# OzAmram/CaloDiffusion

Measured on AMD Instinct MI355X. Metric: sampled showers/sec (Dataset-2, 400-step DDIM), higher is better.
Workload: dtype f32 (convs: fp32 operands as 2-term fp16 splits on the fp16 MFMA pipe, fp32 accumulate; attention/norms fp32)

## Files before the change

calodiffusion_amd/csrc/cd_common.h:

```cpp
#pragma once
#include <hip/hip_runtime.h>
#include <stdint.h>
#include <stddef.h>
#include <string>

typedef float f32x4 __attribute__((ext_vector_type(4)));
typedef float f32x16 __attribute__((ext_vector_type(16)));

struct CdSamplerOp;

namespace cd {

void set_error(const std::string& msg);
struct Fail {
  int code;
  std::string msg;
};
#define CD_HIP(expr)                                                                                  \
  do {                                                                                                \
    hipError_t _e = (expr);                                                                           \
    if (_e != hipSuccess)                                                                             \
      throw cd::Fail{-2, std::string(#expr) + ": " + hipGetErrorString(_e)};                          \
  } while (0)
#define CD_REQUIRE(cond, msg)                                                                         \
  do {                                                                                                \
    if (!(cond)) throw cd::Fail{-1, std::string(msg)};                                                \
  } while (0)

namespace prof {
bool enabled();
void begin();
int end(char* buf, int cap);
struct Scope {
  Scope(const char* category, hipStream_t s, double flops, double bytes);
  ~Scope();
  int idx;
  hipStream_t stream;
};
}

enum ConvPrecision { PREC_F16X2 = 0, PREC_BF16X3 = 1, PREC_F32 = 2 };
int conv_precision();
void set_conv_precision(int p);
void set_conv_precision_override(int p);

struct Dims3 {
  int d, h, w;
  __host__ __device__ int64_t vox() const { return (int64_t)d * h * w; }
};

inline size_t packed_weight_floats(int cin, int cout, int taps) {
  return (size_t)(cin / 32) * taps * ((cout + 31) / 32) * 2048;
}

struct ConvGeom {
  Dims3 in, out;
  int kd, kh, kw;
  int sz, sh, sw;
};

__device__ __forceinline__ float cd_fast_silu(float t) {
  return t * __builtin_amdgcn_rcpf(1.f + __builtin_amdgcn_exp2f(t * -1.4426950408889634f));
}

struct GnDefer {
  const float* part = nullptr;
  int units = 0;
  const float* gamma = nullptr;
  const float* beta = nullptr;
  const float* add = nullptr;
  int add_ld = 0;
  int C = 0, groups = 0;
  int64_t vox = 0;
  float* coef_out = nullptr;
  float* stat_out = nullptr;
};

struct ConvFusion {
  const float* coef = nullptr;
  int act = 0;
  float* ch_part = nullptr;
  int* units = nullptr;
  const void* wpk_bf16x3 = nullptr;
  int* status = nullptr;
  GnDefer defer;
  float* coef_buf = nullptr;
  const unsigned* in_absmax = nullptr;
  const float* add_src = nullptr;
  int* add_done = nullptr;
  int zs_chunks = 0;
  struct GnOut {
    const float* gamma = nullptr;
    const float* beta = nullptr;
    int groups = 0;
    const float* res0 = nullptr;
    const float* res1 = nullptr;
    int res_c0 = 0;
    float* part_out = nullptr;
    int* done = nullptr;
  } gn_out;
};
struct AbsmaxWords {
  unsigned* next = nullptr;
  unsigned* end = nullptr;
  unsigned* take() {
    CD_REQUIRE(next && next < end, "internal: out of max-|x| words");
    return next++;
  }
};
const unsigned* launch_absmax_bits(const float* x, size_t n, AbsmaxWords* words, hipStream_t s);
__host__ __device__ inline void pow2_scale_for(unsigned mb, float* scale, float* inv) {
  const int e = (int)((mb >> 23) & 0xff) - 127;
  int sexp = mb == 0u ? 0 : 10 - e;
  sexp = sexp < -100 ? -100 : (sexp > 100 ? 100 : sexp);
  union { unsigned u; float f; } a, b;
  a.u = (unsigned)(127 + sexp) << 23;
  b.u = (unsigned)(127 - sexp) << 23;
  *scale = a.f;
  *inv = b.f;
}
inline size_t packed_bf16x3_bytes(int cin, int cout, int taps) {
  return (size_t)(cin / 16) * taps * ((cout + 31) / 32) * 3 * 64 * 16;
}
inline size_t packed_f16x2_bytes(int cin, int cout, int taps) {
  return (size_t)(cin / 16) * taps * ((cout + 31) / 32) * 2 * 64 * 16;
}
inline size_t packed_split16_bytes(int cin, int cout, int taps) {
  return packed_bf16x3_bytes(cin, cout, taps) + packed_f16x2_bytes(cin, cout, taps);
}
void launch_pack_weights_bf16x3(const float* w_torch, void* wpk, int cout, int cin, int taps, hipStream_t s,
                                bool transposed = false, bool flip = false);
void launch_pack_weights_f16x2(const float* w_torch, void* wpk, int cout, int cin, int taps, hipStream_t s,
                               bool transposed = false, bool flip = false);
inline void launch_pack_weights_split16(const float* w_torch, void* wpk, int cout, int cin, int taps, hipStream_t s,
                                        bool transposed = false, bool flip = false) {
  launch_pack_weights_bf16x3(w_torch, wpk, cout, cin, taps, s, transposed, flip);
  launch_pack_weights_f16x2(w_torch, (char*)wpk + packed_bf16x3_bytes(cin, cout, taps), cout, cin, taps, s, transposed, flip);
}

void launch_pack_weights(const float* w_torch, float* wpk, int cout, int cin, int taps, bool transposed, hipStream_t s,
                         bool flip = false);
void launch_pack_init_weights(const float* w_torch, float* wpk, int cout, int cin, hipStream_t s);
struct PackJob {
  const float* src;
  float* raw;
  float* pk;
  void* bf3;
  void* f16;
  int cout, cin, taps;
  int kind;
  int tr, flip;
  unsigned long long numel, n_pk, n_bf3, n_f16;
};
void launch_pack_jobs(const PackJob* d_jobs, int njobs, hipStream_t s);
void launch_pack_jobs_f16x2(const PackJob* d_jobs, int njobs, hipStream_t s);

void launch_conv_mfma(const float* in0, int c0, const float* in1, int c1, const float* wpk, const float* bias, float* out,
                      int batch, int cout, const ConvGeom& g, hipStream_t s, const ConvFusion& fu = ConvFusion());
bool try_launch_conv_zslide(const float* in0, int c0, const float* in1, int c1, const void* wpk_f16x2, const float* bias, float* out,
                            int batch, int cout, const ConvGeom& g, hipStream_t s, const ConvFusion& fu);
bool try_launch_conv_small(const float* in0, int c0, const float* in1, int c1, const void* wpk_f16x2, const float* bias, float* out,
                           int batch, int cout, const ConvGeom& g, hipStream_t s, const ConvFusion& fu);
void launch_conv_transpose_mfma(const float* in, int cin, const float* wpk, const float* bias, float* out, int batch,
                                int cout, Dims3 din, Dims3 dout, int kz, int sz, hipStream_t s,
                                const void* wpk_f16x2 = nullptr, int* status = nullptr, const unsigned* in_absmax = nullptr);

enum A_Prologue { A_NONE = 0, A_AFFINE = 1, A_SOFTMAX32 = 2, A_EXPNORM = 3 };
struct PointwiseArgs {
  const float* in0 = nullptr;
  int ld0 = 0, off0 = 0, c0 = 0;
  const float* in1 = nullptr;
  int ld1 = 0, c1 = 0;
  const float* wpk = nullptr;
  int64_t w_batch_stride = 0;
  const float* bias = nullptr;
  const float* residual = nullptr;
  float* out = nullptr;
  int batch = 0, cout = 0;
  int64_t vox = 0;
  int prologue = A_NONE;
  const float* coef = nullptr;
  int out_ld = 0, out_off = 0;
  float* ch_part = nullptr;
  const float* gn_res = nullptr;
  GnDefer gn_defer;
  const void* wpk16 = nullptr;
  int* status = nullptr;
};
inline int pointwise_units(int64_t vox) { return (int)((vox + 127) / 128); }
void launch_pointwise(const PointwiseArgs& a, hipStream_t s);

struct InitConvArgs {
  const float* x = nullptr;
  int cx = 0;
  int cin = 0;
  const float* scale_b = nullptr;
  int scale_stride = 1;
  const float* sigma_b = nullptr;
  float sigma_data = 1.f;
  const float* r_w = nullptr;
  const float* z_d = nullptr;
  const float* phi_h = nullptr;
  int use_rz = 0, use_phi = 0;
  const float* wpk = nullptr;
  const float* bias = nullptr;
  float* out = nullptr;
  int batch = 0, cout = 0;
  Dims3 dims{};
  float* coord_table = nullptr;
  bool table_ready = false;
  int* status = nullptr;
};
void launch_init_conv(const InitConvArgs& a, hipStream_t s);
void launch_init_coord_table(const InitConvArgs& a, hipStream_t s);

int gn_nsplit_for(int64_t vox, int batch);
void launch_ch_stats(const float* x, float* part, int batch, int channels, int64_t vox, int nsplit, hipStream_t s);
void launch_gn_finalize(const float* part, int units, const float* gamma, const float* beta, const float* add_bc, int add_ld,
                        float* coef, int batch, int channels, int groups, int64_t vox, hipStream_t s,
                        float* stat_out = nullptr );

size_t wgrad_partial_floats(int64_t out_vox, int batch, bool per_sample, int A, int Bc, int T);
struct WgradReduceJob {
  const float* partial;
  float* dw;
  int A, Bc, T, nslots, flags , b_total, b_off;
  unsigned first_block;
};
struct WgradReduceQueue {
  static constexpr int kMax = 80;
  WgradReduceJob job[kMax];
  int n = 0;
  unsigned blocks = 0;
};
void wgrad_queue_flush(WgradReduceQueue* q, hipStream_t s);
struct WgradAux {
  WgradReduceQueue* queue = nullptr;
  AbsmaxWords* words = nullptr;
  const unsigned* gmax = nullptr;
  const unsigned* xmax = nullptr;
};
void launch_wgrad(const float* g, int A, Dims3 dg, const float* x, int Bc, int xld, int xoff, Dims3 dx, int kd, int kh, int kw,
                  int sz, int sxy, int batch, bool per_sample, float* partial, float* dw, bool accumulate, bool transposed_out,
                  hipStream_t s, int b_total = 0, int b_off = 0,
                  const float* xcoef = nullptr, const WgradAux& aux = WgradAux());
// ... 26 lines not shown
  float* db;
  int nout, nin, delta_ld, in_ld;
};
void launch_linear_wgrad(const LinearWgradJob* jobs_dev, int njobs, int max_elems, int batch, hipStream_t s);
void launch_fold_phi(const float* src, float* dst, int batch, Dims3 d, int C, hipStream_t s);
void launch_add_slices(const float* a, int lda, int aoff, const float* b, int ldb, int boff, float* out, int channels,
                       int64_t rows, hipStream_t s);
void launch_bias_grad(const float* part, int units, int batch, int channels, float* db, bool accumulate, hipStream_t s);
size_t gn_backward_scratch_floats(int batch, int channels, int64_t vox);
struct GnParamJob {
  const float* sums_bc;
  float *dgamma, *dbeta, *dbias, *dsumdy;
  int batch, channels;
};
struct GnParamJobs {
  static constexpr int kMax = 64;
  GnParamJob job[kMax];
  int n = 0;
};
struct GnParamQueue {
  GnParamJobs jobs;
  float* sums = nullptr;
  float* sums_end = nullptr;
  float* next_sums = nullptr;
  bool discard = false;
};
void launch_gn_param_jobs(const GnParamJobs& jobs, hipStream_t s);
void launch_gn_backward(const float* dy, const float* h, const float* coef, const float* stat, const float* gamma, float* dh,
                        float* dgamma, float* dbeta, float* dadd, int dadd_ld, int batch, int channels, int64_t vox, int groups,
                        int silu, float* scratch, bool accumulate_params, hipStream_t s,
                        float* dbias = nullptr, float* dsumdy = nullptr,
                        GnParamQueue* queue = nullptr,
                        unsigned* dh_absmax = nullptr);
int gn_apply_blocks_per_sample(int batch, int channels, int64_t vox);
void launch_gn_apply(const float* x, float* y, const float* coef, int batch, int channels, int64_t vox, int silu,
                     const float* residual, const float* residual1, int res_c0, float* part_out, hipStream_t s,
                     const GnDefer* defer = nullptr);

int attn_nsplit_for(int64_t vox, int batch);
size_t attn_partial_floats(int batch, int nsplit);
void launch_attn_context(const float* qkv, float* partials, int batch, int64_t vox, int nsplit, hipStream_t s);
void launch_attn_combine(const float* partials, int nsplit, const float* w_out , int cout, float* wpk_b,
                         int batch, float scale, hipStream_t s, float* ctx_out = nullptr ,
                         float* kstat_out = nullptr ,
                         bool layout_T = false );

int attn_fused_nsplit_for(int64_t vox, int batch);
bool try_launch_res_block_small(const float* x0, int c0, const float* x1, int c1, const void* w1_f16x2, const float* b1,
                                const float* gn1_gamma, const float* gn1_beta, const float* emb, int emb_ld, const void* w2_f16x2,
                                const float* b2, const float* gn2_gamma, const float* gn2_beta, int groups, const float* res0,
                                const float* res1, int res_c0, float* h1, float* out, float* part_out, int batch, int cout,
                                Dims3 dims, int* status, hipStream_t s);
struct DeepLevelDesc {
  Dims3 dims{};
  int Ca = 0, Cb = 0, groups = 0;
  struct Res {
    int c0 = 0, c1 = 0, cout = 0;
    const void *w1 = nullptr, *w2 = nullptr;
    const float *b1 = nullptr, *b2 = nullptr, *g1 = nullptr, *be1 = nullptr, *g2 = nullptr, *be2 = nullptr;
    const float* emb = nullptr;
    int emb_ld = 0;
    const void* wres = nullptr;
    const float* bres = nullptr;
  } res[6];
  struct Attn {
    int C = 0;
    const float *ng = nullptr, *nb = nullptr, *wout = nullptr, *bout = nullptr, *gg = nullptr, *gb = nullptr;
    const void* wqkv = nullptr;
  } attn[3];
  int has_attn[3] = {0, 0, 0};
};
bool deep_level_eligible(const DeepLevelDesc& d);
void launch_deep_level(const DeepLevelDesc& d, const float* x_in, float* x_out, int batch, int* status, hipStream_t s);
struct DeepSideConv {
  const float* in = nullptr;
  int ldc = 0, cin = 0;
  const void* wpk = nullptr;
  const float* bias = nullptr;
  float* out = nullptr;
  int cout = 0;
  Dims3 dims{};
};
int deep_side_conv_chunks(int batch, int cin_side, int cout, Dims3 dims);
void launch_deep_level_side(const DeepLevelDesc& d, const float* x_in, float* x_out, int batch, int* status, const DeepSideConv& side,
                            hipStream_t s);
bool attn_small_eligible(int64_t vox);
void launch_attn_small(const float* x, int C, const float* coef, const void* wqkv_f16x2, float* partials, const float* w_out,
                       float scale, const float* bias, const float* out_gamma, const float* out_beta, float* y, float* ch_part,
                       int batch, int64_t vox, hipStream_t s, const GnDefer* defer, int* status = nullptr,
                       int max_parts = 1, unsigned* coop_sync = nullptr);
constexpr int kAttnCoopSamples = 8192;
bool attn_moments_eligible(int C);
size_t attn_moment_floats(int batch, int nsplit);
void launch_attn_kv_context(const float* x, int C, const float* coef, const void* wqkv_f16x2, float* partials, int batch,
                            int64_t vox, int nsplit, hipStream_t s, const GnDefer* defer = nullptr, int* status = nullptr,
                            float* moments = nullptr);
void launch_attn_out(const float* x, int C, const float* coef, const void* wqkv_f16x2, const float* wT_b, const float* bias,
                     float* y, float* ch_part , int batch, int64_t vox, int nsplit, hipStream_t s,
                     const GnDefer* defer = nullptr,
                     const float* partials = nullptr, const float* w_out = nullptr, float scale = 0.f, int* status = nullptr,
                     const float* moments = nullptr, const float* out_gamma = nullptr, const float* out_beta = nullptr);

struct EmbedLayer {
  const float* w;
  const float* b;
  int cout;
  int offset;
};
struct EmbedArgs {
  const float* cond = nullptr;
  const float* time_or_sigma = nullptr;
  int time_kind = 0;
  float sigma_data = 1.f;
  int cond_size = 0, cond_hidden = 0, half = 0;
  const float *tw1, *tb1, *tw2, *tb2, *tw3, *tb3;
  const float *cw1, *cb1, *cw2, *cb2, *cw3, *cb3;
  const EmbedLayer* layers = nullptr;
  int n_layers = 0;
  float* emb = nullptr;
  int emb_ld = 0;
  float* scal = nullptr;
  int batch = 0;
  int time_sin = 0, cond_sin = 0;
  int cond_rows = 0, time_stride = 0;
  int part = 0;
};
void launch_embed(const EmbedArgs& a, hipStream_t s);
void launch_silu_linear(const float* cond, const float* w, const float* bias, float* out, int batch, int nin, int nout,
                        hipStream_t s);

struct HeadArgs {
  const float* h = nullptr;
  const float* w = nullptr;
  const float* bias = nullptr;
  const float* x = nullptr;
  const float* scal = nullptr;
  int objective = 0;
  float* out = nullptr;
  int batch = 0;
  int64_t vox = 0;
  GnDefer defer;
  const float* res = nullptr;
  const float* upd_stepvals = nullptr;
  const float* upd_noise = nullptr;
  float* upd_x_next = nullptr;
  float* upd_xs = nullptr;
  float* upd_x0s = nullptr;
};
void launch_head(const HeadArgs& a, hipStream_t s);

void launch_ddim_update(const float* x, const float* x0, const float* noise, const float* stepvals, float* x_next,
                        float* xs_slot, float* x0s_slot, int64_t n, hipStream_t s);
struct StepChunk {
  const float* emb_src = nullptr;
  float* emb_dst = nullptr;
  int emb_floats = 0;
  const float* scal_src = nullptr;
  float* scal_dst = nullptr;
  int scal_floats = 0;
  int chunk_steps = 0;
  const float* emb_cond = nullptr;
};
void launch_load_step(const float* table, int* counter, float* stepvals, float* sigma_b, int batch, hipStream_t s,
                      const StepChunk* chunk = nullptr);
void launch_scale(const float* x, float* y, const float* stepvals_sigma, int64_t n, hipStream_t s);
void launch_scale_imm(const float* x, float* y, float scale, int64_t n, hipStream_t s);
void launch_randn(float* out, int64_t n, uint64_t seed, uint64_t offset, hipStream_t s);
void launch_randn_step(float* out, int64_t n, const uint64_t* seed_offset_stride_dev, const int* step_counter, hipStream_t s,
// ... 177 lines not shown
```

calodiffusion_amd/csrc/conv_internal.h:

```cpp
#pragma once
#include "cd_common.h"
#include "split16.h"
#include <cstdio>
#include <cstdlib>
#include <map>
#include <string>

namespace cd {

#define MFMA32(a, b, c) __builtin_amdgcn_mfma_f32_32x32x2f32((a), (b), (c), 0, 0, 0)
#define MFMA_BF16(a, b, c) __builtin_amdgcn_mfma_f32_32x32x16_bf16(__builtin_bit_cast(bf16x8, (a)), __builtin_bit_cast(bf16x8, (b)), (c), 0, 0, 0)

typedef __bf16 bf16x8 __attribute__((ext_vector_type(8)));
typedef __bf16 bf16x2 __attribute__((ext_vector_type(2)));

__device__ __forceinline__ unsigned pack_bf16(float lo, float hi) {
  const bf16x2 v = {(__bf16)lo, (__bf16)hi};
  return __builtin_bit_cast(unsigned, v);
}
__device__ __forceinline__ void split3(const f32x4 x, u32x2& t1, u32x2& t2, u32x2& t3) {
  f32x4 r = x;
  t1 = u32x2{pack_bf16(r[0], r[1]), pack_bf16(r[2], r[3])};
  r[0] -= __uint_as_float(t1[0] << 16); r[1] -= __uint_as_float(t1[0] & 0xffff0000u);
  r[2] -= __uint_as_float(t1[1] << 16); r[3] -= __uint_as_float(t1[1] & 0xffff0000u);
  t2 = u32x2{pack_bf16(r[0], r[1]), pack_bf16(r[2], r[3])};
  r[0] -= __uint_as_float(t2[0] << 16); r[1] -= __uint_as_float(t2[0] & 0xffff0000u);
  r[2] -= __uint_as_float(t2[1] << 16); r[3] -= __uint_as_float(t2[1] & 0xffff0000u);
  t3 = u32x2{pack_bf16(r[0], r[1]), pack_bf16(r[2], r[3])};
}

struct ConvKArgs {
  const float* in0;
  const float* in1;
  int c0, c1;
  const float* wpk;
  const float* bias;
  float* out;
  int Din, Hin, Win, Do, Ho, Wo;
  int KD, KH, KW, SZ, SH, SW;
  int TZ, TH, nTZ, nTH;
  int IZ, IH;
  int cout, CTtot;
  const float* coef;
  int act;
};
struct ConvTiled3Args {
  ConvKArgs k;
  float* ch_part;
  int* status;
};
void launch_conv_tiled_f32(int VT, int CT, const ConvKArgs& a, dim3 grid, int threads, size_t lds, hipStream_t s);
void launch_conv_tiled_split16(int VT, int CT, int NTERM, const ConvTiled3Args& a, dim3 grid, int threads, size_t lds, hipStream_t s);

struct ConvFlatArgs {
  const float* in0;
  const float* in1;
  int c0, c1;
  const float* wpk;
  const float* bias;
  float* out;
  int D, H, W;
  int Do, Ho, Wo;
  int R;
  int P;
  int cout, CTtot;
  int dbg;
  const float* coef;
  int act;
  float* ch_part;
  int* status = nullptr;
  GnDefer defer;
  int coef_lds_off = 0;
  const unsigned* in_absmax = nullptr;
  const float* add_src = nullptr;
};
bool try_launch_conv3_flat(const float* in0, int c0, const float* in1, int c1, const void* wpk, const float* bias, float* out,
                           int batch, int cout, const ConvGeom& g, hipStream_t s, const ConvFusion& fu,
                           int prec );
bool launch_conv_flat_split16(int VT, int CT, int NTERM, int geo, const ConvFlatArgs& a, dim3 grid, int threads, size_t lds, hipStream_t s);

std::map<std::string, int>& tune_cache();
template <typename F>
int autotune(const std::string& key, int ncand, F&& run, hipStream_t s) {
  auto it = tune_cache().find(key);
  if (it != tune_cache().end()) return it->second;
  hipStreamCaptureStatus st = hipStreamCaptureStatusNone;
  if (getenv("CD_NO_AUTOTUNE") || hipStreamIsCapturing(s, &st) != hipSuccess || st != hipStreamCaptureStatusNone || prof::enabled())
    return -1;
  hipEvent_t e0, e1;
  CD_HIP(hipEventCreate(&e0));
  CD_HIP(hipEventCreate(&e1));
  int best = 0;
  float best_ms = 1e30f;
  for (int i = 0; i < ncand; ++i) {
    run(i);
    CD_HIP(hipEventRecord(e0, s));
    run(i);
    run(i);
    CD_HIP(hipEventRecord(e1, s));
    CD_HIP(hipEventSynchronize(e1));
    float ms = 0.f;
    CD_HIP(hipEventElapsedTime(&ms, e0, e1));
    if (getenv("CD_TUNE_VERBOSE") && atoi(getenv("CD_TUNE_VERBOSE")) > 1) std::fprintf(stderr, "[calodiff autotune]   %s cand %d: %.1f us\n", key.c_str(), i, ms * 500.f);
    if (ms < best_ms) { best_ms = ms; best = i; }
  }
  hipEventDestroy(e0);
  hipEventDestroy(e1);
  tune_cache()[key] = best;
  if (getenv("CD_TUNE_VERBOSE")) std::fprintf(stderr, "[calodiff autotune] %s -> candidate %d (%.1f us)\n", key.c_str(), best, best_ms * 500.f);
  return best;
}

}
```

calodiffusion_amd/csrc/forward.hip:

```cpp
#include "plan_internal.h"

#include <cstdio>
#include <cstdlib>

namespace cd {

ResP resolve(const CdPlan* p, const ResW& w, const float* emb) {
  ResP r;
  r.cin = w.cin; r.cout = w.cout; r.has_res = w.has_res;
  r.c1w3 = p->packed3(w.c1w); r.c2w3 = p->packed3(w.c2w);
  r.c1w = p->packed(w.c1w); r.c1b = p->raw(w.c1b); r.n1g = p->raw(w.n1g); r.n1b = p->raw(w.n1b);
  r.c2w = p->packed(w.c2w); r.c2b = p->raw(w.c2b); r.n2g = p->raw(w.n2g); r.n2b = p->raw(w.n2b);
  if (w.has_res) {
    r.rw = p->packed(w.rw); r.rb = p->raw(w.rb);
    if (p->packed3(w.rw)) r.rw16 = (const char*)p->packed3(w.rw) + packed_bf16x3_bytes(w.cin, w.cout, 1);
  }
  if (w.has_mlp && emb) { r.emb = emb + w.emb_off; r.emb_ld = p->emb_ld; }
  return r;
}
AttnP resolve(const CdPlan* p, const AttnW& w) {
  AttnP a;
  a.c = w.c;
  a.ng = p->raw(w.ng); a.nb = p->raw(w.nb); a.qkv = p->packed(w.qkv); a.ow = p->raw(w.ow); a.ob = p->raw(w.ob);
  a.qkv16 = (const char*)p->packed3(w.qkv) + packed_bf16x3_bytes(w.c, 96, 1);
  a.gg = p->raw(w.gg); a.gb = p->raw(w.gb);
  a.coop_sync = p->d_attn_sync;
  return a;
}

float* stats_pass(Run& r, const float* x, int C, int64_t vox, int* units) {
  const int ns = gn_nsplit_for(vox, r.B);
  float* part = r.ws->get<float>((size_t)r.B * ns * C * 2);
  if (!r.dry()) launch_ch_stats(x, part, r.B, C, vox, ns, r.s);
  *units = ns;
  return part;
}

float* conv3_with_stats(Run& r, const float* x0, int c0, const float* x1, int c1, const float* wpk, const void* wpk3,
                        const float* bias, float* out, int cout, Dims3 dims, const float* coef_in, int* units,
                        const GnDefer* defer_in, float* coef_buf, const ConvFusion::GnOut* gn_out) {
  const int64_t vox = dims.vox();
  const int cap = (int)((vox + 31) / 32);
  float* part = r.ws->get<float>((size_t)r.B * cap * cout * 2);
  int u = 0;
  if (!r.dry()) {
    ConvGeom g{dims, dims, 3, 3, 3, 1, 1, 1};
    ConvFusion fu;
    fu.coef = coef_in; fu.act = 1; fu.ch_part = part; fu.units = &u; fu.wpk_bf16x3 = wpk3; fu.status = r.status;
    if (defer_in) { fu.defer = *defer_in; fu.coef_buf = coef_buf; fu.coef = nullptr; }
    if (gn_out) fu.gn_out = *gn_out;
    launch_conv_mfma(x0, c0, x1, c1, wpk, bias, out, r.B, cout, g, r.s, fu);
    if (gn_out && *gn_out->done) {
    } else if (u == 0) {
      u = gn_nsplit_for(vox, r.B);
      if (u > cap) u = cap;
      launch_ch_stats(out, part, r.B, cout, vox, u, r.s);
    }
  }
  *units = u;
  return part;
}

static float* conv3_x_half_with_stats(Run& r, const float* x0, int c0, int c1, const void* wpk3, float* out, int cout, Dims3 dims,
                                      int* units) {
  const int64_t vox = dims.vox();
  const int cap = (int)((vox + 31) / 32);
  float* part = r.ws->get<float>((size_t)r.B * cap * cout * 2);
  int u = 0;
  if (!r.dry()) {
    ConvGeom g{dims, dims, 3, 3, 3, 1, 1, 1};
    ConvFusion fu;
    int added = 0;
    fu.act = 1; fu.ch_part = part; fu.units = &u; fu.status = r.status; fu.add_src = out; fu.add_done = &added;
    char cat[128];
    std::snprintf(cat, sizeof cat, "conv3x3x3_s1 C%d(of %d)->%d @%dx%dx%d", c0, c0 + c1, cout, dims.d, dims.h, dims.w);
    prof::Scope scope(cat, r.s, 2.0 * 27 * c0 * cout * (double)vox * r.B, 4.0 * r.B * (double)vox * (c0 + 2 * cout));
    const bool ran = try_launch_conv_zslide(x0, c0, nullptr, 0, (const char*)wpk3 + packed_bf16x3_bytes(c0 + c1, cout, 27), nullptr, out,
                                            r.B, cout, g, r.s, fu);
    CD_REQUIRE(ran && added && u > 0, "internal: the x half of a side conv must run as a z-slide continuation");
  }
  *units = u;
  return part;
}

struct LazyClose {
  GnDefer gn;
  float* part = nullptr;
  bool on = false;
};
float* res_block(Run& r, const ResP& w, const float* x0, int c0, const float* x1, int c1, Dims3 dims,
                 float** part_out, int* units_out, LazyClose* lazy, float* h1_side) {
  Arena* ws = r.ws;
  CD_REQUIRE(c0 + c1 == w.cin, "internal: resnet block input width mismatch");
  const int64_t vox = dims.vox();
  const int G = r.groups;
  int u1 = 0, u2 = 0;
  static const bool defer_gn = getenv("CD_NO_GNDEFER") == nullptr;
  float* h1 = h1_side ? h1_side : ws->get<float>((size_t)r.B * vox * w.cout);
  const bool whole = vox <= 128 && w.cout == 32 && defer_gn && conv_precision() == PREC_F16X2 && w.c1w3 && w.c2w3;
  float* p1 = nullptr;
  CD_REQUIRE(!h1_side || (!whole && c1 > 0), "internal: a side conv belongs to a concat conv on a full-resolution grid");
  if (h1_side) p1 = conv3_x_half_with_stats(r, x0, c0, c1, w.c1w3, h1, w.cout, dims, &u1);
  else if (!whole) p1 = conv3_with_stats(r, x0, c0, x1, c1, w.c1w, w.c1w3, w.c1b, h1, w.cout, dims, nullptr, &u1);
  else p1 = ws->get<float>((size_t)r.B * ((vox + 31) / 32) * w.cout * 2);
  float* coef1 = ws->get<float>((size_t)r.B * w.cout * 4);
  GnDefer d1;
  d1.part = p1; d1.units = u1; d1.gamma = w.n1g; d1.beta = w.n1b; d1.add = w.emb; d1.add_ld = w.emb_ld; d1.C = w.cout; d1.groups = G;
  d1.vox = vox;
  if (!r.dry() && !defer_gn) launch_gn_finalize(p1, u1, w.n1g, w.n1b, w.emb, w.emb_ld, coef1, r.B, w.cout, G, vox, r.s);
  float* h2 = ws->get<float>((size_t)r.B * vox * w.cout);
  const bool small = vox <= 128;
  float* po = nullptr;
  const bool no_pw_close = getenv("CD_NO_PW_CLOSE") != nullptr;
  const bool pw_close = w.has_res && !small && defer_gn && !no_pw_close && w.cout <= 128;
  const int bps = pw_close ? pointwise_units(vox) : gn_apply_blocks_per_sample(r.B, w.cout, vox);
  if (part_out) {
    po = ws->get<float>((size_t)r.B * bps * w.cout * 2);
    *part_out = po;
  }
  float* res = nullptr;
  auto shortcut_conv = [&](const GnDefer* close = nullptr) {
    if (!close) res = ws->get<float>((size_t)r.B * vox * w.cout);
    if (!r.dry()) {
      PointwiseArgs a;
      a.in0 = x0; a.ld0 = c0; a.off0 = 0; a.c0 = c0; a.in1 = x1; a.ld1 = c1; a.c1 = c1;
      a.wpk = w.rw; a.bias = w.rb; a.out = close ? h2 : res; a.batch = r.B; a.cout = w.cout; a.vox = vox;
      if (conv_precision() == PREC_F16X2 && !getenv("CD_PW_F32")) { a.wpk16 = w.rw16; a.status = r.status; }
      if (close) { a.gn_res = h2; a.gn_defer = *close; a.ch_part = po; }
      launch_pointwise(a, r.s);
    }
  };
  if (small && w.has_res) shortcut_conv();
  int fused = 0;
  if (whole && !r.dry()) {
    const float* sc0 = w.has_res ? res : x0;
    const float* sc1 = w.has_res ? nullptr : (c1 ? x1 : nullptr);
    if (try_launch_res_block_small(x0, c0, x1, c1, (const char*)w.c1w3 + packed_bf16x3_bytes(c0 + c1, 32, 27), w.c1b, w.n1g, w.n1b,
                                   w.emb, w.emb_ld, (const char*)w.c2w3 + packed_bf16x3_bytes(32, 32, 27), w.c2b, w.n2g, w.n2b, G, sc0,
                                   sc1, w.has_res ? 0 : c0, h1, h2, po, r.B, w.cout, dims, r.status, r.s))
      fused = 2;
    else
      p1 = (ws->release(p1), conv3_with_stats(r, x0, c0, x1, c1, w.c1w, w.c1w3, w.c1b, h1, w.cout, dims, nullptr, &u1));
  }
  ConvFusion::GnOut go;
  if (small && defer_gn && fused != 2) {
    go.gamma = w.n2g; go.beta = w.n2b; go.groups = G; go.part_out = po; go.done = &fused;
    if (w.has_res) { go.res0 = res; }
    else { go.res0 = x0; go.res1 = c1 ? x1 : nullptr; go.res_c0 = c0; }
  }
  float* p2 = nullptr;
  if (fused == 2) p2 = ws->get<float>((size_t)r.B * ((vox + 31) / 32) * w.cout * 2);
  else p2 = conv3_with_stats(r, h1, w.cout, nullptr, 0, w.c2w, w.c2w3, w.c2b, h2, w.cout, dims, coef1, &u2, defer_gn ? &d1 : nullptr,
                             coef1, go.gamma ? &go : nullptr);
  ws->release(p1);
  ws->release(h1);
  ws->release(coef1);
  float* coef2 = ws->get<float>((size_t)r.B * w.cout * 4);
  GnDefer d2;
  d2.part = p2; d2.units = u2; d2.gamma = w.n2g; d2.beta = w.n2b; d2.C = w.cout; d2.groups = G; d2.vox = vox;
  if (!r.dry() && !defer_gn) launch_gn_finalize(p2, u2, w.n2g, w.n2b, nullptr, 0, coef2, r.B, w.cout, G, vox, r.s);
  const GnDefer* dp2 = defer_gn ? &d2 : nullptr;
  if (part_out) *units_out = fused ? 1 : bps;
  if (pw_close) {
    shortcut_conv(&d2);
  } else if (w.has_res) {
    if (!res) shortcut_conv();
    if (!r.dry() && !fused) launch_gn_apply(h2, h2, coef2, r.B, w.cout, vox, 1, res, nullptr, 0, po, r.s, dp2);
    ws->release(res);
  } else if (lazy && !small && defer_gn && c1 == 0 && w.cout == 32 && !part_out) {
    lazy->gn = d2;
    lazy->part = p2;
    lazy->on = true;
    ws->release(coef2);
    return h2;
  } else {
    if (!r.dry() && !fused) launch_gn_apply(h2, h2, coef2, r.B, w.cout, vox, 1, x0, c1 ? x1 : nullptr, c0, po, r.s, dp2);
  }
  ws->release(p2);
  ws->release(coef2);
  return h2;
}

float* attn_block(Run& r, const AttnP& w, const float* x, Dims3 dims, float* xpart, int xunits) {
  Arena* ws = r.ws;
  const int64_t vox = dims.vox();
// ... 184 lines not shown
  if (dx) {
    float* wp = pre ? nullptr : ws->get<float>(packed_weight_floats(c, c, T));
    float* wp3 = pre ? nullptr : ws->get<float>(packed_split16_bytes(c, c, T) / 4);
    if (!r.dry()) {
      if (!pre) {
        launch_pack_weights(w_raw, wp, c, c, T, false, r.s);
        launch_pack_weights_split16(w_raw, wp3, c, c, T, r.s, false, false);
      }
      ConvGeom gd{dout, din, kz, 4, 4, sz, 2, 2};
      ConvFusion fu;
      fu.wpk_bf16x3 = pre ? img->pk3 : wp3;
      dy_max = launch_absmax_bits(dy, (size_t)r.B * dout.vox() * c, &r.amax, r.s);
      fu.in_absmax = dy_max;
      launch_conv_mfma(dy, c, nullptr, 0, pre ? img->pk : wp, nullptr, dx, r.B, c, gd, r.s, fu);
    }
    if (wp3) ws->release(wp3);
    if (wp) ws->release(wp);
  }
  if (r.param_grads) {
    float* part = r.wgrad_part(wgrad_partial_floats(din.vox(), r.B, false, c, c, T));
    if (!r.dry())
      launch_wgrad(x, c, din, dy, c, c, 0, dout, kz, 4, 4, sz, 2, r.B, false, part, dw, false, false, r.s, 0, 0, nullptr,
                   r.wgrad_aux(nullptr, dy_max));
    r.release_wgrad_part(part);
    if (db) bias_grad(r, dy_full, c, dout_full.vox(), db);
  }
  if (folded) ws->release(folded);
}

bool deep_level_desc(const CdPlan* p, const float* emb, DeepLevelDesc* out) {
  const CdUnetDesc& d = p->desc;
  const int nres = p->nres;
  if (conv_precision() != PREC_F16X2) return false;
  DeepLevelDesc L;
  L.dims = p->shapes[nres - 1];
  L.Ca = d.layer_sizes[nres - 1]; L.Cb = d.layer_sizes[nres]; L.groups = d.groups;
  const ResW* rw[6] = {&p->downs[nres - 1].r1, &p->downs[nres - 1].r2, &p->mid1, &p->mid2, &p->ups[0].r1, &p->ups[0].r2};
  for (int i = 0; i < 6; ++i) {
    const ResW& w = *rw[i];
    DeepLevelDesc::Res& r = L.res[i];
    const bool cat = i == 4;
    r.c0 = cat ? L.Cb : w.cin; r.c1 = cat ? w.cin - L.Cb : 0; r.cout = w.cout;
    if (!p->packed3(w.c1w) || !p->packed3(w.c2w)) return false;
    r.w1 = (const char*)p->packed3(w.c1w) + packed_bf16x3_bytes(w.cin, w.cout, 27);
    r.w2 = (const char*)p->packed3(w.c2w) + packed_bf16x3_bytes(w.cout, w.cout, 27);
    r.b1 = p->raw(w.c1b); r.b2 = p->raw(w.c2b); r.g1 = p->raw(w.n1g); r.be1 = p->raw(w.n1b); r.g2 = p->raw(w.n2g); r.be2 = p->raw(w.n2b);
    if (w.has_mlp && emb) { r.emb = emb + w.emb_off; r.emb_ld = p->emb_ld; }
    if (w.has_res) {
      if (!p->packed3(w.rw)) return false;
      r.wres = (const char*)p->packed3(w.rw) + packed_bf16x3_bytes(w.cin, w.cout, 1);
      r.bres = p->raw(w.rb);
    }
  }
  const AttnW* aw[3] = {&p->downs[nres - 1].attn, &p->mid_attn, &p->ups[0].attn};
  const bool on[3] = {d.block_attn != 0, d.mid_attn != 0, d.block_attn != 0};
  for (int i = 0; i < 3; ++i) {
    L.has_attn[i] = on[i] ? 1 : 0;
    if (!on[i]) continue;
    const AttnW& w = *aw[i];
    DeepLevelDesc::Attn& a = L.attn[i];
    a.C = w.c; a.ng = p->raw(w.ng); a.nb = p->raw(w.nb); a.wout = p->raw(w.ow); a.bout = p->raw(w.ob); a.gg = p->raw(w.gg); a.gb = p->raw(w.gb);
    if (!p->packed3(w.qkv)) return false;
    a.wqkv = (const char*)p->packed3(w.qkv) + packed_bf16x3_bytes(w.c, 96, 1);
  }
  if (L.res[0].c0 != L.Ca || L.res[0].cout != L.Cb || L.res[4].cout != L.Ca || L.res[4].c1 != L.Cb || L.res[5].cout != L.Ca) return false;
  if (!deep_level_eligible(L)) return false;
  *out = L;
  return true;
}

float* unet_body(CdPlan* p, Run& r, const float* emb, float* h, LazyClose* lazy = nullptr, float** xin = nullptr) {
  const CdUnetDesc& d = p->desc;
  const int nres = p->nres;
  const int zs = d.compress_z ? 2 : 1;
  std::vector<float*> skips(nres, nullptr);
  float* x = h;
  int cx = d.layer_sizes[0];
  DeepLevelDesc deep;
  const bool deep_on = deep_level_desc(p, emb, &deep);
  const ResW& side_w = p->ups[nres - 1].r1;
  const int side_c = nres >= 2 ? d.layer_sizes[1] : 0;
  const bool side_on = deep_on && nres >= 2 && side_w.cin == 2 * side_c && p->packed3(side_w.c1w) &&
                       deep_side_conv_chunks(r.B, side_c, side_w.cout, p->shapes[0]) > 0;
  float* side_h1 = nullptr;
  for (int i = 0; i < nres; ++i) {
    const Dims3 dims = p->shapes[i];
    if (deep_on && i == nres - 1) {
      float* y = r.ws->get<float>((size_t)r.B * dims.vox() * cx);
      if (side_on) {
        side_h1 = r.ws->get<float>((size_t)r.B * p->shapes[0].vox() * side_w.cout);
        if (!r.dry()) {
          DeepSideConv sc;
          sc.in = skips[0]; sc.ldc = side_c; sc.cin = side_c;
          sc.wpk = (const char*)p->packed3(side_w.c1w) + packed_bf16x3_bytes(side_w.cin, side_w.cout, 27) +
                   (size_t)(side_c / 16) * 27 * (side_w.cout / 32) * 128 * 16;
          sc.bias = p->raw(side_w.c1b); sc.out = side_h1; sc.cout = side_w.cout; sc.dims = p->shapes[0];
          launch_deep_level_side(deep, x, y, r.B, r.status, sc, r.s);
        }
      } else if (!r.dry()) {
        launch_deep_level(deep, x, y, r.B, r.status, r.s);
      }
      r.ws->release(x);
      x = y;
      break;
    }
    float* t = res_block(r, resolve(p, p->downs[i].r1, emb), x, cx, nullptr, 0, dims);
    r.ws->release(x);
    x = t; cx = p->downs[i].r1.cout;
    float* xp = nullptr;
    int xu = 0;
    t = res_block(r, resolve(p, p->downs[i].r2, emb), x, cx, nullptr, 0, dims, d.block_attn ? &xp : nullptr, &xu);
    r.ws->release(x);
    x = t;
    if (d.block_attn) {
      t = attn_block(r, resolve(p, p->downs[i].attn), x, dims, xp, xu);
      r.ws->release(xp);
      r.ws->release(x);
      x = t;
    }
    skips[i] = x;
    if (i + 1 < nres) {
      const Dims3 nd = p->shapes[i + 1];
      float* y = r.ws->get<float>((size_t)r.B * nd.vox() * cx);
      if (!r.dry()) {
        ConvGeom g{dims, nd, 3, 4, 4, zs, 2, 2};
        ConvFusion fu;
        fu.wpk_bf16x3 = p->packed3(p->downs[i].sw);
        launch_conv_mfma(x, cx, nullptr, 0, p->packed(p->downs[i].sw), p->raw(p->downs[i].sb), y, r.B, cx, g, r.s, fu);
      }
      x = y;
    } else {
      x = skips[i];
    }
  }
  const Dims3 md = p->shapes[nres - 1];
  float* t = nullptr;
  if (!deep_on) {
    float* mp = nullptr;
    int mu = 0;
    t = res_block(r, resolve(p, p->mid1, emb), x, cx, nullptr, 0, md, d.mid_attn ? &mp : nullptr, &mu);
    x = t;
    if (d.mid_attn) {
      t = attn_block(r, resolve(p, p->mid_attn), x, md, mp, mu);
      r.ws->release(mp);
      r.ws->release(x);
      x = t;
    }
    t = res_block(r, resolve(p, p->mid2, emb), x, cx, nullptr, 0, md);
    r.ws->release(x);
    x = t;
  }

  for (int i = 0; i < nres; ++i) {
    const int lv = nres - 1 - i;
    const Dims3 dims = p->shapes[lv];
    const int cs = d.layer_sizes[lv + 1];
    if (!(deep_on && i == 0)) {
      CD_REQUIRE(cx == cs, "internal: up path width mismatch");
      t = res_block(r, resolve(p, p->ups[i].r1, emb), x, cx, skips[lv], cs, dims, nullptr, nullptr, nullptr,
                    lv == 0 ? side_h1 : nullptr);
      r.ws->release(x);
      r.ws->release(skips[lv]);
      x = t; cx = p->ups[i].r1.cout;
      float* up = nullptr;
      int uu = 0;
      t = res_block(r, resolve(p, p->ups[i].r2, emb), x, cx, nullptr, 0, dims, d.block_attn ? &up : nullptr, &uu);
      r.ws->release(x);
      x = t;
      if (d.block_attn) {
        t = attn_block(r, resolve(p, p->ups[i].attn), x, dims, up, uu);
        r.ws->release(up);
        r.ws->release(x);
        x = t;
      }
    }
    if (i + 1 < nres) {
      const Dims3 od = p->up_out[i];
      float* y = r.ws->get<float>((size_t)r.B * od.vox() * cx);
      if (!r.dry())
        launch_conv_transpose_mfma(x, cx, p->packed(p->ups[i].sw), p->raw(p->ups[i].sb), y, r.B, cx, dims, od, p->up_kz[i], zs, r.s,
                                   p->packed3(p->ups[i].sw), r.status);
      r.ws->release(x);
      x = y;
    }
  }
  t = res_block(r, resolve(p, p->fin, nullptr), x, cx, nullptr, 0, p->shapes[0], nullptr, nullptr, lazy);
  if (lazy && lazy->on) *xin = x;
  else r.ws->release(x);
  return t;
}

EmbedArgs embed_args(CdPlan* p, int B, const float* cond, const float* t, int kind, float* emb, float* scal) {
  const CdUnetDesc& d = p->desc;
  EmbedArgs e;
  e.cond = cond; e.time_or_sigma = t; e.time_kind = kind; e.sigma_data = d.sigma_data;
  e.cond_size = d.cond_size; e.half = d.cond_dim / 2;
  e.cond_hidden = d.cond_size > e.half / 2 ? d.cond_size : e.half / 2;
  e.time_sin = d.time_sin; e.cond_sin = d.cond_sin;
  e.tw1 = d.time_sin ? nullptr : p->raw(p->tw[0]); e.tb1 = d.time_sin ? nullptr : p->raw(p->tb[0]);
  e.tw2 = p->raw(p->tw[1]); e.tb2 = p->raw(p->tb[1]);
  e.tw3 = p->raw(p->tw[2]); e.tb3 = p->raw(p->tb[2]);
  e.cw1 = d.cond_sin ? nullptr : p->raw(p->cw[0]); e.cb1 = d.cond_sin ? nullptr : p->raw(p->cb[0]);
  e.cw2 = p->raw(p->cw[1]); e.cb2 = p->raw(p->cb[1]);
  e.cw3 = p->raw(p->cw[2]); e.cb3 = p->raw(p->cb[2]);
  e.layers = p->d_embed_layers; e.n_layers = p->n_embed_layers; e.emb = emb; e.emb_ld = p->emb_ld; e.scal = scal; e.batch = B;
  return e;
}

void forward_impl(CdPlan* p, int B, const float* x, const float* cond, const float* t, float* out, bool raw, hipStream_t s,
                  const FwdOpts* opt) {
  const CdUnetDesc& d = p->desc;
  const Dims3 dims = p->shapes[0];
  Run r{&p->ws, s, B, d.groups};
  r.status = p->status_word;
  const bool pre = opt && opt->emb_pre;
  float* emb = pre ? opt->emb_pre : p->ws.get<float>((size_t)B * p->emb_ld);
  float* scal = pre ? opt->scal_pre : p->ws.get<float>((size_t)B * 4);
  float* h = p->ws.get<float>((size_t)B * dims.vox() * d.layer_sizes[0]);
  if (!r.dry()) {
    if (!pre) launch_embed(embed_args(p, B, cond, t, raw ? CD_TIME_RAW : d.time_embed_kind, emb, raw ? nullptr : scal), s);
    InitConvArgs a;
    a.x = x; a.cin = d.in_channels; a.wpk = p->packed(p->init_w); a.bias = p->raw(p->init_b); a.out = h; a.batch = B;
    a.cout = d.layer_sizes[0]; a.dims = dims;
    if (raw) {
      a.cx = d.in_channels;
    } else {
      a.cx = 1; a.sigma_b = t; a.sigma_data = d.sigma_data; a.use_rz = d.rz_input; a.use_phi = d.phi_input;
      a.r_w = p->d_coords; a.z_d = p->d_coords + d.grid[2]; a.phi_h = p->d_coords + d.grid[2] + d.grid[0];
      a.coord_table = p->d_init_table; a.table_ready = true; a.status = r.status;
    }
    launch_init_conv(a, s);
  }
  LazyClose lazy;
  float* xin = nullptr;
  static const bool head_fused = getenv("CD_NO_HEAD_GN") == nullptr;
  float* hf = unet_body(p, r, emb, h, head_fused ? &lazy : nullptr, &xin);
  if (!r.dry()) {
    HeadArgs ha;
    ha.h = hf; ha.w = p->raw(p->head_w); ha.bias = p->raw(p->head_b); ha.out = out; ha.batch = B; ha.vox = dims.vox();
    if (!raw) { ha.x = x; ha.scal = scal; ha.objective = d.objective; }
    if (lazy.on) { ha.defer = lazy.gn; ha.res = xin; }
    if (opt && opt->upd) {
      ha.upd_stepvals = opt->upd->upd_stepvals; ha.upd_noise = opt->upd->upd_noise; ha.upd_x_next = opt->upd->upd_x_next;
// ... 98 lines not shown
```

calodiffusion_amd/csrc/kernels_conv_flat.hip:

```cpp
#include "conv_internal.h"
#include "gn_defer.h"
#include <vector>

namespace cd {

template <int VT, int CT>
__global__ void __launch_bounds__(512, (VT * CT <= 2 ? 3 : 2)) conv3_flat_kernel(ConvFlatArgs a) {
  extern __shared__ __attribute__((aligned(16))) float lds[];
  const int tid = threadIdx.x, lane = tid & 63, wave = tid >> 6, nthreads = blockDim.x;
  const int b = blockIdx.y;
  const int ct0 = blockIdx.z * CT;
  const int HW = a.H * a.W;
  const int vox = a.D * HW;
  const int v0 = blockIdx.x * a.R;
  const int vend = min(v0 + a.R, vox);
  const int zA = v0 / HW - 1;
  const int zB = (vend - 1) / HW + 1;
  const int nstage = (zB - zA + 1) * HW;
  const int NZ = a.P * HW;
  const int half = lane >> 5, col = lane & 31;
  if (tid < 16) lds[NZ * 16 + tid] = 0.f;

  int nb[VT], rowm[VT], rowp[VT], ooff[VT];
  unsigned wmask[VT];
// ... 381 lines not shown
          const int off = __shfl(ooff, row, 64);
          if (off >= 0) {
#pragma unroll
            for (int ct = 0; ct < CT; ++ct) {
              const float v = acc[ct][r] + bv[ct];
              outb[off + (ct0 + ct) * 32 + col] = v;
              s1[ct] += v;
              s2[ct] += v * v;
            }
          }
        }
        if (a.ch_part) {
#pragma unroll
          for (int ct = 0; ct < CT; ++ct) {
            const float t1 = s1[ct] + __shfl_xor(s1[ct], 32, 64), t2 = s2[ct] + __shfl_xor(s2[ct], 32, 64);
            if (half == 0) {
              scratch[((mw * CT + ct) * 32 + col) * 2] = t1;
              scratch[((mw * CT + ct) * 32 + col) * 2 + 1] = t2;
            }
          }
        }
      }
    }
    __syncthreads();
  }
  if (loader && a.ch_part && nph > 0) {
    const int u = blockIdx.x + (my_units - 1) * gridDim.x;
    for (int i = tid; i < CT * 32; i += nlw * 64) {
      float t1 = 0.f, t2 = 0.f;
      for (int w = 0; w < nmw; ++w) {
        t1 += scratch[((w * CT * 32) + i) * 2];
        t2 += scratch[((w * CT * 32) + i) * 2 + 1];
      }
      float* dst = a.ch_part + ((size_t)u * a.cout + ct0 * 32 + i) * 2;
      dst[0] = t1;
      dst[1] = t2;
    }
  }
}

namespace {
template <int CT, int KD, int KH, int KW, int SZ, int SXY>
void launch_ws_geo(const ConvFlatArgs& a, dim3 grid, int threads, size_t lds, int nlw, int ups, int total, hipStream_t s) {
  static bool attr_set = false;
  if (!attr_set) {
    CD_HIP(hipFuncSetAttribute((const void*)conv_flat_ws_kernel<CT, KD, KH, KW, SZ, SXY>,
                               hipFuncAttributeMaxDynamicSharedMemorySize, 160 * 1024));
    attr_set = true;
  }
  hipLaunchKernelGGL((conv_flat_ws_kernel<CT, KD, KH, KW, SZ, SXY>), grid, dim3(threads), lds, s, a, nlw, ups, total);
  CD_HIP(hipGetLastError());
}
template <int CT>
void launch_ws_inst(const ConvFlatArgs& a, dim3 grid, int threads, size_t lds, int nlw, int ups, int total, hipStream_t s, int geo) {
  if (geo == 0) launch_ws_geo<CT, 3, 3, 3, 1, 1>(a, grid, threads, lds, nlw, ups, total, s);
  else if (geo == 1) launch_ws_geo<CT, 3, 4, 4, 2, 2>(a, grid, threads, lds, nlw, ups, total, s);
  else if (geo == 2) launch_ws_geo<CT, 3, 4, 4, 1, 2>(a, grid, threads, lds, nlw, ups, total, s);
  else launch_ws_geo<CT, 4, 4, 4, 2, 2>(a, grid, threads, lds, nlw, ups, total, s);
}

template <int VT, int CT>
void launch_flat_inst(const ConvFlatArgs& a, dim3 grid, int threads, size_t lds, hipStream_t s) {
  static bool attr_set = false;
  if (!attr_set) {
    CD_HIP(hipFuncSetAttribute((const void*)conv3_flat_kernel<VT, CT>, hipFuncAttributeMaxDynamicSharedMemorySize, 160 * 1024));
    attr_set = true;
  }
  hipLaunchKernelGGL((conv3_flat_kernel<VT, CT>), grid, dim3(threads), lds, s, a);
  CD_HIP(hipGetLastError());
}

bool launch_conv_flat_f32(int VT, int CT, const ConvFlatArgs& a, dim3 grid, int threads, size_t lds, hipStream_t s) {
#define CD_FLAT_CASE(V, C)                                   \
  if (VT == V && CT == C) {                                  \
    launch_flat_inst<V, C>(a, grid, threads, lds, s);        \
    return true;                                             \
  }
  CD_FLAT_CASE(1, 1) CD_FLAT_CASE(2, 1) CD_FLAT_CASE(3, 1) CD_FLAT_CASE(4, 1)
  CD_FLAT_CASE(1, 2) CD_FLAT_CASE(2, 2) CD_FLAT_CASE(3, 2) CD_FLAT_CASE(4, 2)
  CD_FLAT_CASE(1, 3) CD_FLAT_CASE(2, 3)
#undef CD_FLAT_CASE
  return false;
}
}

bool try_launch_conv3_flat(const float* in0, int c0, const float* in1, int c1, const void* wpk, const float* bias, float* out,
                           int batch, int cout, const ConvGeom& g, hipStream_t s, const ConvFusion& fu, int prec) {
  const bool bf16x3 = prec != 0;
  if (getenv("CD_NO_FLAT")) return false;
  int geo = -1;
  if (g.kd == 3 && g.kh == 3 && g.kw == 3 && g.sz == 1 && g.sh == 1 && g.sw == 1) geo = 0;
  else if (g.kd == 3 && g.kh == 4 && g.kw == 4 && g.sh == 2 && g.sw == 2 && (g.sz == 1 || g.sz == 2)) geo = g.sz == 2 ? 1 : 2;
  else if (g.kd == 4 && g.kh == 4 && g.kw == 4 && g.sh == 2 && g.sw == 2 && g.sz == 2) geo = 3;
  if (geo < 0 || (geo != 0 && !bf16x3)) return false;
  const Dims3 d = g.in;
  const int CTtot = cout / 32;
  const int CTmax = CTtot <= 3 ? CTtot : 2;
  if (CTtot % CTmax) return false;
  const int HW = d.h * d.w, HWo = g.out.h * g.out.w;
  const size_t vox_bytes = prec == 3 ? 96 : (prec == 2 ? 80 : 64);
  auto planes = [&](int NT) { return ((32 * NT - 1) / HWo + 1) * g.sz + g.kd; };
  auto args_for = [&](int NT) {
    ConvFlatArgs a;
    a.in0 = in0; a.in1 = in1; a.c0 = c0; a.c1 = c1; a.wpk = (const float*)wpk; a.bias = bias; a.out = out;
    a.D = d.d; a.H = d.h; a.W = d.w; a.Do = g.out.d; a.Ho = g.out.h; a.Wo = g.out.w;
    a.R = 32 * NT; a.P = planes(NT); a.cout = cout; a.CTtot = CTtot;
    a.coef = fu.coef; a.act = fu.act; a.ch_part = fu.ch_part;
    return a;
  };
  auto launch = [&](int NT, int VT, int CT) -> bool {
    if (VT < 0) {
      const int NLW = -VT;
      ConvFlatArgs a = args_for(NT);
      a.dbg = 0;
      const size_t lds = 2 * ((size_t)a.P * HW + 1) * 96 + (size_t)NT * CT * 64 * 4;
      const int ups = (int)((g.out.vox() + a.R - 1) / a.R);
      const int total = ups * batch;
      const int nblk = total < 256 ? total : 256;
      dim3 grid((unsigned)nblk, 1, (unsigned)(CTtot / CT));
      if (fu.units) *fu.units = ups;
      const int threads = (NT + NLW) * 64;
      switch (CT) {
        case 1: launch_ws_inst<1>(a, grid, threads, lds, NLW, ups, total, s, geo); break;
        case 2: launch_ws_inst<2>(a, grid, threads, lds, NLW, ups, total, s, geo); break;
        case 3: launch_ws_inst<3>(a, grid, threads, lds, NLW, ups, total, s, geo); break;
        default: return false;
      }
      return true;
    }
    ConvFlatArgs a = args_for(NT);
    a.dbg = getenv("CD_FLAT_DBG") ? atoi(getenv("CD_FLAT_DBG")) : 0;
    a.status = fu.status; a.in_absmax = fu.in_absmax;
    a.add_src = prec >= 2 && !bias ? fu.add_src : nullptr;
    size_t lds = ((size_t)a.P * HW + 1) * vox_bytes;
    const size_t red = (size_t)(NT / VT) * CT * 32 * 2 * 4;
    if (lds < red) lds = red;
    if (fu.defer.part) {
      lds = (lds + 15) & ~(size_t)15;
      a.defer = fu.defer;
      a.coef_lds_off = (int)lds;
      lds += (size_t)fu.defer.C * 16 + gn_defer_scratch_bytes(fu.defer.C);
      if (lds > 160 * 1024) return false;
    }
    dim3 grid((unsigned)((g.out.vox() + a.R - 1) / a.R), (unsigned)batch, (unsigned)(CTtot / CT));
    if (fu.units) *fu.units = (int)grid.x;
    const int threads = (NT / VT) * 64;
    const bool launched = prec != 0 ? launch_conv_flat_split16(VT, CT, prec, geo, a, grid, threads, lds, s)
                                    : launch_conv_flat_f32(VT, CT, a, grid, threads, lds, s);
    if (!launched) return false;
    if (a.add_src && fu.add_done) *fu.add_done = 1;
    return true;
  };
  if (const char* ov = getenv("CD_FLAT_TILE")) {
    int nt, vt;
    if (sscanf(ov, "%d,%d", &nt, &vt) == 2 && nt % vt == 0 && nt / vt <= 8 && vt * CTmax <= 8 &&
        ((size_t)planes(nt) * HW + 1) * vox_bytes <= 160 * 1024 && (prec != 2 || vt * CTmax <= 4))
      return launch(nt, vt, CTmax);
  }
  static const int kCand[][2] = {{8, 2}, {4, 1}, {8, 1}, {12, 3}, {16, 2}, {16, 4}, {4, 2}, {6, 2}, {6, 3}, {2, 1},
                                 {3, 1}, {1, 1}, {2, 2}, {12, 2}, {8, 4}, {6, 1}, {3, 3}};
  struct Cand { int nt, vt, ct; };
  std::vector<Cand> cand;
  const bool small = g.out.vox() * batch <= 64 * 1024;
  for (int pass = 0; pass < (small && CTmax > 1 ? 2 : 1); ++pass) {
    const int CT = pass == 0 ? CTmax : 1;
    for (auto& c : kCand) {
      const int NT = c[0], VT = c[1];
      if (VT * CT > 8 || (CT == 3 && VT > 2)) continue;
      if (prec == 2 && VT * CT > 4) continue;
      static const bool no_extra_waves = getenv("CD_FLAT_NO_EXTRA_WAVES") != nullptr;
      const bool extra_ok = !no_extra_waves && g.out.vox() <= 128 && VT == 1 && NT <= 8;
      if ((int64_t)32 * (NT - 1) >= g.out.vox() && !extra_ok) continue;
      if (((size_t)planes(NT) * HW + 1) * vox_bytes > 150 * 1024) continue;
      if (pass == 1 && NT > 4) continue;
      cand.push_back({NT, VT, CT});
    }
  }
  if (prec == 3 && !getenv("CD_NO_WS")) {
    static const int kWs[][2] = {{8, 4}, {8, 2}, {4, 2}, {4, 4}, {8, 3}, {6, 2}, {2, 2}, {3, 1}, {1, 1}, {2, 1}};
    for (auto& c : kWs) {
      const int NMW = c[0], NLW = c[1];
      if ((int64_t)32 * (NMW - 1) >= g.out.vox()) continue;
      const size_t lds = 2 * ((size_t)planes(NMW) * HW + 1) * 96 + (size_t)NMW * CTmax * 64 * 4;
      if (lds > 160 * 1024 - 256) continue;
      cand.push_back({NMW, -NLW, CTmax});
    }
  }
  if (cand.empty()) return false;
  char key[192];
  std::snprintf(key, sizeof key, "flat%s g%d %dx%dx%d c%d+%d->%d b%d", prec == 3 ? "_bf16x3" : (prec == 2 ? "_f16x2" : "_f32"), geo,
                d.d, d.h, d.w, c0, c1, cout, batch);
  const int pick = autotune(key, (int)cand.size(), [&](int i) { launch(cand[i].nt, cand[i].vt, cand[i].ct); }, s);
  const Cand& c = cand[pick < 0 ? 0 : pick];
  return launch(c.nt, c.vt, c.ct);
}

}
```

calodiffusion_amd/csrc/kernels_conv_flat16.hip:

```cpp
#include "conv_internal.h"
#include "gn_defer.h"

namespace cd {

template <int VT, int CT, int KD, int KH, int KW, int SZ, int SXY, int NTERM>
__global__ void __launch_bounds__(512, (VT * CT * (NTERM == 2 ? 2 : 1) <= 2 ? 3 : 2)) conv3_flat_bf16x3_kernel(ConvFlatArgs a) {
  extern __shared__ __attribute__((aligned(16))) float lds[];
  char* ldsb = (char*)lds;
  constexpr int T = KD * KH * KW;
  constexpr int VB = NTERM == 3 ? 96 : 80;
  constexpr int WS = 64 * NTERM;
  const int tid = threadIdx.x, lane = tid & 63, wave = tid >> 6, nthreads = blockDim.x;
  const int b = blockIdx.y;
  const int ct0 = blockIdx.z * CT;
  const int HW = a.H * a.W;
  const int vox = a.D * HW;
  const int HWo = a.Ho * a.Wo;
  const int voxo = a.Do * HWo;
  const int v0 = blockIdx.x * a.R;
  const int vend = min(v0 + a.R, voxo);
  const float inv_hwo = 1.f / (float)HWo, inv_wo = 1.f / (float)a.Wo;
  auto fdiv = [](int x, float inv) { return (int)(((float)x + 0.5f) * inv); };
  const int zA = fdiv(v0, inv_hwo) * SZ - 1;
  const int zB = fdiv(vend - 1, inv_hwo) * SZ + KD - 2;
  const int nstage = (zB - zA + 1) * HW;
  const int NZ = a.P * HW;
  const int half = lane >> 5, col = lane & 31;
  if (a.defer.part) gn_defer_to_lds(a.defer, b, (float*)(ldsb + a.coef_lds_off), ldsb + a.coef_lds_off + a.defer.C * 16);
  const bool normed = a.coef || a.defer.part;
  if (tid < VB / 4) ((float*)(ldsb + (size_t)NZ * VB))[tid] = 0.f;

  int nb[VT], rowoff[VT][KH], ooff[VT];
  unsigned wmask[VT];
  bool any_valid = false;
#pragma unroll
  for (int vt = 0; vt < VT; ++vt) {
    const int v = v0 + (wave * VT + vt) * 32 + col;
    const bool valid = v < vend;
    const int vv = valid ? v : v0;
    const int oz = fdiv(vv, inv_hwo);
    const int r = vv - oz * HWo;
    const int oh = fdiv(r, inv_wo), ow = r - oh * a.Wo;
    const int ih0 = oh * SXY, iw0 = ow * SXY;
    nb[vt] = (oz * SZ - 1 - zA) * HW + ih0 * a.W + iw0;
    unsigned m = 0;
#pragma unroll
    for (int kh = 0; kh < KH; ++kh) {
      int ih = ih0 + kh - 1;
      ih = ih < 0 ? ih + a.H : (ih >= a.H ? ih - a.H : ih);
      ih = ih >= a.H ? ih - a.H : ih;
      rowoff[vt][kh] = (ih - ih0) * a.W;
    }
#pragma unroll
    for (int kw = 0; kw < KW; ++kw) {
      const int iw = iw0 + kw - 1;
      if (valid && iw >= 0 && iw < a.W) m |= 1u << kw;
    }
    wmask[vt] = m;
    ooff[vt] = valid ? v * a.cout : -1;
    any_valid |= valid;
  }
  const bool wave_active = __any(any_valid);

  f32x16 acc[VT][CT], accB[NTERM == 2 ? VT : 1][NTERM == 2 ? CT : 1];
#pragma unroll
  for (int vt = 0; vt < VT; ++vt)
#pragma unroll
    for (int ct = 0; ct < CT; ++ct)
#pragma unroll
      for (int r = 0; r < 16; ++r) {
        acc[vt][ct][r] = 0.f;
        if (NTERM == 2) accB[vt][ct][r] = 0.f;
      }

  float amax = 0.f;
  float gscale = 1.f, ginv = 1.f;
  if (NTERM == 2 && a.in_absmax) pow2_scale_for(*a.in_absmax, &gscale, &ginv);
  const int nsub = (a.c0 + a.c1) >> 4;
  const int gbase = zA * HW;
  const int nslots = nstage * 4;

  auto tap_voxel = [&](int vt, int tap) -> int {
#ifdef CD_FLAT_ABL_TAPS
    return nb[vt] + tap;
#endif
    const int kz = tap / (KH * KW), kh = (tap / KW) % KH, kw = tap % KW;
    const int n = nb[vt] + kz * HW + rowoff[vt][kh] + kw - 1;
    return ((wmask[vt] >> kw) & 1u) ? n : NZ;
  };

  for (int sc = 0; sc < nsub; ++sc) {
    const float* src;
    int ldc, coff;
    if (sc * 16 < a.c0) {
      src = a.in0; ldc = a.c0; coff = sc * 16;
    } else {
      src = a.in1; ldc = a.c1; coff = sc * 16 - a.c0;
    }
    const int pq = tid & 3;
    src += (size_t)b * vox * ldc + coff + pq * 4;
    f32x4 cf[4];
    if (a.defer.part) {
#pragma unroll
      for (int e = 0; e < 4; ++e) cf[e] = *(const f32x4*)(ldsb + a.coef_lds_off + (sc * 16 + pq * 4 + e) * 16);
    } else if (a.coef) {
#pragma unroll
      for (int e = 0; e < 4; ++e) cf[e] = *(const f32x4*)(a.coef + ((size_t)b * (a.c0 + a.c1) + sc * 16 + pq * 4 + e) * 4);
    }
    __syncthreads();
    for (int s0 = tid; s0 < ((a.dbg & 1) ? 0 : nslots); s0 += 4 * nthreads) {
      f32x4 val[4];
#pragma unroll
      for (int k = 0; k < 4; ++k) {
        const int sidx = s0 + k * nthreads;
        const int g = gbase + (sidx >> 2);
        val[k] = f32x4{0.f, 0.f, 0.f, 0.f};
        if (sidx < nslots && g >= 0 && g < vox) {
          val[k] = *(const f32x4*)(src + (size_t)g * ldc);
          if (normed) {
#pragma unroll
            for (int e = 0; e < 4; ++e) {
              float t = cf[e][0] * val[k][e] + cf[e][1];
              if (a.act) t = cd_fast_silu(t);
              val[k][e] = t + cf[e][2];
            }
          }
        }
      }
#pragma unroll
      for (int k = 0; k < 4; ++k) {
        const int sidx = s0 + k * nthreads;
        if (sidx < nslots) {
          char* d = ldsb + (size_t)(sidx >> 2) * VB + pq * 8;
          if (NTERM == 3) {
            u32x2 t1, t2, t3;
            split3(val[k], t1, t2, t3);
            *(u32x2*)d = t1;
            *(u32x2*)(d + 32) = t2;
            *(u32x2*)(d + 64) = t3;
          } else {
            const f32x4 vs = val[k] * gscale;
            amax = fmaxf(amax, fmaxf(fmaxf(fabsf(vs[0]), fabsf(vs[1])), fmaxf(fabsf(vs[2]), fabsf(vs[3]))));
            u32x2 t1, t2;
            split2(vs, t1, t2);
            *(u32x2*)d = t1;
            *(u32x2*)(d + 32) = t2;
          }
        }
      }
    }
    __syncthreads();
    if (!wave_active || (a.dbg & 2)) continue;

#pragma unroll
    for (int vt = 0; vt < VT; ++vt) asm volatile("" : "+v"(nb[vt]));

    const u32x4* wq = (const u32x4*)a.wpk + ((size_t)sc * T * a.CTtot + ct0) * WS + lane;
#ifndef CD_FLAT_WD
#define CD_FLAT_WD 3
#endif
#ifndef CD_FLAT_AD
#define CD_FLAT_AD 2
#endif
    constexpr bool DEEP = NTERM == 2;
    constexpr int WD = DEEP ? CD_FLAT_WD : 1, AD = DEEP ? CD_FLAT_AD : 1;
    u32x4 bw[WD + 1][CT][NTERM], av[AD + 1][VT][NTERM];
    auto load_w = [&](int tap) {
#pragma unroll
      for (int ct = 0; ct < CT; ++ct)
#pragma unroll
        for (int t = 0; t < NTERM; ++t) bw[tap % (WD + 1)][ct][t] = wq[((size_t)tap * a.CTtot + ct) * WS + t * 64];
    };
    auto load_a = [&](int tap) {
#pragma unroll
      for (int vt = 0; vt < VT; ++vt) {
        const char* p = ldsb + (size_t)tap_voxel(vt, tap) * VB + half * 16;
#pragma unroll
        for (int t = 0; t < NTERM; ++t) av[tap % (AD + 1)][vt][t] = *(const u32x4*)(p + t * 32);
      }
    };
#pragma unroll
    for (int t0 = 0; t0 < WD; ++t0) load_w(t0);
#pragma unroll
    for (int t0 = 0; t0 < AD; ++t0) load_a(t0);
#pragma unroll
    for (int tap = 0; tap < T; ++tap) {
      if (tap + WD < T) load_w(tap + WD);
      if (tap + AD < T) load_a(tap + AD);
      __builtin_amdgcn_sched_barrier(0);
      const int wc = tap % (WD + 1), ac = tap % (AD + 1);
#pragma unroll
      for (int vt = 0; vt < VT; ++vt)
#pragma unroll
        for (int ct = 0; ct < CT; ++ct) {
          if (NTERM == 3) {
            f32x16 c = acc[vt][ct];
            c = MFMA_BF16(av[ac][vt][NTERM - 1], bw[wc][ct][0], c);
            c = MFMA_BF16(av[ac][vt][1], bw[wc][ct][1], c);
            c = MFMA_BF16(av[ac][vt][0], bw[wc][ct][NTERM - 1], c);
            c = MFMA_BF16(av[ac][vt][1], bw[wc][ct][0], c);
            c = MFMA_BF16(av[ac][vt][0], bw[wc][ct][1], c);
            c = MFMA_BF16(av[ac][vt][0], bw[wc][ct][0], c);
            acc[vt][ct] = c;
          } else {
            acc[vt][ct] = MFMA_F16(av[ac][vt][0], bw[wc][ct][0], acc[vt][ct]);
            accB[vt][ct] = MFMA_F16(av[ac][vt][0], bw[wc][ct][1], accB[vt][ct]);
            accB[vt][ct] = MFMA_F16(av[ac][vt][1], bw[wc][ct][0], accB[vt][ct]);
          }
        }
    }
  }

  if (NTERM == 2) {
#pragma unroll
    for (int vt = 0; vt < VT; ++vt)
#pragma unroll
      for (int ct = 0; ct < CT; ++ct)
#pragma unroll
        for (int r = 0; r < 16; ++r) acc[vt][ct][r] = (acc[vt][ct][r] + accB[vt][ct][r] * (1.f / 2048.f)) * ginv;
  }
  if (NTERM == 2 && a.status && amax > 65504.f) atomicOr(a.status, 1);
  float* outb = a.out + (size_t)b * voxo * a.cout;
  float bv[CT];
#pragma unroll
  for (int ct = 0; ct < CT; ++ct) bv[ct] = a.bias ? a.bias[(ct0 + ct) * 32 + col] : 0.f;
  if (a.add_src) {
    const float* addb = a.add_src + (size_t)b * voxo * a.cout;
#pragma unroll
    for (int vt = 0; vt < VT; ++vt) {
      float ad[16][CT];
#pragma unroll
      for (int r = 0; r < 16; ++r) {
        const int off = __shfl(ooff[vt], (r & 3) + 8 * (r >> 2) + 4 * half, 64);
#pragma unroll
        for (int ct = 0; ct < CT; ++ct) ad[r][ct] = off >= 0 ? addb[off + (ct0 + ct) * 32 + col] : 0.f;
      }
#pragma unroll
      for (int r = 0; r < 16; ++r)
#pragma unroll
        for (int ct = 0; ct < CT; ++ct) acc[vt][ct][r] += ad[r][ct];
    }
  }
#pragma unroll
  for (int vt = 0; vt < VT; ++vt) {
#pragma unroll
    for (int r = 0; r < 16; ++r) {
      const int row = (r & 3) + 8 * (r >> 2) + 4 * half;
      const int off = __shfl(ooff[vt], row, 64);
      if (off >= 0) {
#pragma unroll
        for (int ct = 0; ct < CT; ++ct) outb[off + (ct0 + ct) * 32 + col] = acc[vt][ct][r] + bv[ct];
      }
    }
  }
  if (a.ch_part) {
    float s1[CT], s2[CT];
#pragma unroll
    for (int ct = 0; ct < CT; ++ct) s1[ct] = s2[ct] = 0.f;
#pragma unroll
    for (int vt = 0; vt < VT; ++vt)
#pragma unroll
      for (int r = 0; r < 16; ++r) {
        const int row = (r & 3) + 8 * (r >> 2) + 4 * half;
        const bool ok = __shfl(ooff[vt], row, 64) >= 0;
#pragma unroll
        for (int ct = 0; ct < CT; ++ct) {
          const float v = ok ? acc[vt][ct][r] + bv[ct] : 0.f;
          s1[ct] += v;
          s2[ct] += v * v;
        }
      }
    __syncthreads();
    const int nw = nthreads >> 6;
#pragma unroll
    for (int ct = 0; ct < CT; ++ct) {
      const float t1 = s1[ct] + __shfl_xor(s1[ct], 32, 64), t2 = s2[ct] + __shfl_xor(s2[ct], 32, 64);
      if (half == 0) {
        lds[((wave * CT + ct) * 32 + col) * 2] = t1;
        lds[((wave * CT + ct) * 32 + col) * 2 + 1] = t2;
      }
    }
    __syncthreads();
    for (int i = tid; i < CT * 32; i += nthreads) {
      float t1 = 0.f, t2 = 0.f;
      for (int w = 0; w < nw; ++w) {
        t1 += lds[((w * CT * 32) + i) * 2];
        t2 += lds[((w * CT * 32) + i) * 2 + 1];
      }
      float* dst = a.ch_part + (((size_t)b * gridDim.x + blockIdx.x) * a.cout + ct0 * 32 + i) * 2;
      dst[0] = t1;
      dst[1] = t2;
    }
  }
}

namespace {
template <int VT, int CT, int KD, int KH, int KW, int SZ, int SXY, int NTERM>
void launch_flat3_geo(const ConvFlatArgs& a, dim3 grid, int threads, size_t lds, hipStream_t s) {
  static bool attr_set = false;
  if (!attr_set) {
    CD_HIP(hipFuncSetAttribute((const void*)conv3_flat_bf16x3_kernel<VT, CT, KD, KH, KW, SZ, SXY, NTERM>,
                               hipFuncAttributeMaxDynamicSharedMemorySize, 160 * 1024));
    attr_set = true;
  }
  hipLaunchKernelGGL((conv3_flat_bf16x3_kernel<VT, CT, KD, KH, KW, SZ, SXY, NTERM>), grid, dim3(threads), lds, s, a);
  CD_HIP(hipGetLastError());
}
template <int VT, int CT, int NTERM>
void launch_flat3_inst(const ConvFlatArgs& a, dim3 grid, int threads, size_t lds, hipStream_t s, int geo = 0) {
  if (geo == 0) launch_flat3_geo<VT, CT, 3, 3, 3, 1, 1, NTERM>(a, grid, threads, lds, s);
  else if (geo == 1) launch_flat3_geo<VT, CT, 3, 4, 4, 2, 2, NTERM>(a, grid, threads, lds, s);
  else if (geo == 2) launch_flat3_geo<VT, CT, 3, 4, 4, 1, 2, NTERM>(a, grid, threads, lds, s);
  else launch_flat3_geo<VT, CT, 4, 4, 4, 2, 2, NTERM>(a, grid, threads, lds, s);
}
}

bool launch_conv_flat_split16(int VT, int CT, int NTERM, int geo, const ConvFlatArgs& a, dim3 grid, int threads, size_t lds, hipStream_t s) {
#define CD_FLAT_CASE(V, C)                                                                 \
  if (VT == V && CT == C) {                                                                \
    if (NTERM == 3) launch_flat3_inst<V, C, 3>(a, grid, threads, lds, s, geo);             \
    else if constexpr (V * C <= 4) launch_flat3_inst<V, C, 2>(a, grid, threads, lds, s, geo); \
    else return false;                                                                     \
    return true;                                                                           \
  }
  CD_FLAT_CASE(1, 1) CD_FLAT_CASE(2, 1) CD_FLAT_CASE(3, 1) CD_FLAT_CASE(4, 1)
  CD_FLAT_CASE(1, 2) CD_FLAT_CASE(2, 2) CD_FLAT_CASE(3, 2) CD_FLAT_CASE(4, 2)
  CD_FLAT_CASE(1, 3) CD_FLAT_CASE(2, 3)
#undef CD_FLAT_CASE
  return false;
}

}
```

calodiffusion_amd/csrc/kernels_deep_side.hip:

```cpp
#include "cd_common.h"
#include "split16.h"
#include "gn_defer.h"

#include <cstdio>
#include <cstdlib>
#include <cstring>

namespace cd {

#include "deep_body.inc"
#include "conv_zs_body.inc"

namespace {

static_assert(DC_THREADS == 256, "both roles are programs of four waves");

struct DeepSideArgs {
  DeepArgs deep;
  ConvZsArgs side;
  int ndeep;
};

template <int NT>
__global__ void __launch_bounds__(256, 1) deep_level_side_kernel(DeepSideArgs a) {
  extern __shared__ __attribute__((aligned(16))) char ds_lds[];
  const int bx = blockIdx.x;
  if (bx < a.ndeep) {
    deep_level_body<NT>(a.deep, ds_lds, bx);
    return;
  }
  const int j = bx - a.ndeep;
  ZsBlk kb;
  kb.y = j / a.side.nchunk;
  kb.x = j - kb.y * a.side.nchunk;
  kb.z = 0;
  kb.nx = a.side.nchunk;
  switch (threadIdx.x >> 6) {
    case 0: z3_wave<0, false, 0, 0, ZS_NSL>(a.side, ds_lds, kb); break;
    case 1: z3_wave<1, false, 0, 0, ZS_NSL>(a.side, ds_lds, kb); break;
    case 2: z3_wave<2, false, 0, 0, ZS_NSL>(a.side, ds_lds, kb); break;
    default: z3_wave<3, false, 0, 0, ZS_NSL>(a.side, ds_lds, kb); break;
  }
}

template <int NT>
void launch_deep_side_inst(const DeepSideArgs& a, unsigned grid, size_t lds, hipStream_t s) {
  static bool attr_set = false;
  if (!attr_set) {
    CD_HIP(hipFuncSetAttribute((const void*)deep_level_side_kernel<NT>, hipFuncAttributeMaxDynamicSharedMemorySize, 160 * 1024));
    attr_set = true;
  }
  hipLaunchKernelGGL(deep_level_side_kernel<NT>, dim3(grid), dim3(256), lds, s, a);
  CD_HIP(hipGetLastError());
}

int side_ring(const Dims3& d) { return d.h * d.w >= 2 * ZS_STEP ? 4 : 5; }
size_t side_lds(const Dims3& d) {
  const size_t plane = ((size_t)d.h * d.w * ZS_VB + 255) & ~(size_t)255;
  return (size_t)ZS_ZERO + Z3_COEF + (size_t)side_ring(d) * plane + 2 * Z3_XCH;
}

}

int deep_side_conv_chunks(int batch, int cin_side, int cout, Dims3 dims) {
  if (getenv("CD_NO_DEEP_SIDE_CONV")) return 0;
  static const bool zs_switched = getenv("CD_NO_ZSLIDE") || getenv("CD_ZS_V1") || getenv("CD_ZS_STRIP") || getenv("CD_ZS_DBG") ||
                                  getenv("CD_ZS_NSL5") || getenv("CD_ZS_NSL");
  if (zs_switched) return 0;
  if (Z3_PAD || cin_side != 32 || cout != 32 || batch < 1) return 0;
  const int PV = dims.h * dims.w;
  if (PV < ZS_STEP || PV > ZS_NSL * 32 || side_lds(dims) > 160 * 1024) return 0;
  const int64_t svox = (int64_t)dims.d * PV;
  int best = 0;
  int64_t best_gap = 0;
  for (int n = 1; n <= 8 && svox >= (int64_t)2 * ZS_STEP * n; ++n) {
    const int64_t cv = ((svox + n - 1) / n + ZS_STEP - 1) / ZS_STEP * ZS_STEP;
    if ((svox + cv - 1) / cv != n) continue;
    const int64_t total = (int64_t)batch * (1 + n);
    const int64_t gap = (total + 255) / 256 * 256 - total;
    if (!best || gap < best_gap) { best = n; best_gap = gap; }
  }
  return best;
}

void launch_deep_level_side(const DeepLevelDesc& d, const float* x_in, float* x_out, int batch, int* status, const DeepSideConv& sc,
                            hipStream_t s) {
  DeepSideArgs a;
  double flops = 0.0;
  const size_t lds_deep = deep_fill_args(d, x_in, x_out, status, &a.deep, &flops);
  const int nchunk = deep_side_conv_chunks(batch, sc.cin, sc.cout, sc.dims);
  CD_REQUIRE(nchunk > 0 && sc.in && sc.wpk && sc.out, "internal: deep level launched with an ineligible side conv");
  const int PV = sc.dims.h * sc.dims.w;
  const int64_t svox = (int64_t)sc.dims.d * PV;
  ConvZsArgs& z = a.side;
  z = ConvZsArgs{};
  z.in = sc.in; z.ldc = sc.ldc; z.coef = nullptr; z.coef_c = sc.cin; z.act = 0;
  z.wpk = (const u32x4*)sc.wpk; z.CTtot = sc.cout / 32;
  z.bias = sc.bias; z.acc_delta = 0; z.out = sc.out; z.cout = sc.cout; z.ch_part = nullptr;
  z.D = sc.dims.d; z.H = sc.dims.h; z.W = sc.dims.w; z.NR = side_ring(sc.dims); z.HS = sc.dims.h;
  z.nchunk = nchunk;
  z.CV = (int)(((svox + nchunk - 1) / nchunk + ZS_STEP - 1) / ZS_STEP * ZS_STEP);
  z.status = status; z.defer = GnDefer(); z.choff = 0; z.in_absmax = nullptr; z.dbg = 0;
  a.ndeep = batch;
  const size_t lds_side = side_lds(sc.dims);
  const size_t lds = lds_deep > lds_side ? lds_deep : lds_side;
  const int64_t grid = (int64_t)batch * (1 + nchunk);
  CD_REQUIRE(lds <= 160 * 1024 && grid < (1ll << 31), "deep level + side conv: launch geometry out of range");
  const double vox = (double)d.dims.vox();
  char cat[128];
  std::snprintf(cat, sizeof cat, "deep_level C%d/%d @%dx%dx%d + conv3x3x3 K-block C%d->%d @%dx%dx%d", d.Ca, d.Cb, d.dims.d, d.dims.h,
                d.dims.w, sc.cin, sc.cout, sc.dims.d, sc.dims.h, sc.dims.w);
  prof::Scope scope(cat, s, flops * batch + 2.0 * 27 * sc.cin * sc.cout * (double)svox * batch,
                    8.0 * batch * vox * d.Ca + 4.0 * batch * (double)svox * (sc.cin + sc.cout));
  const int NT = (int)((d.dims.vox() + 31) / 32);
  switch (NT) {
    case 1: launch_deep_side_inst<1>(a, (unsigned)grid, lds, s); break;
    case 2: launch_deep_side_inst<2>(a, (unsigned)grid, lds, s); break;
    case 3: launch_deep_side_inst<3>(a, (unsigned)grid, lds, s); break;
    default: launch_deep_side_inst<4>(a, (unsigned)grid, lds, s); break;
  }
}

}
```

calodiffusion_amd/csrc/ops.hip:

```cpp
#include "plan_internal.h"

extern "C" {

static AbsmaxWords op_absmax_words(Arena& ws, hipStream_t s) {
  constexpr size_t kWords = 8;
  unsigned* w = ws.get<unsigned>(kWords);
  CD_HIP(hipMemsetAsync(w, 0, sizeof(unsigned) * kWords, s));
  return AbsmaxWords{w, w + kWords};
}
size_t cd_op_scratch_bytes(int batch, int max_channels, int64_t max_voxels) {
  return (size_t)256 * 256 * 64 * 4 * 4 + (size_t)batch * 64 * 64 * 16 + (size_t)batch * max_channels * max_voxels * 4 + (1 << 20);
}

int cd_op_to_channels_last(const float* ncdhw, float* ndhwc, int batch, int channels, int64_t voxels, void* stream) {
  return guarded([&] { launch_transpose_to_cl(ncdhw, ndhwc, batch, channels, voxels, (hipStream_t)stream); });
}
int cd_op_to_ncdhw(const float* ndhwc, float* ncdhw, int batch, int channels, int64_t voxels, void* stream) {
  return guarded([&] { launch_transpose_to_planar(ndhwc, ncdhw, batch, channels, voxels, (hipStream_t)stream); });
}

int cd_op_cyl_conv(const float* x0, int c0, const float* x1, int c1, const float* w, const float* bias, float* y,
                   int batch, int cout, const int32_t dims_in[3], const int32_t kernel[3], const int32_t stride[3],
                   void* scratch, void* stream) {
  return guarded([&] {
    CD_REQUIRE(x0 && w && y && scratch, "null argument");
    hipStream_t s = (hipStream_t)stream;
    const int taps = kernel[0] * kernel[1] * kernel[2];
    float* wpk = (float*)scratch;
    launch_pack_weights(w, wpk, cout, c0 + c1, taps, false, s);
    const Dims3 din{dims_in[0], dims_in[1], dims_in[2]};
    if (taps == 1) {
      PointwiseArgs a;
      a.in0 = x0; a.ld0 = c0; a.c0 = c0; a.in1 = x1; a.ld1 = c1; a.c1 = c1; a.wpk = wpk; a.bias = bias; a.out = y;
      a.batch = batch; a.cout = cout; a.vox = din.vox();
      launch_pointwise(a, s);
    } else {
      CD_REQUIRE(cout % 32 == 0, "cout must be a multiple of 32");
      ConvGeom g;
      g.in = din;
      g.kd = kernel[0]; g.kh = kernel[1]; g.kw = kernel[2]; g.sz = stride[0]; g.sh = stride[1]; g.sw = stride[2];
      g.out = Dims3{(din.d + 2 - g.kd) / g.sz + 1, (din.h + 2 - g.kh) / g.sh + 1, (din.w + 2 - g.kw) / g.sw + 1};
      ConvFusion fu;
      if (taps == 27 || taps == 48) {
        float* w3 = wpk + packed_weight_floats(c0 + c1, cout, taps);
        launch_pack_weights_split16(w, w3, cout, c0 + c1, taps, s);
        fu.wpk_bf16x3 = w3;
      }
      launch_conv_mfma(x0, c0, x1, c1, wpk, bias, y, batch, cout, g, s, fu);
    }
  });
}

int cd_op_zslide_conv(const float* x, int cin, const float* w, const float* bias, float* y, float* ch_part, int* units, int batch,
                      int cout, const int32_t dims[3], int chunks, void* scratch, void* stream) {
  return guarded([&] {
    CD_REQUIRE(x && w && y && ch_part && units && scratch && chunks >= 0, "bad argument");
    CD_REQUIRE(cin % 32 == 0 && cout % 32 == 0, "channel counts must be multiples of 32");
    hipStream_t s = (hipStream_t)stream;
    launch_pack_weights_f16x2(w, scratch, cout, cin, 27, s);
    const Dims3 d{dims[0], dims[1], dims[2]};
    ConvGeom g{d, d, 3, 3, 3, 1, 1, 1};
    ConvFusion fu;
    int u = 0;
    fu.act = 1; fu.ch_part = ch_part; fu.units = &u; fu.zs_chunks = chunks;
    CD_REQUIRE(try_launch_conv_zslide(x, cin, nullptr, 0, scratch, bias, y, batch, cout, g, s, fu) && u > 0,
               "this grid is not eligible for the z-slide kernel");
    *units = u;
  });
}

int cd_op_cyl_conv_transpose(const float* x, const float* w, const float* bias, float* y, int batch, int channels,
                             const int32_t dims_in[3], int kernel_z, int stride_z, const int32_t out_pad[3],
                             void* scratch, void* stream) {
  return guarded([&] {
    CD_REQUIRE(x && w && y && scratch, "null argument");
    CD_REQUIRE(out_pad[0] == 0, "z output padding is always 0 (models.py:339)");
    hipStream_t s = (hipStream_t)stream;
    float* wpk = (float*)scratch;
    launch_pack_weights(w, wpk, channels, channels, kernel_z * 16, true, s);
    float* wpk16 = wpk + ((packed_weight_floats(channels, channels, kernel_z * 16) + 63) & ~(size_t)63);
    launch_pack_weights_f16x2(w, wpk16, channels, channels, kernel_z * 16, s, true, false);
    const Dims3 din{dims_in[0], dims_in[1], dims_in[2]};
    const Dims3 dout{(din.d - 1) * stride_z - 2 + kernel_z, 2 * din.h + out_pad[1], 2 * din.w + out_pad[2]};
    launch_conv_transpose_mfma(x, channels, wpk, bias, y, batch, channels, din, dout, kernel_z, stride_z, s, wpk16, nullptr);
  });
}

int cd_op_init_conv(const float* x_ncdhw, const float* w, const float* bias, float* y, int batch, int cin, int cout,
                    const int32_t dims[3], void* scratch, void* stream) {
  return guarded([&] {
    CD_REQUIRE(x_ncdhw && w && y && scratch, "null argument");
    hipStream_t s = (hipStream_t)stream;
    float* wpk = (float*)scratch;
    launch_pack_init_weights(w, wpk, cout, cin, s);
    InitConvArgs a;
    a.x = x_ncdhw; a.cx = cin; a.cin = cin; a.wpk = wpk; a.bias = bias; a.out = y; a.batch = batch; a.cout = cout;
    a.dims = Dims3{dims[0], dims[1], dims[2]};
    launch_init_conv(a, s);
  });
}

int cd_op_group_norm(const float* x, float* y, const float* gamma, const float* beta, int batch, int channels,
                     int64_t voxels, int groups, int silu, const float* add_bc, const float* residual,
                     void* scratch, void* stream) {
  return guarded([&] {
    CD_REQUIRE(x && y && gamma && beta && scratch, "null argument");
    hipStream_t s = (hipStream_t)stream;
    const int ns = gn_nsplit_for(voxels, batch);
    float* part = (float*)scratch;
    float* coef = part + (size_t)batch * ns * channels * 2;
    launch_ch_stats(x, part, batch, channels, voxels, ns, s);
    launch_gn_finalize(part, ns, gamma, beta, add_bc, channels, coef, batch, channels, groups, voxels, s);
    launch_gn_apply(x, y, coef, batch, channels, voxels, silu, residual, nullptr, 0, nullptr, s);
  });
}

int cd_op_resnet_block(const float* x0, int c0, const float* x1, int c1, const float* const* w, const float* cond, float* y,
                       int batch, int cout, const int32_t dims[3], int groups, void* workspace, size_t workspace_bytes,
                       void* stream) {
  return guarded([&] {
    CD_REQUIRE(x0 && w && y && workspace, "null argument");
    hipStream_t s = (hipStream_t)stream;
    const int cin = c0 + c1;
    Arena ws;
    ws.reset((char*)workspace, workspace_bytes, false);
    float* p1 = ws.get<float>(packed_weight_floats(cin, cout, 27));
    float* p2 = ws.get<float>(packed_weight_floats(cout, cout, 27));
    launch_pack_weights(w[0], p1, cout, cin, 27, false, s);
    launch_pack_weights(w[4], p2, cout, cout, 27, false, s);
    float* q1 = ws.get<float>(packed_split16_bytes(cin, cout, 27) / 4);
    float* q2 = ws.get<float>(packed_split16_bytes(cout, cout, 27) / 4);
    launch_pack_weights_split16(w[0], q1, cout, cin, 27, s);
    launch_pack_weights_split16(w[4], q2, cout, cout, 27, s);
    ResP r;
    r.cin = cin; r.cout = cout; r.has_res = w[10] != nullptr;
    r.c1w3 = q1; r.c2w3 = q2;
    r.c1w = p1; r.c1b = w[1]; r.n1g = w[2]; r.n1b = w[3]; r.c2w = p2; r.c2b = w[5]; r.n2g = w[6]; r.n2b = w[7];
    if (r.has_res) {
      float* p3 = ws.get<float>(packed_weight_floats(cin, cout, 1));
      launch_pack_weights(w[10], p3, cout, cin, 1, false, s);
      r.rw = p3; r.rb = w[11];
    }
    if (w[8] && cond) {
      float* emb = ws.get<float>((size_t)batch * cout);
      launch_silu_linear(cond, w[8], w[9], emb, batch, 128, cout, s);
      r.emb = emb; r.emb_ld = cout;
    }
    Run run{&ws, s, batch, groups};
    const Dims3 d{dims[0], dims[1], dims[2]};
    float* out = res_block(run, r, x0, c0, x1, c1, d);
    CD_HIP(hipMemcpyAsync(y, out, sizeof(float) * (size_t)batch * d.vox() * cout, hipMemcpyDeviceToDevice, s));
  });
}
// ... 77 lines not shown
```

calodiffusion_amd/csrc/plan_internal.h:

```cpp
#pragma once
#include "../../include/calodiff.h"
#include "cd_common.h"

#include <map>
#include <string>
#include <vector>

namespace cd {

enum PackKind { PK_NONE = 0, PK_CONV = 1, PK_CONVT = 2, PK_INIT = 3 };
struct WeightEntry {
  std::string name;
  int64_t numel = 0;
  size_t raw_off = 0;
  PackKind pack = PK_NONE;
  int cin = 0, cout = 0, taps = 0;
  size_t pk_off = 0;
  size_t pk3_off = 0;
  size_t grad_off = 0;
  bool set = false;
  int dg_mode = 0;
  size_t dg_pk_off = 0, dg_pk3_off = 0;
  bool dg_1x1 = false;
};
// ... 151 lines not shown
    if (dg_images && w.dg_mode) {
      g.pk = dg_images + w.dg_pk_off;
      if (w.dg_mode != 1) g.pk3 = dg_images + w.dg_pk3_off;
    }
    return g;
  }
  unsigned* d_attn_sync = nullptr;
  StepGraph ddim_graph, prog_graph;

  size_t grad_floats = 0;
  std::vector<LinearWgradJob> lin_jobs_host;
  LinearWgradJob* d_lin_jobs = nullptr;

  Arena ws;

  const float* raw(int i) const { return arena + weights[i].raw_off; }
  const float* packed(int i) const { return arena + weights[i].pk_off; }
  const void* packed3(int i) const { return weights[i].pk3_off ? (const void*)(arena + weights[i].pk3_off) : nullptr; }
};

namespace cd {

struct Run {
  Arena* ws;
  hipStream_t s;
  int B;
  int groups;
  int* status = nullptr;
  GnParamQueue* gq = nullptr;
  WgradReduceQueue* wq = nullptr;
  std::vector<float*> wq_held;
  AbsmaxWords amax;
  bool param_grads = true;
  bool dry() const { return ws->dry(); }
  unsigned* amax_word() { return dry() ? nullptr : amax.take(); }
  float* wgrad_part(size_t floats) {
    float* part = ws->get<float>(floats);
    if (wq) wq_held.push_back(part);
    return part;
  }
  void release_wgrad_part(float* part) {
    if (!wq) ws->release(part);
  }
  WgradAux wgrad_aux(const unsigned* gmax = nullptr, const unsigned* xmax = nullptr) {
    WgradAux a;
    a.queue = wq; a.words = &amax; a.gmax = gmax; a.xmax = xmax;
    return a;
  }
};

struct ResP {
  int cin = 0, cout = 0;
  bool has_res = false;
  const float *c1w = nullptr, *c1b = nullptr, *n1g = nullptr, *n1b = nullptr;
  const void *c1w3 = nullptr, *c2w3 = nullptr;
  const float *c2w = nullptr, *c2b = nullptr, *n2g = nullptr, *n2b = nullptr;
  const float *rw = nullptr, *rb = nullptr;
  const void* rw16 = nullptr;
  const float* emb = nullptr;
  int emb_ld = 0;
};
struct AttnP {
  int c = 0;
  const float *ng = nullptr, *nb = nullptr, *qkv = nullptr, *ow = nullptr, *ob = nullptr, *gg = nullptr, *gb = nullptr;
  const void* qkv16 = nullptr;
  unsigned* coop_sync = nullptr;
};

ResP resolve(const CdPlan* p, const ResW& w, const float* emb);
AttnP resolve(const CdPlan* p, const AttnW& w);

struct FwdOpts {
  float* emb_pre = nullptr;
  float* scal_pre = nullptr;
  const HeadArgs* upd = nullptr;
};

struct LazyClose;
float* stats_pass(Run& r, const float* x, int C, int64_t vox, int* units);
float* conv3_with_stats(Run& r, const float* x0, int c0, const float* x1, int c1, const float* wpk, const void* wpk3,
                        const float* bias, float* out, int cout, Dims3 dims, const float* coef_in, int* units,
                        const GnDefer* defer_in = nullptr, float* coef_buf = nullptr, const ConvFusion::GnOut* gn_out = nullptr);
float* res_block(Run& r, const ResP& w, const float* x0, int c0, const float* x1, int c1, Dims3 dims,
                 float** part_out = nullptr, int* units_out = nullptr, LazyClose* lazy = nullptr, float* h1_side = nullptr);
float* attn_block(Run& r, const AttnP& w, const float* x, Dims3 dims, float* xpart = nullptr, int xunits = 0);
void bias_grad(Run& r, const float* dy, int C, int64_t vox, float* db);
void conv_backward(Run& r, const float* x0, int c0, const float* x1, int c1, const float* w_raw, const float* dy, float* dx,
                   float* dw, float* db, int cout, const ConvGeom& g, const DgImg* img = nullptr, const float* xcoef = nullptr,
                   const float* dx_add = nullptr, int* dx_added = nullptr, const unsigned* dy_max = nullptr);
void conv_transpose_backward(Run& r, const float* x, const float* w_raw, const float* dy, float* dx, float* dw, float* db, int c,
                             Dims3 din, Dims3 dout, int kz, int sz, const DgImg* img = nullptr);
EmbedArgs embed_args(CdPlan* p, int B, const float* cond, const float* t, int kind, float* emb, float* scal);
void forward_impl(CdPlan* p, int B, const float* x, const float* cond, const float* t, float* out, bool raw, hipStream_t s,
                  const FwdOpts* opt = nullptr);
void check_ready(CdPlan* p, bool need_coords);
void dgrad_images(CdPlan* p);
void denoise_vjp_impl(CdPlan* p, int B, const float* x, const float* sigma, const float* cond, const float* gy, float* dx, float* grads,
                      bool param_grads, hipStream_t s);

template <typename F>
int guarded(F&& f) {
  (void)hipGetLastError();
  try {
    f();
    return CD_OK;
  } catch (const Fail& e) {
    (void)hipGetLastError();
    set_error(e.msg);
    return e.code;
  } catch (const std::exception& e) {
    (void)hipGetLastError();
    set_error(std::string("internal error: ") + e.what());
    return CD_EINVAL;
  }
}

template <typename F>
size_t dry_forward_bytes(CdPlan* plan, int batch, F&& front) {
  struct Restore {
    ~Restore() { set_conv_precision_override(-1); }
  } restore;
  size_t need = 0;
  for (int mode : {(int)PREC_F16X2, (int)PREC_BF16X3, (int)PREC_F32}) {
    set_conv_precision_override(mode);
    plan->ws.reset(nullptr, 0, true);
    front();
    forward_impl(plan, batch, nullptr, nullptr, nullptr, nullptr, false, nullptr);
    need = plan->ws.high() > need ? plan->ws.high() : need;
  }
  return need;
}

template <typename F>
bool run_with_range_fallback(CdPlan* plan, hipStream_t s, F&& run, bool report_sticky = true) {
  struct Restore {
    CdPlan* p;
    ~Restore() {
      p->status_word = p->d_counter + 2;
      set_conv_precision_override(-1);
    }
  } restore{plan};
  plan->status_word = plan->d_counter + 3;
  CD_HIP(hipMemsetAsync(plan->d_counter + 3, 0, sizeof(int), s));
  run(false);
  if (conv_precision() != PREC_F16X2) return false;
  int flags = 0;
  CD_HIP(hipMemcpyAsync(&flags, plan->d_counter + 3, sizeof(int), hipMemcpyDeviceToHost, s));
  CD_HIP(hipStreamSynchronize(s));
  if (!(flags & 1)) return false;
  set_conv_precision_override(PREC_BF16X3);
  run(true);
  if (report_sticky) launch_or_word(plan->d_counter + 2, 2, s);
  return true;
}

}
```

calodiffusion_amd/engine.py:

```python
from __future__ import annotations

import ctypes as C
import os
from typing import Dict, Optional, Sequence

import numpy as np
import torch

_HERE = os.path.dirname(os.path.abspath(__file__))
LIB_PATH = os.environ.get("CALODIFF_LIB") or os.path.join(_HERE, "lib", "libcalodiff_hip.so")

CD_MAX_SIZES = 8
CD_ABI_VERSION = 3
TIME_KINDS = {"log": 0, "sigma": 1, "raw": 2}
OBJECTIVES = {"hybrid": 0, "noise_pred": 1, "mean_pred": 2}
LOSS_TYPES = {"l2": 0, "l1": 1, "mse": 2, "huber": 3}


class CdUnetDesc(C.Structure):
    _fields_ = [
        ("struct_size", C.c_uint32),
        ("grid", C.c_int32 * 3),
        ("in_channels", C.c_int32),
        ("n_sizes", C.c_int32),
# ... 12 lines not shown
        ("time_sin", C.c_int32),
        ("cond_sin", C.c_int32),
    ]


SOP_LINCOMB, SOP_DENOISE, SOP_RANDN, SOP_RECORD, SOP_LINDIV, SOP_DENOISE_PS = 0, 1, 2, 3, 4, 5


class CdSamplerOp(C.Structure):
    _fields_ = [("kind", C.c_int32), ("dst", C.c_int32), ("nsrc", C.c_int32), ("src", C.c_int32 * 6), ("col", C.c_int32)]


class CdLayerMlpDesc(C.Structure):
    _fields_ = [("struct_size", C.c_uint32), ("dim_in", C.c_int32), ("hidden", C.c_int32), ("cond_emb", C.c_int32), ("cond_size", C.c_int32),
                ("n_res", C.c_int32), ("time_embed_kind", C.c_int32), ("objective", C.c_int32), ("sigma_data", C.c_float)]


class CdStep(C.Structure):
    _fields_ = [("sigma", C.c_float), ("sigma_prev_masked", C.c_float), ("ddim_sigma", C.c_float), ("denom", C.c_float)]


_P = C.c_void_p
_SIGNATURES = {
    "cd_last_error": (C.c_char_p, []),
    "cd_abi_version": (C.c_int, []),
    "cd_device_check": (C.c_int, [C.c_char_p, C.c_int]),
    "cd_plan_create": (C.c_int, [C.POINTER(CdUnetDesc), C.POINTER(_P)]),
    "cd_plan_destroy": (C.c_int, [_P]),
    "cd_plan_num_weights": (C.c_int, [_P, C.POINTER(C.c_int)]),
    "cd_plan_weight_name": (C.c_int, [_P, C.c_int, C.c_char_p, C.c_int, C.POINTER(C.c_int64)]),
    "cd_plan_set_weight": (C.c_int, [_P, C.c_char_p, _P, C.c_int64, _P]),
    "cd_plan_set_weights": (C.c_int, [_P, C.c_int, C.POINTER(_P), _P]),
    "cd_plan_set_coords": (C.c_int, [_P, _P, _P, _P, _P]),
    "cd_plan_workspace_bytes": (C.c_int, [_P, C.c_int, C.POINTER(C.c_size_t)]),
    "cd_unet_forward": (C.c_int, [_P, C.c_int, _P, _P, _P, _P, _P, C.c_size_t, _P]),
    "cd_denoise": (C.c_int, [_P, C.c_int, _P, _P, _P, _P, _P, C.c_size_t, _P]),
    "cd_denoise_safe": (C.c_int, [_P, C.c_int, _P, _P, _P, _P, _P, C.c_size_t, C.POINTER(C.c_int), _P]),
    "cd_ddim_sample": (C.c_int, [_P, C.c_int, _P, _P, C.POINTER(CdStep), C.c_int, _P, C.c_uint64, C.c_uint64, C.c_uint64, _P, _P, _P,
                                 C.c_int, _P, C.c_size_t, _P]),
    "cd_plan_sampler_workspace_bytes": (C.c_int, [_P, C.c_int, C.c_int, C.c_int, C.c_int, C.POINTER(C.c_size_t)]),
    "cd_sampler_run": (C.c_int, [_P, C.c_int, _P, C.c_float, _P, C.c_int, C.c_int, C.POINTER(CdSamplerOp), C.c_int,
                                 C.POINTER(C.c_int32), _P, C.c_int, _P, C.c_uint64, C.c_uint64, C.c_uint64, _P, _P, _P, C.c_int,
                                 _P, C.c_size_t, _P]),
    "cd_randn": (C.c_int, [_P, C.c_int64, C.c_uint64, C.c_uint64, _P]),
    "cd_plan_grad_layout": (C.c_int, [_P, C.c_int, C.POINTER(C.c_int64), C.POINTER(C.c_int64)]),
    "cd_plan_train_workspace_bytes": (C.c_int, [_P, C.c_int, C.POINTER(C.c_size_t)]),
    "cd_plan_status": (C.c_int, [_P, C.POINTER(C.c_int), _P]),
    "cd_layer_forward": (C.c_int, [_P, C.POINTER(C.c_void_p), C.c_int, C.c_int, _P, _P, _P, _P, _P]),
    "cd_layer_denoise": (C.c_int, [_P, C.POINTER(C.c_void_p), C.c_int, C.c_int, _P, _P, _P, _P, _P]),
    "cd_layer_sample": (C.c_int, [_P, C.POINTER(C.c_void_p), C.c_int, C.c_int, _P, _P, _P, C.c_int, _P, _P, _P, _P, _P]),
    "cd_layer_sampler_run": (C.c_int, [_P, C.POINTER(C.c_void_p), C.c_int, C.c_int, _P, C.c_float, _P, C.c_int, C.c_int, _P, C.c_int,
                                       _P, _P, C.c_int, _P, C.c_uint64, C.c_uint64, C.c_uint64, _P, _P, _P, _P]),
    "cd_layer_train_workspace_bytes": (C.c_int, [_P, C.c_int, C.POINTER(C.c_size_t)]),
    "cd_layer_train_step": (C.c_int, [_P, C.POINTER(C.c_void_p), C.c_int, C.c_int, _P, _P, _P, _P, _P, _P, _P, C.c_size_t, _P]),
    "cd_layer_train_step_loss": (C.c_int, [_P, C.POINTER(C.c_void_p), C.c_int, C.c_int, _P, _P, _P, _P, C.c_int, _P, _P, _P, C.c_size_t,
                                           _P]),
    "cd_layer_loss": (C.c_int, [_P, C.POINTER(C.c_void_p), C.c_int, C.c_int, _P, _P, _P, _P, C.c_int, _P, _P, C.c_size_t, _P]),
    "cd_layer_vjp_workspace_bytes": (C.c_int, [_P, C.c_int, C.c_int, C.POINTER(C.c_size_t)]),
    "cd_layer_denoise_vjp": (C.c_int, [_P, C.POINTER(C.c_void_p), C.c_int, C.c_int, _P, _P, _P, _P, _P, _P, _P, C.c_size_t, _P]),
    "cd_reverse_norm": (C.c_int, [_P, _P, _P, _P, C.c_int, C.POINTER(C.c_int32), C.POINTER(C.c_float), C.c_float, C.c_float, _P]),
    "cd_reverse_norm_staged": (C.c_int, [_P, _P, _P, _P, C.c_int, C.POINTER(C.c_int32), C.POINTER(C.c_float), C.c_float, C.c_float,
                                         C.c_float, C.c_float, C.c_int, _P]),
    "cd_preprocess": (C.c_int, [_P, _P, _P, _P, _P, _P, C.c_int, C.POINTER(C.c_int32), C.POINTER(C.c_float), C.c_float, C.c_float,
                                C.c_float, C.c_int, C.c_float, _P]),
    "cd_adam_step": (C.c_int, [C.c_int, C.POINTER(C.c_void_p), C.POINTER(C.c_void_p), C.POINTER(C.c_void_p), C.POINTER(C.c_void_p),
                               C.POINTER(C.c_int64), C.c_double, C.c_double, C.c_double, C.c_float, C.c_float, C.c_int, _P]),
    "cd_train_step": (C.c_int, [_P, C.c_int, _P, _P, _P, _P, C.c_int, _P, _P, _P, C.c_size_t, _P]),
    "cd_plan_vjp_workspace_bytes": (C.c_int, [_P, C.c_int, C.c_int, C.POINTER(C.c_size_t)]),
    "cd_denoise_vjp": (C.c_int, [_P, C.c_int, _P, _P, _P, _P, _P, _P, _P, C.c_size_t, _P]),
    "cd_plan_bns_workspace_bytes": (C.c_int, [_P, C.c_int, C.c_int, C.POINTER(C.c_size_t)]),
    "cd_bns_theta_grad": (C.c_int, [_P, C.c_int, C.c_int, _P, _P, _P, _P, _P, _P, _P, C.c_size_t, _P]),
    "cd_set_conv_precision": (C.c_int, [C.c_char_p]),
    "cd_get_conv_precision": (C.c_char_p, []),
    "cd_profile_begin": (C.c_int, []),
    "cd_profile_end": (C.c_int, [C.c_char_p, C.c_int]),
    "cd_loss_hybrid_l2": (C.c_int, [_P, C.c_int, _P, _P, _P, _P, _P, _P, C.c_size_t, _P]),
    "cd_loss_hybrid": (C.c_int, [_P, C.c_int, _P, _P, _P, _P, C.c_int, _P, _P, C.c_size_t, _P]),
    "cd_op_to_channels_last": (C.c_int, [_P, _P, C.c_int, C.c_int, C.c_int64, _P]),
    "cd_op_to_ncdhw": (C.c_int, [_P, _P, C.c_int, C.c_int, C.c_int64, _P]),
    "cd_op_cyl_conv": (C.c_int, [_P, C.c_int, _P, C.c_int, _P, _P, _P, C.c_int, C.c_int, C.POINTER(C.c_int32),
                                 C.POINTER(C.c_int32), C.POINTER(C.c_int32), _P, _P]),
    "cd_op_zslide_conv": (C.c_int, [_P, C.c_int, _P, _P, _P, _P, C.POINTER(C.c_int), C.c_int, C.c_int, C.POINTER(C.c_int32), C.c_int,
                                    _P, _P]),
    "cd_op_cyl_conv_transpose": (C.c_int, [_P, _P, _P, _P, C.c_int, C.c_int, C.POINTER(C.c_int32), C.c_int, C.c_int,
                                           C.POINTER(C.c_int32), _P, _P]),
    "cd_op_init_conv": (C.c_int, [_P, _P, _P, _P, C.c_int, C.c_int, C.c_int, C.POINTER(C.c_int32), _P, _P]),
    "cd_op_group_norm": (C.c_int, [_P, _P, _P, _P, C.c_int, C.c_int, C.c_int64, C.c_int, C.c_int, _P, _P, _P, _P]),
    "cd_op_resnet_block": (C.c_int, [_P, C.c_int, _P, C.c_int, C.POINTER(_P), _P, _P, C.c_int, C.c_int,
                                     C.POINTER(C.c_int32), C.c_int, _P, C.c_size_t, _P]),
    "cd_op_linear_attention": (C.c_int, [_P, C.POINTER(_P), _P, C.c_int, C.c_int, C.POINTER(C.c_int32), _P, C.c_size_t, _P]),
    "cd_op_conv_backward": (C.c_int, [_P, C.c_int, _P, C.c_int, _P, _P, _P, _P, _P, C.c_int, C.c_int, C.POINTER(C.c_int32),
                                      C.POINTER(C.c_int32), C.POINTER(C.c_int32), _P, C.c_size_t, _P]),
    "cd_op_conv_transpose_backward": (C.c_int, [_P, _P, _P, _P, _P, _P, C.c_int, C.c_int, C.POINTER(C.c_int32), C.c_int, C.c_int,
                                                C.POINTER(C.c_int32), _P, C.c_size_t, _P]),
    "cd_op_group_norm_backward": (C.c_int, [_P, _P, _P, _P, _P, _P, _P, _P, C.c_int, C.c_int, C.c_int64, C.c_int, C.c_int, _P,
                                            C.c_size_t, _P]),
    "cd_op_scratch_bytes": (C.c_size_t, [C.c_int, C.c_int, C.c_int64]),
}
EXPORTED_SYMBOLS = tuple(_SIGNATURES)

_lib = None


def load_library() -> C.CDLL:
    global _lib
    if _lib is not None:
        return _lib
    if not os.path.exists(LIB_PATH):
        raise RuntimeError(
            f"{LIB_PATH} is missing: build it with `python -m calodiffusion_amd.build` (hipcc, --offload-arch=gfx950). "
            "calodiffusion_amd has no CPU or PyTorch fallback.")
    _check_built_from_these_sources()
    lib = C.CDLL(LIB_PATH)
    for name, (res, args) in _SIGNATURES.items():
        fn = getattr(lib, name)
        fn.restype, fn.argtypes = res, args
    if lib.cd_abi_version() != CD_ABI_VERSION:
        raise RuntimeError(f"{LIB_PATH} reports ABI version {lib.cd_abi_version()}, this binding is written against "
                           f"{CD_ABI_VERSION} (include/calodiff.h): rebuild with `python -m calodiffusion_amd.build`")
    _lib = lib
    return lib


def _check_built_from_these_sources():
    if os.environ.get("CALODIFF_LIB") or os.environ.get("CD_SKIP_SRCHASH"):
        return
    from . import build
    stamp = LIB_PATH + ".srchash"
    have = open(stamp).read().strip() if os.path.exists(stamp) else None
    want = build.source_hash()
    if have != want:
        raise RuntimeError(f"{LIB_PATH} was not built from the sources in {build.CSRC} (stamp {str(have)[:12]}, sources "
                           f"{want[:12]}): run `python -m calodiffusion_amd.build`")


def _check(code: int):
    if code != 0:
        msg = load_library().cd_last_error().decode(errors="replace")
        exc = ValueError if code == -1 else RuntimeError
        raise exc(f"calodiff[{code}]: {msg}")


def require_gpu() -> str:
    lib = load_library()
    if not torch.cuda.is_available():
        raise RuntimeError("calodiffusion_amd needs an MI355X (gfx950) GPU: torch.cuda.is_available() is False and "
                           "there is no CPU fallback")
    buf = C.create_string_buffer(256)
    _check(lib.cd_device_check(buf, 256))
    return buf.value.decode()


def _ptr(t: Optional[torch.Tensor]) -> Optional[int]:
    return None if t is None else t.data_ptr()


def _stream() -> int:
    return torch.cuda.current_stream().cuda_stream


def _dev32(t: torch.Tensor, name: str) -> torch.Tensor:
    if not isinstance(t, torch.Tensor) or not t.is_cuda:
        raise RuntimeError(f"{name} must be a CUDA(ROCm) tensor: calodiffusion_amd computes on the GPU only")
    if t.dtype != torch.float32 or not t.is_contiguous():
        t = t.to(torch.float32).contiguous()
    return t
# ... 15 lines not shown
        d.grid = _i32x3(unet.grid)
        d.in_channels = unet.channels
        d.n_sizes = len(unet.layer_sizes)
        for i, v in enumerate(unet.layer_sizes):
            d.layer_sizes[i] = int(v)
        d.groups = unet.groups
        d.block_attn = int(bool(unet.block_attn))
        d.mid_attn = int(unet.mid_attn is not False)
        d.compress_z = int(bool(unet.compress_Z))
        d.cond_size, d.cond_dim = unet.cond_size, unet.cond_dim
        d.rz_input, d.phi_input = int(bool(rz_input)), int(bool(phi_input))
        d.time_embed_kind = TIME_KINDS[time_kind]
        d.objective = OBJECTIVES[objective]
        d.sigma_data = float(sigma_data)
        d.time_sin, d.cond_sin = int(bool(getattr(unet, "time_embed", False))), int(bool(getattr(unet, "cond_embed", False)))
        self.desc = d
        self.grid = tuple(unet.grid)
        self.voxels = int(np.prod(self.grid))
        handle = _P()
        _check(self.lib.cd_plan_create(C.byref(d), C.byref(handle)))
        self.plan = handle
        self._weights_version = None
        self._weight_order = None
        self._weight_ids = None
        self._held_weights = []
        self._ws: Dict[tuple, torch.Tensor] = {}
        self.device = next(unet.parameters()).device
        if self.device.type != "cuda":
            raise RuntimeError("move the model to the GPU first (model.to('cuda')): calodiffusion_amd has no CPU path")
        if coords is not None:
            r, z, phi = (np.ascontiguousarray(a, dtype=np.float32) for a in coords)
            assert len(r) == self.grid[2] and len(z) == self.grid[0] and len(phi) == self.grid[1]
            _check(self.lib.cd_plan_set_coords(self.plan, r.ctypes.data, z.ctypes.data, phi.ctypes.data, _stream()))
        self.sync_weights(force=True)

    @classmethod
    def for_unet(cls, unet):
        opts = getattr(unet, "_engine_opts", {})
        return cls(unet, **opts)

    def __del__(self):
        try:
            if getattr(self, "plan", None):
                self.lib.cd_plan_destroy(self.plan)
                self.plan = None
        except Exception:
            pass

    def _version(self):
        ps = list(self.unet.parameters())
        return tuple(p._version for p in ps) + tuple(p.data_ptr() for p in ps) + (tuple(id(p) for p in ps),)

    def sync_weights(self, force=False):
        ver = self._version()
        if not force and ver == self._weights_version:
            return
        ids = ver[-1]
        if self._weight_order is None or self._weight_ids != ids:
            sd = self.unet.state_dict(keep_vars=True)
            n = C.c_int()
            _check(self.lib.cd_plan_num_weights(self.plan, C.byref(n)))
            buf = C.create_string_buffer(256)
            numel = C.c_int64()
            order = []
            for i in range(n.value):
                _check(self.lib.cd_plan_weight_name(self.plan, i, buf, 256, C.byref(numel)))
                name = buf.value.decode()
                if name not in sd:
                    raise RuntimeError(f"state_dict has no tensor named {name!r}")
                if sd[name].numel() != numel.value:
                    raise RuntimeError(f"{name}: {sd[name].numel()} elements, HIP plan expects {numel.value}")
                order.append((name, sd[name]))
            missing = set(sd) - {name for name, _ in order}
            if missing:
                raise RuntimeError(f"HIP plan does not consume these state_dict tensors: {sorted(missing)[:5]} ...")
            self._weight_order, self._weight_ids = order, ids
        tensors = [_dev32(t.detach(), name) for name, t in self._weight_order]
        ptrs = (_P * len(tensors))(*[t.data_ptr() for t in tensors])
        _check(self.lib.cd_plan_set_weights(self.plan, len(tensors), ptrs, _stream()))
        self._held_weights = tensors
        self._weights_version = ver

    _WS_SWITCHES = ("CD_NO_DEEP_LEVEL", "CD_NO_PW_CLOSE", "CD_NO_FUSED_ATTN", "CD_NO_GNDEFER", "CD_ATTN_COMBINE_LAUNCH", "CD_PW_F32",
                    "CD_NO_ATTN_MOMENTS", "CD_ATTN_MOM_MIN", "CD_NO_DEEP_SIDE_CONV")

    def _ws_key(self, batch: int):
        return (int(batch),) + tuple(os.environ.get(k) for k in self._WS_SWITCHES)

    def workspace(self, batch: int) -> torch.Tensor:
        key = ("net",) + self._ws_key(batch)
        ws = self._ws.get(key)
        if ws is None:
            nbytes = C.c_size_t()
            _check(self.lib.cd_plan_workspace_bytes(self.plan, batch, C.byref(nbytes)))
            self._ws = {k: v for k, v in self._ws.items() if k[0] != "net"}
            ws = torch.empty(nbytes.value, dtype=torch.uint8, device=self.device)
            self._ws[key] = ws
        return ws

    def unet_forward(self, x, cond, time):
        x, cond, time = _dev32(x, "x"), _dev32(cond, "cond"), _dev32(time, "time")
        B = x.shape[0]
        if tuple(x.shape[1:]) != (self.unet.channels,) + self.grid:
            raise ValueError(f"x has shape {tuple(x.shape)}, expected (B, {self.unet.channels}, {self.grid})")
        if self.desc.cond_sin:
            if cond.numel() != B:
                raise ValueError("cond_embed='sin' takes cond of shape (B,)")
        elif cond.shape != (B, self.unet.cond_size):
            raise ValueError("cond must be (B, cond_size)")
        if time.numel() != B:
            raise ValueError("time must be (B,)")
        self.sync_weights()
        ws = self.workspace(B)
        out = torch.empty((B, 1) + self.grid, dtype=torch.float32, device=x.device)
        _check(self.lib.cd_unet_forward(self.plan, B, x.data_ptr(), cond.data_ptr(), time.data_ptr(), out.data_ptr(),
                                        ws.data_ptr(), ws.numel(), _stream()))
        return out

    safe_denoise = True

    def denoise(self, x, sigma, cond):
        x, cond = _dev32(x, "x"), _dev32(cond, "cond")
        B = x.shape[0]
        sigma = _dev32(sigma, "sigma").reshape(-1)
        if sigma.numel() == 1 and B > 1:
            sigma = sigma.expand(B).contiguous()
        if tuple(x.shape[1:]) != (1,) + self.grid or sigma.numel() != B or cond.shape != (B, self.unet.cond_size):
            raise ValueError(f"denoise shapes: x {tuple(x.shape)}, sigma {tuple(sigma.shape)}, cond {tuple(cond.shape)}")
        self.sync_weights()
        ws = self.workspace(B)
        out = torch.empty_like(x)
        if self.safe_denoise:
            fell = C.c_int(0)
            _check(self.lib.cd_denoise_safe(self.plan, B, x.data_ptr(), sigma.data_ptr(), cond.data_ptr(), out.data_ptr(),
                                            ws.data_ptr(), ws.numel(), C.byref(fell), _stream()))
            if fell.value:
                self.range_fallbacks = getattr(self, "range_fallbacks", 0) + 1
        else:
            _check(self.lib.cd_denoise(self.plan, B, x.data_ptr(), sigma.data_ptr(), cond.data_ptr(), out.data_ptr(),
                                       ws.data_ptr(), ws.numel(), _stream()))
        return out

    def ddim_sample(self, start, cond, steps: np.ndarray, step_noise=None, seed=0, offset=0, debug=False, use_graph=True,
                    out=None, noise_stride=0):
        start, cond = _dev32(start, "start"), _dev32(cond, "cond")
        B = start.shape[0]
        steps = np.ascontiguousarray(steps, dtype=np.float32)
        n_steps = steps.shape[0]
        assert steps.shape == (n_steps, 4)
        self.sync_weights()
        ws = self.workspace(B)
        x_out = torch.empty_like(start) if out is None else out
        xs = x0s = None
        if debug:
            xs = torch.empty((n_steps,) + tuple(start.shape), dtype=torch.float32, device=start.device)
            x0s = torch.empty_like(xs)
        if step_noise is not None:
            step_noise = _dev32(step_noise, "step_noise")
            assert step_noise.shape[0] == n_steps and step_noise[0].numel() == start.numel()
        _check(self.lib.cd_ddim_sample(self.plan, B, start.data_ptr(), cond.data_ptr(),
                                       steps.ctypes.data_as(C.POINTER(CdStep)), n_steps, _ptr(step_noise), int(seed),
                                       int(offset), int(noise_stride), x_out.data_ptr(), _ptr(xs), _ptr(x0s),
                                       int(bool(use_graph)), ws.data_ptr(), ws.numel(), _stream()))
        self.check_status()
        return x_out, xs, x0s

    def sampler_run(self, start, cond, program, step_noise=None, seed=0, offset=0, noise_stride=0, debug=False, use_graph=True):
# ... 369 lines not shown

def get_conv_precision() -> str:
    return load_library().cd_get_conv_precision().decode()


def profile_begin():
    _check(load_library().cd_profile_begin())


def profile_end() -> dict:
    import json
    buf = C.create_string_buffer(1 << 18)
    _check(load_library().cd_profile_end(buf, 1 << 18))
    return json.loads(buf.value.decode())


def randn(shape, device, seed: int, offset: int = 0) -> torch.Tensor:
    lib = load_library()
    require_gpu()
    out = torch.empty(tuple(shape), dtype=torch.float32, device=device)
    _check(lib.cd_randn(out.data_ptr(), out.numel(), int(seed), int(offset), _stream()))
    return out


class Ops:

    def __init__(self):
        self.lib = load_library()
        require_gpu()
        self._scratch = None

    def scratch(self, batch, channels, voxels):
        need = self.lib.cd_op_scratch_bytes(batch, channels, voxels)
        if self._scratch is None or self._scratch.numel() < need:
            self._scratch = torch.empty(need, dtype=torch.uint8, device="cuda")
        return self._scratch

    def to_channels_last(self, x):
        x = _dev32(x, "x")
        B, Cc = x.shape[:2]
        vox = int(np.prod(x.shape[2:]))
        y = torch.empty((B,) + tuple(x.shape[2:]) + (Cc,), dtype=torch.float32, device=x.device)
        _check(self.lib.cd_op_to_channels_last(x.data_ptr(), y.data_ptr(), B, Cc, vox, _stream()))
        return y

    def to_ncdhw(self, y):
        y = _dev32(y, "y")
        B, Cc = y.shape[0], y.shape[-1]
        vox = int(np.prod(y.shape[1:-1]))
        x = torch.empty((B, Cc) + tuple(y.shape[1:-1]), dtype=torch.float32, device=y.device)
        _check(self.lib.cd_op_to_ncdhw(y.data_ptr(), x.data_ptr(), B, Cc, vox, _stream()))
        return x

    def cyl_conv(self, x_cl, w, bias, stride=(1, 1, 1), x1_cl=None):
        x_cl, w = _dev32(x_cl, "x"), _dev32(w, "w")
        B, D, H, W, c0 = x_cl.shape
        c1 = 0 if x1_cl is None else x1_cl.shape[-1]
        cout = w.shape[0]
        k = tuple(w.shape[2:])
        if k == (1, 1, 1):
            od = (D, H, W)
        else:
            od = ((D + 2 - k[0]) // stride[0] + 1, (H + 2 - k[1]) // stride[1] + 1, (W + 2 - k[2]) // stride[2] + 1)
        y = torch.empty((B,) + od + (cout,), dtype=torch.float32, device=x_cl.device)
        sc = self.scratch(B, max(c0 + c1, cout), D * H * W)
        _check(self.lib.cd_op_cyl_conv(x_cl.data_ptr(), c0, _ptr(x1_cl), c1, w.data_ptr(), _ptr(bias), y.data_ptr(), B, cout,
                                       _i32x3((D, H, W)), _i32x3(k), _i32x3(stride), sc.data_ptr(), _stream()))
        return y

    def zslide_conv_chunked(self, x_cl, w, bias, chunks=0):
        x_cl, w = _dev32(x_cl, "x"), _dev32(w, "w")
        B, D, H, W, cin = x_cl.shape
        cout = w.shape[0]
        y = torch.empty((B, D, H, W, cout), dtype=torch.float32, device=x_cl.device)
        cap = (D * H * W + 31) // 32
        part = torch.zeros((B, cap, cout, 2), dtype=torch.float32, device=x_cl.device)
        units = C.c_int()
        sc = self.scratch(B, max(cin, cout), D * H * W)
        _check(self.lib.cd_op_zslide_conv(x_cl.data_ptr(), cin, w.data_ptr(), _ptr(bias), y.data_ptr(), part.data_ptr(), C.byref(units),
                                          B, cout, _i32x3((D, H, W)), int(chunks), sc.data_ptr(), _stream()))
        u = units.value
        return y, part.view(-1)[:B * u * cout * 2].view(B, u, cout, 2).double().sum(1)

    def cyl_conv_transpose(self, x_cl, w, bias, kernel_z, stride_z, out_pad):
        x_cl, w = _dev32(x_cl, "x"), _dev32(w, "w")
        B, D, H, W, c = x_cl.shape
        od = ((D - 1) * stride_z - 2 + kernel_z, 2 * H + out_pad[1], 2 * W + out_pad[2])
        y = torch.empty((B,) + od + (c,), dtype=torch.float32, device=x_cl.device)
        sc = self.scratch(B, c, int(np.prod(od)))
        _check(self.lib.cd_op_cyl_conv_transpose(x_cl.data_ptr(), w.data_ptr(), _ptr(bias), y.data_ptr(), B, c,
                                                 _i32x3((D, H, W)), kernel_z, stride_z, _i32x3(out_pad), sc.data_ptr(),
                                                 _stream()))
        return y

    def init_conv(self, x_ncdhw, w, bias):
        x, w = _dev32(x_ncdhw, "x"), _dev32(w, "w")
        B, cin, D, H, W = x.shape
        cout = w.shape[0]
        y = torch.empty((B, D, H, W, cout), dtype=torch.float32, device=x.device)
        sc = self.scratch(B, cout, D * H * W)
        _check(self.lib.cd_op_init_conv(x.data_ptr(), w.data_ptr(), _ptr(bias), y.data_ptr(), B, cin, cout, _i32x3((D, H, W)),
                                        sc.data_ptr(), _stream()))
        return y

    def group_norm(self, x_cl, gamma, beta, groups, silu=False, add_bc=None, residual=None):
        x = _dev32(x_cl, "x")
        B, Cc = x.shape[0], x.shape[-1]
        vox = int(np.prod(x.shape[1:-1]))
        y = torch.empty_like(x)
        sc = self.scratch(B, Cc, vox)
        _check(self.lib.cd_op_group_norm(x.data_ptr(), y.data_ptr(), gamma.data_ptr(), beta.data_ptr(), B, Cc, vox, groups,
                                         int(silu), _ptr(add_bc), _ptr(residual), sc.data_ptr(), _stream()))
        return y

    def _bws(self, nbytes=1 << 30):
        if getattr(self, "_bwd_ws", None) is None or self._bwd_ws.numel() < nbytes:
            self._bwd_ws = torch.empty(nbytes, dtype=torch.uint8, device="cuda")
        return self._bwd_ws

    def conv_backward(self, x_cl, w, dy_cl, stride=(1, 1, 1), x1_cl=None, need_dx=True, bias=True):
        x, w, dy = _dev32(x_cl, "x"), _dev32(w, "w"), _dev32(dy_cl, "dy")
        B, D, H, W, c0 = x.shape
        c1 = 0 if x1_cl is None else x1_cl.shape[-1]
        cout, k = w.shape[0], tuple(w.shape[2:])
        dx = torch.empty((B, D, H, W, c0 + c1), dtype=torch.float32, device=x.device) if need_dx else None
        dw = torch.empty_like(w)
        db = torch.empty((cout,), dtype=torch.float32, device=x.device) if bias else None
        ws = self._bws()
        _check(self.lib.cd_op_conv_backward(x.data_ptr(), c0, _ptr(x1_cl), c1, w.data_ptr(), dy.data_ptr(), _ptr(dx), dw.data_ptr(),
                                            _ptr(db), B, cout, _i32x3((D, H, W)), _i32x3(k), _i32x3(stride), ws.data_ptr(),
                                            ws.numel(), _stream()))
        return dx, dw, db

    def conv_transpose_backward(self, x_cl, w, dy_cl, kernel_z, stride_z, out_pad):
        x, w, dy = _dev32(x_cl, "x"), _dev32(w, "w"), _dev32(dy_cl, "dy")
        B, D, H, W, c = x.shape
        dx, dw = torch.empty_like(x), torch.empty_like(w)
        db = torch.empty((c,), dtype=torch.float32, device=x.device)
        ws = self._bws()
        _check(self.lib.cd_op_conv_transpose_backward(x.data_ptr(), w.data_ptr(), dy.data_ptr(), dx.data_ptr(), dw.data_ptr(),
                                                      db.data_ptr(), B, c, _i32x3((D, H, W)), kernel_z, stride_z, _i32x3(out_pad),
                                                      ws.data_ptr(), ws.numel(), _stream()))
        return dx, dw, db

    def group_norm_backward(self, x_cl, gamma, beta, dy_cl, groups, silu=False, want_dadd=False):
        x, dy = _dev32(x_cl, "x"), _dev32(dy_cl, "dy")
        B, Cc = x.shape[0], x.shape[-1]
        vox = int(np.prod(x.shape[1:-1]))
        dx, dg, db = torch.empty_like(x), torch.empty_like(gamma), torch.empty_like(beta)
        dadd = torch.empty((B, Cc), dtype=torch.float32, device=x.device) if want_dadd else None
        ws = self._bws()
        _check(self.lib.cd_op_group_norm_backward(x.data_ptr(), gamma.data_ptr(), beta.data_ptr(), dy.data_ptr(), dx.data_ptr(),
                                                  dg.data_ptr(), db.data_ptr(), _ptr(dadd), B, Cc, vox, groups, int(silu),
                                                  ws.data_ptr(), ws.numel(), _stream()))
        return dx, dg, db, dadd

    _RES_KEYS = ("block1.proj.conv.weight", "block1.proj.conv.bias", "block1.norm.weight", "block1.norm.bias",
                 "block2.proj.conv.weight", "block2.proj.conv.bias", "block2.norm.weight", "block2.norm.bias",
                 "mlp.1.weight", "mlp.1.bias", "res_conv.conv.weight", "res_conv.conv.bias")

    def resnet_block(self, x_cl, sd: Dict[str, torch.Tensor], cond=None, groups=8, x1_cl=None):
        x = _dev32(x_cl, "x")
        B, D, H, W, c0 = x.shape
        c1 = 0 if x1_cl is None else x1_cl.shape[-1]
        cout = sd["block1.proj.conv.weight"].shape[0]
        ptrs = (_P * 12)(*[(sd[k].data_ptr() if k in sd else None) for k in self._RES_KEYS])
# ... 21 lines not shown
```

include/calodiff.h:

```cpp
#ifndef CALODIFF_H
#define CALODIFF_H

#include <stddef.h>
#include <stdint.h>

#ifdef __cplusplus
extern "C" {
#endif

#define CD_OK 0
#define CD_EINVAL -1
#define CD_EHIP -2
#define CD_ENOGPU -3
#define CD_EWEIGHTS -4
#define CD_EWORKSPACE -5

#define CD_MAX_SIZES 8

#define CD_ABI_VERSION 3

#define CD_TIME_LOG 0
#define CD_TIME_SIGMA 1
#define CD_TIME_RAW 2

// ... 79 lines not shown
int cd_plan_grad_layout(const CdPlan* plan, int idx, int64_t* offset, int64_t* total_floats);
int cd_plan_train_workspace_bytes(CdPlan* plan, int batch, size_t* bytes);

int cd_plan_status(CdPlan* plan, int* flags, void* stream);
int cd_train_step(CdPlan* plan, int batch, const float* data, const float* noise, const float* sigma, const float* cond,
                  int loss_type , double* loss_out, float* grads, void* workspace, size_t workspace_bytes,
                  void* stream);

int cd_plan_vjp_workspace_bytes(CdPlan* plan, int batch, int with_param_grads, size_t* bytes);
int cd_denoise_vjp(CdPlan* plan, int batch, const float* x, const float* sigma, const float* cond, const float* gy,
                   float* dx, float* grads , void* workspace, size_t workspace_bytes, void* stream);

int cd_plan_bns_workspace_bytes(CdPlan* plan, int batch, int n_steps, size_t* bytes);
int cd_bns_theta_grad(CdPlan* plan, int batch, int n_steps, const float* data, const float* cond, const float* theta,
                      const float* sigma, double* loss_out, float* dtheta, void* workspace, size_t workspace_bytes, void* stream);

int cd_adam_step(int n, float* const* params, const float* const* grads, float* const* exp_avg, float* const* exp_avg_sq,
                 const int64_t* numel, double lr, double beta1, double beta2, float eps, float weight_decay, int step, void* stream);

int cd_reverse_norm(const float* voxels, const float* energy, const float* layerE, float* out, int batch, const int32_t dims[3],
                    const float consts[6], float max_deposit, float ecut, void* stream);

int cd_reverse_norm_staged(const float* voxels, const float* energy, const float* layerE, float* out, int batch,
                           const int32_t dims[3], const float consts[6], float max_deposit, float ecut, float alpha, float layer_eps,
                           int stage, void* stream);

int cd_preprocess(const float* showers, const float* energy, float* out, float* layerE, float* e_out, int32_t* status, int batch,
                  const int32_t dims[3], const float consts[6], float max_deposit, float emin, float emax, int logE,
                  float shower_scale, void* stream);

typedef struct CdLayerMlpDesc {
  uint32_t struct_size;
  int32_t dim_in;
  int32_t hidden;
  int32_t cond_emb;
  int32_t cond_size;
  int32_t n_res;
  int32_t time_embed_kind;
  int32_t objective;
  float sigma_data;
} CdLayerMlpDesc;

int cd_layer_forward(const CdLayerMlpDesc* desc, const float* const* weights, int n_weights, int batch, const float* x,
                     const float* cond, const float* time, float* out, void* stream);
int cd_layer_denoise(const CdLayerMlpDesc* desc, const float* const* weights, int n_weights, int batch, const float* x,
                     const float* sigma, const float* cond, float* out, void* stream);
int cd_layer_sample(const CdLayerMlpDesc* desc, const float* const* weights, int n_weights, int batch, const float* start,
                    const float* cond, const CdStep* steps_dev, int n_steps, const float* step_noise, float* x_out, float* xs,
                    float* x0s, void* stream);
int cd_layer_sampler_run(const CdLayerMlpDesc* desc, const float* const* weights, int n_weights, int batch, const float* start,
                         float start_scale, const float* cond, int n_bufs, int n_steps, const CdSamplerOp* ops_dev, int n_ops,
                         const int32_t* op_begin_dev, const float* coefs_dev, int n_coef, const float* step_noise, uint64_t seed,
                         uint64_t offset, uint64_t noise_stride, float* x_out, float* xs, float* x0s, void* stream);

int cd_layer_train_workspace_bytes(const CdLayerMlpDesc* desc, int batch, size_t* bytes);
int cd_layer_train_step(const CdLayerMlpDesc* desc, const float* const* weights, int n_weights, int batch, const float* data,
                        const float* noise, const float* sigma, const float* cond, double* loss_out, float* grads,
                        void* workspace, size_t workspace_bytes, void* stream);
int cd_layer_train_step_loss(const CdLayerMlpDesc* desc, const float* const* weights, int n_weights, int batch, const float* data,
                             const float* noise, const float* sigma, const float* cond, int loss_type ,
                             double* loss_out, float* grads, void* workspace, size_t workspace_bytes, void* stream);
int cd_layer_loss(const CdLayerMlpDesc* desc, const float* const* weights, int n_weights, int batch, const float* data,
                  const float* noise, const float* sigma, const float* cond, int loss_type , double* loss_out,
                  void* workspace, size_t workspace_bytes, void* stream);

int cd_layer_vjp_workspace_bytes(const CdLayerMlpDesc* desc, int batch, int with_param_grads, size_t* bytes);
int cd_layer_denoise_vjp(const CdLayerMlpDesc* desc, const float* const* weights, int n_weights, int batch, const float* x,
                         const float* sigma, const float* cond, const float* gy, float* dx, float* grads ,
                         void* workspace, size_t workspace_bytes, void* stream);

int cd_set_conv_precision(const char* mode);
const char* cd_get_conv_precision(void);

int cd_profile_begin(void);
int cd_profile_end(char* json, int cap);

int cd_op_to_channels_last(const float* ncdhw, float* ndhwc, int batch, int channels, int64_t voxels, void* stream);
int cd_op_to_ncdhw(const float* ndhwc, float* ncdhw, int batch, int channels, int64_t voxels, void* stream);
int cd_op_cyl_conv(const float* x0, int c0, const float* x1, int c1, const float* w, const float* bias, float* y,
                   int batch, int cout, const int32_t dims_in[3], const int32_t kernel[3], const int32_t stride[3],
                   void* scratch, void* stream);
int cd_op_zslide_conv(const float* x, int cin, const float* w, const float* bias, float* y, float* ch_part, int* units, int batch,
                      int cout, const int32_t dims[3], int chunks, void* scratch, void* stream);
int cd_op_cyl_conv_transpose(const float* x, const float* w, const float* bias, float* y, int batch, int channels,
                             const int32_t dims_in[3], int kernel_z, int stride_z, const int32_t out_pad[3],
                             void* scratch, void* stream);
int cd_op_init_conv(const float* x_ncdhw, const float* w, const float* bias, float* y, int batch, int cin, int cout,
                    const int32_t dims[3], void* scratch, void* stream);
int cd_op_group_norm(const float* x, float* y, const float* gamma, const float* beta, int batch, int channels,
                     int64_t voxels, int groups, int silu, const float* add_bc, const float* residual,
                     void* scratch, void* stream);
int cd_op_resnet_block(const float* x0, int c0, const float* x1, int c1, const float* const* w, const float* cond, float* y,
                       int batch, int cout, const int32_t dims[3], int groups, void* workspace, size_t workspace_bytes,
                       void* stream);
int cd_op_linear_attention(const float* x, const float* const* w, float* y, int batch, int channels, const int32_t dims[3],
                           void* workspace, size_t workspace_bytes, void* stream);
int cd_op_conv_backward(const float* x0, int c0, const float* x1, int c1, const float* w, const float* dy, float* dx, float* dw,
                        float* db, int batch, int cout, const int32_t dims_in[3], const int32_t kernel[3],
                        const int32_t stride[3], void* workspace, size_t workspace_bytes, void* stream);
int cd_op_conv_transpose_backward(const float* x, const float* w, const float* dy, float* dx, float* dw, float* db, int batch,
                                  int channels, const int32_t dims_in[3], int kernel_z, int stride_z, const int32_t out_pad[3],
                                  void* workspace, size_t workspace_bytes, void* stream);
int cd_op_group_norm_backward(const float* x, const float* gamma, const float* beta, const float* dy, float* dx, float* dgamma,
                              float* dbeta, float* dadd, int batch, int channels, int64_t voxels, int groups, int silu,
                              void* workspace, size_t workspace_bytes, void* stream);
size_t cd_op_scratch_bytes(int batch, int max_channels, int64_t max_voxels);

#ifdef __cplusplus
}
#endif
#endif
```

Measured before the change: 91.57.

## Fuse a second level side conv into the deep-level launch via flat kernel

Extends the deep-level fused launch so it also runs the skip-half K-block of a second upsampling level's concat conv (level 1) as flat f16x2 conv units, appended to the same grid. The remaining x half then runs as a flat conv that accumulates onto that side result through add_src. The aim is to fill idle CUs during the latency-bound deep level and drop a separate launch. In exchange it adds LDS and register pressure to the fused kernel, more workspace bookkeeping, and a new side-tile tiling path.

Result: no change. 92.43, median of 6 (+0.9%).

```diff
diff --git a/calodiffusion_amd/csrc/cd_common.h b/calodiffusion_amd/csrc/cd_common.h
--- a/calodiffusion_amd/csrc/cd_common.h
+++ b/calodiffusion_amd/csrc/cd_common.h
@@ -89,6 +89,7 @@
   const float* add_src = nullptr;
   int* add_done = nullptr;
   int zs_chunks = 0;
+  bool flat_side_tile = false;
   struct GnOut {
     const float* gamma = nullptr;
     const float* beta = nullptr;
@@ -161,6 +162,9 @@
                             int batch, int cout, const ConvGeom& g, hipStream_t s, const ConvFusion& fu);
 bool try_launch_conv_small(const float* in0, int c0, const float* in1, int c1, const void* wpk_f16x2, const float* bias, float* out,
                            int batch, int cout, const ConvGeom& g, hipStream_t s, const ConvFusion& fu);
+bool try_launch_conv3_flat(const float* in0, int c0, const float* in1, int c1, const void* wpk, const float* bias, float* out,
+                           int batch, int cout, const ConvGeom& g, hipStream_t s, const ConvFusion& fu,
+                           int prec );
 void launch_conv_transpose_mfma(const float* in, int cin, const float* wpk, const float* bias, float* out, int batch,
                                 int cout, Dims3 din, Dims3 dout, int kz, int sz, hipStream_t s,
                                 const void* wpk_f16x2 = nullptr, int* status = nullptr, const unsigned* in_absmax = nullptr);
@@ -353,8 +357,9 @@
   Dims3 dims{};
 };
 int deep_side_conv_chunks(int batch, int cin_side, int cout, Dims3 dims);
+int deep_side_flat_units(int cin_side, int cout, Dims3 dims);
 void launch_deep_level_side(const DeepLevelDesc& d, const float* x_in, float* x_out, int batch, int* status, const DeepSideConv& side,
-                            hipStream_t s);
+                            const DeepSideConv* side1, hipStream_t s);
 bool attn_small_eligible(int64_t vox);
 void launch_attn_small(const float* x, int C, const float* coef, const void* wqkv_f16x2, float* partials, const float* w_out,
                        float scale, const float* bias, const float* out_gamma, const float* out_beta, float* y, float* ch_part,
diff --git a/calodiffusion_amd/csrc/conv_flat16_body.inc b/calodiffusion_amd/csrc/conv_flat16_body.inc
--- /dev/null
+++ b/calodiffusion_amd/csrc/conv_flat16_body.inc
@@ -0,0 +1,286 @@
+  char* ldsb = (char*)lds;
+  constexpr int T = KD * KH * KW;
+  constexpr int VB = NTERM == 3 ? 96 : 80;
+  constexpr int WS = 64 * NTERM;
+  const int tid = threadIdx.x, lane = tid & 63, wave = tid >> 6, nthreads = blockDim.x;
+  const int b = kb.y;
+  const int ct0 = kb.z * CT;
+  const int HW = a.H * a.W;
+  const int vox = a.D * HW;
+  const int HWo = a.Ho * a.Wo;
+  const int voxo = a.Do * HWo;
+  const int v0 = kb.x * a.R;
+  const int vend = min(v0 + a.R, voxo);
+  const float inv_hwo = 1.f / (float)HWo, inv_wo = 1.f / (float)a.Wo;
+  auto fdiv = [](int x, float inv) { return (int)(((float)x + 0.5f) * inv); };
+  const int zA = fdiv(v0, inv_hwo) * SZ - 1;
+  const int zB = fdiv(vend - 1, inv_hwo) * SZ + KD - 2;
+  const int nstage = (zB - zA + 1) * HW;
+  const int NZ = a.P * HW;
+  const int half = lane >> 5, col = lane & 31;
+  if (a.defer.part) gn_defer_to_lds(a.defer, b, (float*)(ldsb + a.coef_lds_off), ldsb + a.coef_lds_off + a.defer.C * 16);
+  const bool normed = a.coef || a.defer.part;
+  if (tid < VB / 4) ((float*)(ldsb + (size_t)NZ * VB))[tid] = 0.f;
+
+  int nb[VT], rowoff[VT][KH], ooff[VT];
+  unsigned wmask[VT];
+  bool any_valid = false;
+#pragma unroll
+  for (int vt = 0; vt < VT; ++vt) {
+    const int v = v0 + (wave * VT + vt) * 32 + col;
+    const bool valid = v < vend;
+    const int vv = valid ? v : v0;
+    const int oz = fdiv(vv, inv_hwo);
+    const int r = vv - oz * HWo;
+    const int oh = fdiv(r, inv_wo), ow = r - oh * a.Wo;
+    const int ih0 = oh * SXY, iw0 = ow * SXY;
+    nb[vt] = (oz * SZ - 1 - zA) * HW + ih0 * a.W + iw0;
+    unsigned m = 0;
+#pragma unroll
+    for (int kh = 0; kh < KH; ++kh) {
+      int ih = ih0 + kh - 1;
+      ih = ih < 0 ? ih + a.H : (ih >= a.H ? ih - a.H : ih);
+      ih = ih >= a.H ? ih - a.H : ih;
+      rowoff[vt][kh] = (ih - ih0) * a.W;
+    }
+#pragma unroll
+    for (int kw = 0; kw < KW; ++kw) {
+      const int iw = iw0 + kw - 1;
+      if (valid && iw >= 0 && iw < a.W) m |= 1u << kw;
+    }
+    wmask[vt] = m;
+    ooff[vt] = valid ? v * a.cout : -1;
+    any_valid |= valid;
+  }
+  const bool wave_active = __any(any_valid);
+
+  f32x16 acc[VT][CT], accB[NTERM == 2 ? VT : 1][NTERM == 2 ? CT : 1];
+#pragma unroll
+  for (int vt = 0; vt < VT; ++vt)
+#pragma unroll
+    for (int ct = 0; ct < CT; ++ct)
+#pragma unroll
+      for (int r = 0; r < 16; ++r) {
+        acc[vt][ct][r] = 0.f;
+        if (NTERM == 2) accB[vt][ct][r] = 0.f;
+      }
+
+  float amax = 0.f;
+  float gscale = 1.f, ginv = 1.f;
+  if (NTERM == 2 && a.in_absmax) pow2_scale_for(*a.in_absmax, &gscale, &ginv);
+  const int nsub = (a.c0 + a.c1) >> 4;
+  const int gbase = zA * HW;
+  const int nslots = nstage * 4;
+
+  auto tap_voxel = [&](int vt, int tap) -> int {
+#ifdef CD_FLAT_ABL_TAPS
+    return nb[vt] + tap;
+#endif
+    const int kz = tap / (KH * KW), kh = (tap / KW) % KH, kw = tap % KW;
+    const int n = nb[vt] + kz * HW + rowoff[vt][kh] + kw - 1;
+    return ((wmask[vt] >> kw) & 1u) ? n : NZ;
+  };
+
+  for (int sc = 0; sc < nsub; ++sc) {
+    const float* src;
+    int ldc, coff;
+    if (sc * 16 < a.c0) {
+      src = a.in0; ldc = a.c0; coff = sc * 16;
+    } else {
+      src = a.in1; ldc = a.c1; coff = sc * 16 - a.c0;
+    }
+    const int pq = tid & 3;
+    src += (size_t)b * vox * ldc + coff + pq * 4;
+    f32x4 cf[4];
+    if (a.defer.part) {
+#pragma unroll
+      for (int e = 0; e < 4; ++e) cf[e] = *(const f32x4*)(ldsb + a.coef_lds_off + (sc * 16 + pq * 4 + e) * 16);
+    } else if (a.coef) {
+#pragma unroll
+      for (int e = 0; e < 4; ++e) cf[e] = *(const f32x4*)(a.coef + ((size_t)b * (a.c0 + a.c1) + sc * 16 + pq * 4 + e) * 4);
+    }
+    __syncthreads();
+    for (int s0 = tid; s0 < ((a.dbg & 1) ? 0 : nslots); s0 += 4 * nthreads) {
+      f32x4 val[4];
+#pragma unroll
+      for (int k = 0; k < 4; ++k) {
+        const int sidx = s0 + k * nthreads;
+        const int g = gbase + (sidx >> 2);
+        val[k] = f32x4{0.f, 0.f, 0.f, 0.f};
+        if (sidx < nslots && g >= 0 && g < vox) {
+          val[k] = *(const f32x4*)(src + (size_t)g * ldc);
+          if (normed) {
+#pragma unroll
+            for (int e = 0; e < 4; ++e) {
+              float t = cf[e][0] * val[k][e] + cf[e][1];
+              if (a.act) t = cd_fast_silu(t);
+              val[k][e] = t + cf[e][2];
+            }
+          }
+        }
+      }
+#pragma unroll
+      for (int k = 0; k < 4; ++k) {
+        const int sidx = s0 + k * nthreads;
+        if (sidx < nslots) {
+          char* d = ldsb + (size_t)(sidx >> 2) * VB + pq * 8;
+          if (NTERM == 3) {
+            u32x2 t1, t2, t3;
+            split3(val[k], t1, t2, t3);
+            *(u32x2*)d = t1;
+            *(u32x2*)(d + 32) = t2;
+            *(u32x2*)(d + 64) = t3;
+          } else {
+            const f32x4 vs = val[k] * gscale;
+            amax = fmaxf(amax, fmaxf(fmaxf(fabsf(vs[0]), fabsf(vs[1])), fmaxf(fabsf(vs[2]), fabsf(vs[3]))));
+            u32x2 t1, t2;
+            split2(vs, t1, t2);
+            *(u32x2*)d = t1;
+            *(u32x2*)(d + 32) = t2;
+          }
+        }
+      }
+    }
+    __syncthreads();
+    if (!wave_active || (a.dbg & 2)) continue;
+
+#pragma unroll
+    for (int vt = 0; vt < VT; ++vt) asm volatile("" : "+v"(nb[vt]));
+
+    const u32x4* wq = (const u32x4*)a.wpk + ((size_t)sc * T * a.CTtot + ct0) * WS + lane;
+#ifndef CD_FLAT_WD
+#define CD_FLAT_WD 3
+#endif
+#ifndef CD_FLAT_AD
+#define CD_FLAT_AD 2
+#endif
+    constexpr bool DEEP = NTERM == 2;
+    constexpr int WD = DEEP ? CD_FLAT_WD : 1, AD = DEEP ? CD_FLAT_AD : 1;
+    u32x4 bw[WD + 1][CT][NTERM], av[AD + 1][VT][NTERM];
+    auto load_w = [&](int tap) {
+#pragma unroll
+      for (int ct = 0; ct < CT; ++ct)
+#pragma unroll
+        for (int t = 0; t < NTERM; ++t) bw[tap % (WD + 1)][ct][t] = wq[((size_t)tap * a.CTtot + ct) * WS + t * 64];
+    };
+    auto load_a = [&](int tap) {
+#pragma unroll
+      for (int vt = 0; vt < VT; ++vt) {
+        const char* p = ldsb + (size_t)tap_voxel(vt, tap) * VB + half * 16;
+#pragma unroll
+        for (int t = 0; t < NTERM; ++t) av[tap % (AD + 1)][vt][t] = *(const u32x4*)(p + t * 32);
+      }
+    };
+#pragma unroll
+    for (int t0 = 0; t0 < WD; ++t0) load_w(t0);
+#pragma unroll
+    for (int t0 = 0; t0 < AD; ++t0) load_a(t0);
+#pragma unroll
+    for (int tap = 0; tap < T; ++tap) {
+      if (tap + WD < T) load_w(tap + WD);
+      if (tap + AD < T) load_a(tap + AD);
+      __builtin_amdgcn_sched_barrier(0);
+      const int wc = tap % (WD + 1), ac = tap % (AD + 1);
+#pragma unroll
+      for (int vt = 0; vt < VT; ++vt)
+#pragma unroll
+        for (int ct = 0; ct < CT; ++ct) {
+          if (NTERM == 3) {
+            f32x16 c = acc[vt][ct];
+            c = MFMA_BF16(av[ac][vt][NTERM - 1], bw[wc][ct][0], c);
+            c = MFMA_BF16(av[ac][vt][1], bw[wc][ct][1], c);
+            c = MFMA_BF16(av[ac][vt][0], bw[wc][ct][NTERM - 1], c);
+            c = MFMA_BF16(av[ac][vt][1], bw[wc][ct][0], c);
+            c = MFMA_BF16(av[ac][vt][0], bw[wc][ct][1], c);
+            c = MFMA_BF16(av[ac][vt][0], bw[wc][ct][0], c);
+            acc[vt][ct] = c;
+          } else {
+            acc[vt][ct] = MFMA_F16(av[ac][vt][0], bw[wc][ct][0], acc[vt][ct]);
+            accB[vt][ct] = MFMA_F16(av[ac][vt][0], bw[wc][ct][1], accB[vt][ct]);
+            accB[vt][ct] = MFMA_F16(av[ac][vt][1], bw[wc][ct][0], accB[vt][ct]);
+          }
+        }
+    }
+  }
+
+  if (NTERM == 2) {
+#pragma unroll
+    for (int vt = 0; vt < VT; ++vt)
+#pragma unroll
+      for (int ct = 0; ct < CT; ++ct)
+#pragma unroll
+        for (int r = 0; r < 16; ++r) acc[vt][ct][r] = (acc[vt][ct][r] + accB[vt][ct][r] * (1.f / 2048.f)) * ginv;
+  }
+  if (NTERM == 2 && a.status && amax > 65504.f) atomicOr(a.status, 1);
+  float* outb = a.out + (size_t)b * voxo * a.cout;
+  float bv[CT];
+#pragma unroll
+  for (int ct = 0; ct < CT; ++ct) bv[ct] = a.bias ? a.bias[(ct0 + ct) * 32 + col] : 0.f;
+  if (a.add_src) {
+    const float* addb = a.add_src + (size_t)b * voxo * a.cout;
+#pragma unroll
+    for (int vt = 0; vt < VT; ++vt) {
+      float ad[16][CT];
+#pragma unroll
+      for (int r = 0; r < 16; ++r) {
+        const int off = __shfl(ooff[vt], (r & 3) + 8 * (r >> 2) + 4 * half, 64);
+#pragma unroll
+        for (int ct = 0; ct < CT; ++ct) ad[r][ct] = off >= 0 ? addb[off + (ct0 + ct) * 32 + col] : 0.f;
+      }
+#pragma unroll
+      for (int r = 0; r < 16; ++r)
+#pragma unroll
+        for (int ct = 0; ct < CT; ++ct) acc[vt][ct][r] += ad[r][ct];
+    }
+  }
+#pragma unroll
+  for (int vt = 0; vt < VT; ++vt) {
+#pragma unroll
+    for (int r = 0; r < 16; ++r) {
+      const int row = (r & 3) + 8 * (r >> 2) + 4 * half;
+      const int off = __shfl(ooff[vt], row, 64);
+      if (off >= 0) {
+#pragma unroll
+        for (int ct = 0; ct < CT; ++ct) outb[off + (ct0 + ct) * 32 + col] = acc[vt][ct][r] + bv[ct];
+      }
+    }
+  }
+  if (a.ch_part) {
+    float s1[CT], s2[CT];
+#pragma unroll
+    for (int ct = 0; ct < CT; ++ct) s1[ct] = s2[ct] = 0.f;
+#pragma unroll
+    for (int vt = 0; vt < VT; ++vt)
+#pragma unroll
+      for (int r = 0; r < 16; ++r) {
+        const int row = (r & 3) + 8 * (r >> 2) + 4 * half;
+        const bool ok = __shfl(ooff[vt], row, 64) >= 0;
+#pragma unroll
+        for (int ct = 0; ct < CT; ++ct) {
+          const float v = ok ? acc[vt][ct][r] + bv[ct] : 0.f;
+          s1[ct] += v;
+          s2[ct] += v * v;
+        }
+      }
+    __syncthreads();
+    const int nw = nthreads >> 6;
+#pragma unroll
+    for (int ct = 0; ct < CT; ++ct) {
+      const float t1 = s1[ct] + __shfl_xor(s1[ct], 32, 64), t2 = s2[ct] + __shfl_xor(s2[ct], 32, 64);
+      if (half == 0) {
+        lds[((wave * CT + ct) * 32 + col) * 2] = t1;
+        lds[((wave * CT + ct) * 32 + col) * 2 + 1] = t2;
+      }
+    }
+    __syncthreads();
+    for (int i = tid; i < CT * 32; i += nthreads) {
+      float t1 = 0.f, t2 = 0.f;
+      for (int w = 0; w < nw; ++w) {
+        t1 += lds[((w * CT * 32) + i) * 2];
+        t2 += lds[((w * CT * 32) + i) * 2 + 1];
+      }
+      float* dst = a.ch_part + (((size_t)b * kb.nx + kb.x) * a.cout + ct0 * 32 + i) * 2;
+      dst[0] = t1;
+      dst[1] = t2;
+    }
+  }
diff --git a/calodiffusion_amd/csrc/conv_internal.h b/calodiffusion_amd/csrc/conv_internal.h
--- a/calodiffusion_amd/csrc/conv_internal.h
+++ b/calodiffusion_amd/csrc/conv_internal.h
@@ -74,9 +74,12 @@
   const unsigned* in_absmax = nullptr;
   const float* add_src = nullptr;
 };
-bool try_launch_conv3_flat(const float* in0, int c0, const float* in1, int c1, const void* wpk, const float* bias, float* out,
-                           int batch, int cout, const ConvGeom& g, hipStream_t s, const ConvFusion& fu,
-                           int prec );
+struct FlatBlk {
+  unsigned x, y, z, nx;
+};
+__device__ __forceinline__ FlatBlk flat_blk_of_grid() { return FlatBlk{blockIdx.x, blockIdx.y, blockIdx.z, gridDim.x}; }
+bool flat_side_job(const float* in, int cin, const void* wpk_f16x2, const float* bias, float* out, int cout, Dims3 dims, int* status,
+                   ConvFlatArgs* args, size_t* lds_bytes, int* units);
 bool launch_conv_flat_split16(int VT, int CT, int NTERM, int geo, const ConvFlatArgs& a, dim3 grid, int threads, size_t lds, hipStream_t s);
 
 std::map<std::string, int>& tune_cache();
diff --git a/calodiffusion_amd/csrc/forward.hip b/calodiffusion_amd/csrc/forward.hip
--- a/calodiffusion_amd/csrc/forward.hip
+++ b/calodiffusion_amd/csrc/forward.hip
@@ -83,24 +83,49 @@
   return part;
 }
 
+static float* conv3_x_half_flat_with_stats(Run& r, const float* x0, int c0, int c1, const void* wpk3, const float* side, float* out,
+                                           int cout, Dims3 dims, int* units) {
+  const int64_t vox = dims.vox();
+  const int cap = (int)((vox + 31) / 32);
+  float* part = r.ws->get<float>((size_t)r.B * cap * cout * 2);
+  int u = 0;
+  if (!r.dry()) {
+    ConvGeom g{dims, dims, 3, 3, 3, 1, 1, 1};
+    ConvFusion fu;
+    int added = 0;
+    fu.act = 1; fu.ch_part = part; fu.units = &u; fu.status = r.status; fu.add_src = side; fu.add_done = &added;
+    char cat[128];
+    std::snprintf(cat, sizeof cat, "conv3x3x3_s1 C%d(of %d)->%d @%dx%dx%d", c0, c0 + c1, cout, dims.d, dims.h, dims.w);
+    prof::Scope scope(cat, r.s, 2.0 * 27 * c0 * cout * (double)vox * r.B, 4.0 * r.B * (double)vox * (c0 + 2 * cout));
+    const bool ran = try_launch_conv3_flat(x0, c0, nullptr, 0, (const char*)wpk3 + packed_bf16x3_bytes(c0 + c1, cout, 27), nullptr, out, r.B,
+                                           cout, g, r.s, fu, 2);
+    CD_REQUIRE(ran && added && u > 0, "internal: the x half of a level-1 side conv must run as a flat f16x2 continuation");
+  }
+  *units = u;
+  return part;
+}
+
 struct LazyClose {
   GnDefer gn;
   float* part = nullptr;
   bool on = false;
 };
 float* res_block(Run& r, const ResP& w, const float* x0, int c0, const float* x1, int c1, Dims3 dims,
-                 float** part_out, int* units_out, LazyClose* lazy, float* h1_side) {
+                 float** part_out, int* units_out, LazyClose* lazy, float* h1_side, bool side_flat) {
   Arena* ws = r.ws;
   CD_REQUIRE(c0 + c1 == w.cin, "internal: resnet block input width mismatch");
   const int64_t vox = dims.vox();
   const int G = r.groups;
   int u1 = 0, u2 = 0;
   static const bool defer_gn = getenv("CD_NO_GNDEFER") == nullptr;
-  float* h1 = h1_side ? h1_side : ws->get<float>((size_t)r.B * vox * w.cout);
+  float* h1 = h1_side && !side_flat ? h1_side : ws->get<float>((size_t)r.B * vox * w.cout);
   const bool whole = vox <= 128 && w.cout == 32 && defer_gn && conv_precision() == PREC_F16X2 && w.c1w3 && w.c2w3;
   float* p1 = nullptr;
-  CD_REQUIRE(!h1_side || (!whole && c1 > 0), "internal: a side conv belongs to a concat conv on a full-resolution grid");
-  if (h1_side) p1 = conv3_x_half_with_stats(r, x0, c0, c1, w.c1w3, h1, w.cout, dims, &u1);
+  CD_REQUIRE(!h1_side || (!whole && c1 > 0), "internal: a side conv belongs to a concat conv that runs as two K-blocks");
+  if (h1_side && side_flat) {
+    p1 = conv3_x_half_flat_with_stats(r, x0, c0, c1, w.c1w3, h1_side, h1, w.cout, dims, &u1);
+    ws->release(h1_side);
+  } else if (h1_side) p1 = conv3_x_half_with_stats(r, x0, c0, c1, w.c1w3, h1, w.cout, dims, &u1);
   else if (!whole) p1 = conv3_with_stats(r, x0, c0, x1, c1, w.c1w, w.c1w3, w.c1b, h1, w.cout, dims, nullptr, &u1);
   else p1 = ws->get<float>((size_t)r.B * ((vox + 31) / 32) * w.cout * 2);
   float* coef1 = ws->get<float>((size_t)r.B * w.cout * 4);
@@ -451,20 +476,34 @@
   const int side_c = nres >= 2 ? d.layer_sizes[1] : 0;
   const bool side_on = deep_on && nres >= 2 && side_w.cin == 2 * side_c && p->packed3(side_w.c1w) &&
                        deep_side_conv_chunks(r.B, side_c, side_w.cout, p->shapes[0]) > 0;
+  const int l1 = nres - 2;
+  const ResW& side1_w = p->ups[nres >= 3 ? 1 : 0].r1;
+  const int side1_c = nres >= 3 ? d.layer_sizes[l1 + 1] : 0;
+  const bool side1_on = side_on && nres >= 3 && side1_w.cin == 2 * side1_c && p->packed3(side1_w.c1w) &&
+                        deep_side_flat_units(side1_c, side1_w.cout, p->shapes[l1]) > 0;
   float* side_h1 = nullptr;
+  float* side1_h1 = nullptr;
   for (int i = 0; i < nres; ++i) {
     const Dims3 dims = p->shapes[i];
     if (deep_on && i == nres - 1) {
       float* y = r.ws->get<float>((size_t)r.B * dims.vox() * cx);
       if (side_on) {
         side_h1 = r.ws->get<float>((size_t)r.B * p->shapes[0].vox() * side_w.cout);
+        if (side1_on) side1_h1 = r.ws->get<float>((size_t)r.B * p->shapes[l1].vox() * side1_w.cout);
         if (!r.dry()) {
           DeepSideConv sc;
           sc.in = skips[0]; sc.ldc = side_c; sc.cin = side_c;
           sc.wpk = (const char*)p->packed3(side_w.c1w) + packed_bf16x3_bytes(side_w.cin, side_w.cout, 27) +
                    (size_t)(side_c / 16) * 27 * (side_w.cout / 32) * 128 * 16;
           sc.bias = p->raw(side_w.c1b); sc.out = side_h1; sc.cout = side_w.cout; sc.dims = p->shapes[0];
-          launch_deep_level_side(deep, x, y, r.B, r.status, sc, r.s);
+          DeepSideConv sc1;
+          if (side1_on) {
+            sc1.in = skips[l1]; sc1.ldc = side1_c; sc1.cin = side1_c;
+            sc1.wpk = (const char*)p->packed3(side1_w.c1w) + packed_bf16x3_bytes(side1_w.cin, side1_w.cout, 27) +
+                      (size_t)(side1_c / 16) * 27 * (side1_w.cout / 32) * 128 * 16;
+            sc1.bias = p->raw(side1_w.c1b); sc1.out = side1_h1; sc1.cout = side1_w.cout; sc1.dims = p->shapes[l1];
+          }
+          launch_deep_level_side(deep, x, y, r.B, r.status, sc, side1_on ? &sc1 : nullptr, r.s);
         }
       } else if (!r.dry()) {
         launch_deep_level(deep, x, y, r.B, r.status, r.s);
@@ -527,7 +566,7 @@
     if (!(deep_on && i == 0)) {
       CD_REQUIRE(cx == cs, "internal: up path width mismatch");
       t = res_block(r, resolve(p, p->ups[i].r1, emb), x, cx, skips[lv], cs, dims, nullptr, nullptr, nullptr,
-                    lv == 0 ? side_h1 : nullptr);
+                    lv == 0 ? side_h1 : (lv == l1 ? side1_h1 : nullptr), lv != 0);
       r.ws->release(x);
       r.ws->release(skips[lv]);
       x = t; cx = p->ups[i].r1.cout;
diff --git a/calodiffusion_amd/csrc/kernels_conv_flat.hip b/calodiffusion_amd/csrc/kernels_conv_flat.hip
--- a/calodiffusion_amd/csrc/kernels_conv_flat.hip
+++ b/calodiffusion_amd/csrc/kernels_conv_flat.hip
@@ -487,6 +487,34 @@
 #undef CD_FLAT_CASE
   return false;
 }
+}
+
+static constexpr int kSideNT = 8, kSideVT = 2;
+static_assert(kSideNT / kSideVT * 64 == 256, "the deepest level's launch has four waves per workgroup");
+
+bool flat_side_job(const float* in, int cin, const void* wpk_f16x2, const float* bias, float* out, int cout, Dims3 d, int* status,
+                   ConvFlatArgs* args, size_t* lds_bytes, int* units) {
+  if (getenv("CD_NO_FLAT") || getenv("CD_FLAT_TILE") || getenv("CD_FLAT_DBG")) return false;
+  if (cin < 16 || cin % 16 || cout < 32 || cout % 32) return false;
+  const int CTtot = cout / 32;
+  if (CTtot % (CTtot <= 3 ? CTtot : 2)) return false;
+  const int HW = d.h * d.w;
+  const int64_t vox = d.vox();
+  if (HW < 1 || HW >= 64 || vox <= 128 || vox <= 32 * (kSideNT - 1) || vox >= (1 << 20)) return false;
+  const int P = ((32 * kSideNT - 1) / HW + 1) + 3;
+  const size_t lds = ((size_t)P * HW + 1) * 80;
+  if (lds > 150 * 1024) return false;
+  if (args) {
+    ConvFlatArgs a;
+    a.in0 = in; a.in1 = nullptr; a.c0 = cin; a.c1 = 0; a.wpk = (const float*)wpk_f16x2; a.bias = bias; a.out = out;
+    a.D = d.d; a.H = d.h; a.W = d.w; a.Do = d.d; a.Ho = d.h; a.Wo = d.w;
+    a.R = 32 * kSideNT; a.P = P; a.cout = cout; a.CTtot = CTtot; a.dbg = 0;
+    a.coef = nullptr; a.act = 0; a.ch_part = nullptr; a.status = status;
+    *args = a;
+  }
+  if (lds_bytes) *lds_bytes = lds;
+  if (units) *units = (int)((vox + 32 * kSideNT - 1) / (32 * kSideNT));
+  return true;
 }
 
 bool try_launch_conv3_flat(const float* in0, int c0, const float* in1, int c1, const void* wpk, const float* bias, float* out,
@@ -556,6 +584,9 @@
     if (a.add_src && fu.add_done) *fu.add_done = 1;
     return true;
   };
+  if (fu.flat_side_tile)
+    return prec == 2 && geo == 0 && c1 == 0 && flat_side_job(in0, c0, wpk, bias, out, cout, d, nullptr, nullptr, nullptr, nullptr) &&
+           launch(kSideNT, kSideVT, 1);
   if (const char* ov = getenv("CD_FLAT_TILE")) {
     int nt, vt;
     if (sscanf(ov, "%d,%d", &nt, &vt) == 2 && nt % vt == 0 && nt / vt <= 8 && vt * CTmax <= 8 &&
diff --git a/calodiffusion_amd/csrc/kernels_conv_flat16.hip b/calodiffusion_amd/csrc/kernels_conv_flat16.hip
--- a/calodiffusion_amd/csrc/kernels_conv_flat16.hip
+++ b/calodiffusion_amd/csrc/kernels_conv_flat16.hip
@@ -6,292 +6,8 @@
 template <int VT, int CT, int KD, int KH, int KW, int SZ, int SXY, int NTERM>
 __global__ void __launch_bounds__(512, (VT * CT * (NTERM == 2 ? 2 : 1) <= 2 ? 3 : 2)) conv3_flat_bf16x3_kernel(ConvFlatArgs a) {
   extern __shared__ __attribute__((aligned(16))) float lds[];
-  char* ldsb = (char*)lds;
-  constexpr int T = KD * KH * KW;
-  constexpr int VB = NTERM == 3 ? 96 : 80;
-  constexpr int WS = 64 * NTERM;
-  const int tid = threadIdx.x, lane = tid & 63, wave = tid >> 6, nthreads = blockDim.x;
-  const int b = blockIdx.y;
-  const int ct0 = blockIdx.z * CT;
-  const int HW = a.H * a.W;
-  const int vox = a.D * HW;
-  const int HWo = a.Ho * a.Wo;
-  const int voxo = a.Do * HWo;
-  const int v0 = blockIdx.x * a.R;
-  const int vend = min(v0 + a.R, voxo);
-  const float inv_hwo = 1.f / (float)HWo, inv_wo = 1.f / (float)a.Wo;
-  auto fdiv = [](int x, float inv) { return (int)(((float)x + 0.5f) * inv); };
-  const int zA = fdiv(v0, inv_hwo) * SZ - 1;
-  const int zB = fdiv(vend - 1, inv_hwo) * SZ + KD - 2;
-  const int nstage = (zB - zA + 1) * HW;
-  const int NZ = a.P * HW;
-  const int half = lane >> 5, col = lane & 31;
-  if (a.defer.part) gn_defer_to_lds(a.defer, b, (float*)(ldsb + a.coef_lds_off), ldsb + a.coef_lds_off + a.defer.C * 16);
-  const bool normed = a.coef || a.defer.part;
-  if (tid < VB / 4) ((float*)(ldsb + (size_t)NZ * VB))[tid] = 0.f;
-
-  int nb[VT], rowoff[VT][KH], ooff[VT];
-  unsigned wmask[VT];
-  bool any_valid = false;
-#pragma unroll
-  for (int vt = 0; vt < VT; ++vt) {
-    const int v = v0 + (wave * VT + vt) * 32 + col;
-    const bool valid = v < vend;
-    const int vv = valid ? v : v0;
-    const int oz = fdiv(vv, inv_hwo);
-    const int r = vv - oz * HWo;
-    const int oh = fdiv(r, inv_wo), ow = r - oh * a.Wo;
-    const int ih0 = oh * SXY, iw0 = ow * SXY;
-    nb[vt] = (oz * SZ - 1 - zA) * HW + ih0 * a.W + iw0;
-    unsigned m = 0;
-#pragma unroll
-    for (int kh = 0; kh < KH; ++kh) {
-      int ih = ih0 + kh - 1;
-      ih = ih < 0 ? ih + a.H : (ih >= a.H ? ih - a.H : ih);
-      ih = ih >= a.H ? ih - a.H : ih;
-      rowoff[vt][kh] = (ih - ih0) * a.W;
-    }
-#pragma unroll
-    for (int kw = 0; kw < KW; ++kw) {
-      const int iw = iw0 + kw - 1;
-      if (valid && iw >= 0 && iw < a.W) m |= 1u << kw;
-    }
-    wmask[vt] = m;
-    ooff[vt] = valid ? v * a.cout : -1;
-    any_valid |= valid;
-  }
-  const bool wave_active = __any(any_valid);
-
-  f32x16 acc[VT][CT], accB[NTERM == 2 ? VT : 1][NTERM == 2 ? CT : 1];
-#pragma unroll
-  for (int vt = 0; vt < VT; ++vt)
-#pragma unroll
-    for (int ct = 0; ct < CT; ++ct)
-#pragma unroll
-      for (int r = 0; r < 16; ++r) {
-        acc[vt][ct][r] = 0.f;
-        if (NTERM == 2) accB[vt][ct][r] = 0.f;
-      }
-
-  float amax = 0.f;
-  float gscale = 1.f, ginv = 1.f;
-  if (NTERM == 2 && a.in_absmax) pow2_scale_for(*a.in_absmax, &gscale, &ginv);
-  const int nsub = (a.c0 + a.c1) >> 4;
-  const int gbase = zA * HW;
-  const int nslots = nstage * 4;
-
-  auto tap_voxel = [&](int vt, int tap) -> int {
-#ifdef CD_FLAT_ABL_TAPS
-    return nb[vt] + tap;
-#endif
-    const int kz = tap / (KH * KW), kh = (tap / KW) % KH, kw = tap % KW;
-    const int n = nb[vt] + kz * HW + rowoff[vt][kh] + kw - 1;
-    return ((wmask[vt] >> kw) & 1u) ? n : NZ;
-  };
-
-  for (int sc = 0; sc < nsub; ++sc) {
-    const float* src;
-    int ldc, coff;
-    if (sc * 16 < a.c0) {
-      src = a.in0; ldc = a.c0; coff = sc * 16;
-    } else {
-      src = a.in1; ldc = a.c1; coff = sc * 16 - a.c0;
-    }
-    const int pq = tid & 3;
-    src += (size_t)b * vox * ldc + coff + pq * 4;
-    f32x4 cf[4];
-    if (a.defer.part) {
-#pragma unroll
-      for (int e = 0; e < 4; ++e) cf[e] = *(const f32x4*)(ldsb + a.coef_lds_off + (sc * 16 + pq * 4 + e) * 16);
-    } else if (a.coef) {
-#pragma unroll
-      for (int e = 0; e < 4; ++e) cf[e] = *(const f32x4*)(a.coef + ((size_t)b * (a.c0 + a.c1) + sc * 16 + pq * 4 + e) * 4);
-    }
-    __syncthreads();
-    for (int s0 = tid; s0 < ((a.dbg & 1) ? 0 : nslots); s0 += 4 * nthreads) {
-      f32x4 val[4];
-#pragma unroll
-      for (int k = 0; k < 4; ++k) {
-        const int sidx = s0 + k * nthreads;
-        const int g = gbase + (sidx >> 2);
-        val[k] = f32x4{0.f, 0.f, 0.f, 0.f};
-        if (sidx < nslots && g >= 0 && g < vox) {
-          val[k] = *(const f32x4*)(src + (size_t)g * ldc);
-          if (normed) {
-#pragma unroll
-            for (int e = 0; e < 4; ++e) {
-              float t = cf[e][0] * val[k][e] + cf[e][1];
-              if (a.act) t = cd_fast_silu(t);
-              val[k][e] = t + cf[e][2];
-            }
-          }
-        }
-      }
-#pragma unroll
-      for (int k = 0; k < 4; ++k) {
-        const int sidx = s0 + k * nthreads;
-        if (sidx < nslots) {
-          char* d = ldsb + (size_t)(sidx >> 2) * VB + pq * 8;
-          if (NTERM == 3) {
-            u32x2 t1, t2, t3;
-            split3(val[k], t1, t2, t3);
-            *(u32x2*)d = t1;
-            *(u32x2*)(d + 32) = t2;
-            *(u32x2*)(d + 64) = t3;
-          } else {
-            const f32x4 vs = val[k] * gscale;
-            amax = fmaxf(amax, fmaxf(fmaxf(fabsf(vs[0]), fabsf(vs[1])), fmaxf(fabsf(vs[2]), fabsf(vs[3]))));
-            u32x2 t1, t2;
-            split2(vs, t1, t2);
-            *(u32x2*)d = t1;
-            *(u32x2*)(d + 32) = t2;
-          }
-        }
-      }
-    }
-    __syncthreads();
-    if (!wave_active || (a.dbg & 2)) continue;
-
-#pragma unroll
-    for (int vt = 0; vt < VT; ++vt) asm volatile("" : "+v"(nb[vt]));
-
-    const u32x4* wq = (const u32x4*)a.wpk + ((size_t)sc * T * a.CTtot + ct0) * WS + lane;
-#ifndef CD_FLAT_WD
-#define CD_FLAT_WD 3
-#endif
-#ifndef CD_FLAT_AD
-#define CD_FLAT_AD 2
-#endif
-    constexpr bool DEEP = NTERM == 2;
-    constexpr int WD = DEEP ? CD_FLAT_WD : 1, AD = DEEP ? CD_FLAT_AD : 1;
-    u32x4 bw[WD + 1][CT][NTERM], av[AD + 1][VT][NTERM];
-    auto load_w = [&](int tap) {
-#pragma unroll
-      for (int ct = 0; ct < CT; ++ct)
-#pragma unroll
-        for (int t = 0; t < NTERM; ++t) bw[tap % (WD + 1)][ct][t] = wq[((size_t)tap * a.CTtot + ct) * WS + t * 64];
-    };
-    auto load_a = [&](int tap) {
-#pragma unroll
-      for (int vt = 0; vt < VT; ++vt) {
-        const char* p = ldsb + (size_t)tap_voxel(vt, tap) * VB + half * 16;
-#pragma unroll
-        for (int t = 0; t < NTERM; ++t) av[tap % (AD + 1)][vt][t] = *(const u32x4*)(p + t * 32);
-      }
-    };
-#pragma unroll
-    for (int t0 = 0; t0 < WD; ++t0) load_w(t0);
-#pragma unroll
-    for (int t0 = 0; t0 < AD; ++t0) load_a(t0);
-#pragma unroll
-    for (int tap = 0; tap < T; ++tap) {
-      if (tap + WD < T) load_w(tap + WD);
-      if (tap + AD < T) load_a(tap + AD);
-      __builtin_amdgcn_sched_barrier(0);
-      const int wc = tap % (WD + 1), ac = tap % (AD + 1);
-#pragma unroll
-      for (int vt = 0; vt < VT; ++vt)
-#pragma unroll
-        for (int ct = 0; ct < CT; ++ct) {
-          if (NTERM == 3) {
-            f32x16 c = acc[vt][ct];
-            c = MFMA_BF16(av[ac][vt][NTERM - 1], bw[wc][ct][0], c);
-            c = MFMA_BF16(av[ac][vt][1], bw[wc][ct][1], c);
-            c = MFMA_BF16(av[ac][vt][0], bw[wc][ct][NTERM - 1], c);
-            c = MFMA_BF16(av[ac][vt][1], bw[wc][ct][0], c);
-            c = MFMA_BF16(av[ac][vt][0], bw[wc][ct][1], c);
-            c = MFMA_BF16(av[ac][vt][0], bw[wc][ct][0], c);
-            acc[vt][ct] = c;
-          } else {
-            acc[vt][ct] = MFMA_F16(av[ac][vt][0], bw[wc][ct][0], acc[vt][ct]);
-            accB[vt][ct] = MFMA_F16(av[ac][vt][0], bw[wc][ct][1], accB[vt][ct]);
-            accB[vt][ct] = MFMA_F16(av[ac][vt][1], bw[wc][ct][0], accB[vt][ct]);
-          }
-        }
-    }
-  }
-
-  if (NTERM == 2) {
-#pragma unroll
-    for (int vt = 0; vt < VT; ++vt)
-#pragma unroll
-      for (int ct = 0; ct < CT; ++ct)
-#pragma unroll
-        for (int r = 0; r < 16; ++r) acc[vt][ct][r] = (acc[vt][ct][r] + accB[vt][ct][r] * (1.f / 2048.f)) * ginv;
-  }
-  if (NTERM == 2 && a.status && amax > 65504.f) atomicOr(a.status, 1);
-  float* outb = a.out + (size_t)b * voxo * a.cout;
-  float bv[CT];
-#pragma unroll
-  for (int ct = 0; ct < CT; ++ct) bv[ct] = a.bias ? a.bias[(ct0 + ct) * 32 + col] : 0.f;
-  if (a.add_src) {
-    const float* addb = a.add_src + (size_t)b * voxo * a.cout;
-#pragma unroll
-    for (int vt = 0; vt < VT; ++vt) {
-      float ad[16][CT];
-#pragma unroll
-      for (int r = 0; r < 16; ++r) {
-        const int off = __shfl(ooff[vt], (r & 3) + 8 * (r >> 2) + 4 * half, 64);
-#pragma unroll
-        for (int ct = 0; ct < CT; ++ct) ad[r][ct] = off >= 0 ? addb[off + (ct0 + ct) * 32 + col] : 0.f;
-      }
-#pragma unroll
-      for (int r = 0; r < 16; ++r)
-#pragma unroll
-        for (int ct = 0; ct < CT; ++ct) acc[vt][ct][r] += ad[r][ct];
-    }
-  }
-#pragma unroll
-  for (int vt = 0; vt < VT; ++vt) {
-#pragma unroll
-    for (int r = 0; r < 16; ++r) {
-      const int row = (r & 3) + 8 * (r >> 2) + 4 * half;
-      const int off = __shfl(ooff[vt], row, 64);
-      if (off >= 0) {
-#pragma unroll
-        for (int ct = 0; ct < CT; ++ct) outb[off + (ct0 + ct) * 32 + col] = acc[vt][ct][r] + bv[ct];
-      }
-    }
-  }
-  if (a.ch_part) {
-    float s1[CT], s2[CT];
-#pragma unroll
-    for (int ct = 0; ct < CT; ++ct) s1[ct] = s2[ct] = 0.f;
-#pragma unroll
-    for (int vt = 0; vt < VT; ++vt)
-#pragma unroll
-      for (int r = 0; r < 16; ++r) {
-        const int row = (r & 3) + 8 * (r >> 2) + 4 * half;
-        const bool ok = __shfl(ooff[vt], row, 64) >= 0;
-#pragma unroll
-        for (int ct = 0; ct < CT; ++ct) {
-          const float v = ok ? acc[vt][ct][r] + bv[ct] : 0.f;
-          s1[ct] += v;
-          s2[ct] += v * v;
-        }
-      }
-    __syncthreads();
-    const int nw = nthreads >> 6;
-#pragma unroll
-    for (int ct = 0; ct < CT; ++ct) {
-      const float t1 = s1[ct] + __shfl_xor(s1[ct], 32, 64), t2 = s2[ct] + __shfl_xor(s2[ct], 32, 64);
-      if (half == 0) {
-        lds[((wave * CT + ct) * 32 + col) * 2] = t1;
-        lds[((wave * CT + ct) * 32 + col) * 2 + 1] = t2;
-      }
-    }
-    __syncthreads();
-    for (int i = tid; i < CT * 32; i += nthreads) {
-      float t1 = 0.f, t2 = 0.f;
-      for (int w = 0; w < nw; ++w) {
-        t1 += lds[((w * CT * 32) + i) * 2];
-        t2 += lds[((w * CT * 32) + i) * 2 + 1];
-      }
-      float* dst = a.ch_part + (((size_t)b * gridDim.x + blockIdx.x) * a.cout + ct0 * 32 + i) * 2;
-      dst[0] = t1;
-      dst[1] = t2;
-    }
-  }
+  const FlatBlk kb = flat_blk_of_grid();
+#include "conv_flat16_body.inc"
 }
 
 namespace {
diff --git a/calodiffusion_amd/csrc/kernels_deep_side.hip b/calodiffusion_amd/csrc/kernels_deep_side.hip
--- a/calodiffusion_amd/csrc/kernels_deep_side.hip
+++ b/calodiffusion_amd/csrc/kernels_deep_side.hip
@@ -1,5 +1,4 @@
-#include "cd_common.h"
-#include "split16.h"
+#include "conv_internal.h"
 #include "gn_defer.h"
 
 #include <cstdio>
@@ -19,7 +18,14 @@
   DeepArgs deep;
   ConvZsArgs side;
   int ndeep;
+  ConvFlatArgs flat;
+  int nzs, fl_units, fl_ct;
 };
+
+__device__ __forceinline__ void flat_side_body(const ConvFlatArgs& a, float* lds, const FlatBlk kb) {
+  constexpr int VT = 2, CT = 1, KD = 3, KH = 3, KW = 3, SZ = 1, SXY = 1, NTERM = 2;
+#include "conv_flat16_body.inc"
+}
 
 template <int NT>
 __global__ void __launch_bounds__(256, 1) deep_level_side_kernel(DeepSideArgs a) {
@@ -30,6 +36,16 @@
     return;
   }
   const int j = bx - a.ndeep;
+  if (j >= a.nzs) {
+    const unsigned k = j - a.nzs, r = k / a.fl_units;
+    FlatBlk fb;
+    fb.x = k - r * a.fl_units;
+    fb.y = r / a.fl_ct;
+    fb.z = r - fb.y * a.fl_ct;
+    fb.nx = a.fl_units;
+    flat_side_body(a.flat, (float*)ds_lds, fb);
+    return;
+  }
   ZsBlk kb;
   kb.y = j / a.side.nchunk;
   kb.x = j - kb.y * a.side.nchunk;
@@ -83,8 +99,14 @@
   return best;
 }
 
+int deep_side_flat_units(int cin_side, int cout, Dims3 dims) {
+  if (getenv("CD_NO_DEEP_SIDE_CONV") || getenv("CD_NO_DEEP_SIDE_L1")) return 0;
+  int units = 0;
+  return flat_side_job(nullptr, cin_side, nullptr, nullptr, nullptr, cout, dims, nullptr, nullptr, nullptr, &units) ? units : 0;
+}
+
 void launch_deep_level_side(const DeepLevelDesc& d, const float* x_in, float* x_out, int batch, int* status, const DeepSideConv& sc,
-                            hipStream_t s) {
+                            const DeepSideConv* sc1, hipStream_t s) {
   DeepSideArgs a;
   double flops = 0.0;
   const size_t lds_deep = deep_fill_args(d, x_in, x_out, status, &a.deep, &flops);
@@ -102,16 +124,35 @@
   z.CV = (int)(((svox + nchunk - 1) / nchunk + ZS_STEP - 1) / ZS_STEP * ZS_STEP);
   z.status = status; z.defer = GnDefer(); z.choff = 0; z.in_absmax = nullptr; z.dbg = 0;
   a.ndeep = batch;
+  a.nzs = batch * nchunk;
   const size_t lds_side = side_lds(sc.dims);
-  const size_t lds = lds_deep > lds_side ? lds_deep : lds_side;
-  const int64_t grid = (int64_t)batch * (1 + nchunk);
+  size_t lds = lds_deep > lds_side ? lds_deep : lds_side;
+  int64_t grid = (int64_t)batch * (1 + nchunk);
+  a.flat = ConvFlatArgs{};
+  a.fl_units = a.fl_ct = 1;
+  double flops1 = 0.0, bytes1 = 0.0;
+  char cat1[64] = "";
+  if (sc1) {
+    size_t lds_flat = 0;
+    CD_REQUIRE(sc1->in && sc1->wpk && sc1->out && sc1->ldc == sc1->cin && deep_side_flat_units(sc1->cin, sc1->cout, sc1->dims) > 0 &&
+                   flat_side_job(sc1->in, sc1->cin, sc1->wpk, sc1->bias, sc1->out, sc1->cout, sc1->dims, status, &a.flat, &lds_flat,
+                                 &a.fl_units),
+               "internal: deep level launched with an ineligible second side conv");
+    a.fl_ct = sc1->cout / 32;
+    lds = lds > lds_flat ? lds : lds_flat;
+    grid += (int64_t)batch * a.fl_ct * a.fl_units;
+    const double vox1 = (double)sc1->dims.vox();
+    flops1 = 2.0 * 27 * sc1->cin * sc1->cout * vox1 * batch;
+    bytes1 = 4.0 * batch * vox1 * (sc1->cin + sc1->cout);
+    std::snprintf(cat1, sizeof cat1, " + conv3x3x3 K-block C%d->%d @%dx%dx%d", sc1->cin, sc1->cout, sc1->dims.d, sc1->dims.h, sc1->dims.w);
+  }
   CD_REQUIRE(lds <= 160 * 1024 && grid < (1ll << 31), "deep level + side conv: launch geometry out of range");
   const double vox = (double)d.dims.vox();
-  char cat[128];
-  std::snprintf(cat, sizeof cat, "deep_level C%d/%d @%dx%dx%d + conv3x3x3 K-block C%d->%d @%dx%dx%d", d.Ca, d.Cb, d.dims.d, d.dims.h,
-                d.dims.w, sc.cin, sc.cout, sc.dims.d, sc.dims.h, sc.dims.w);
-  prof::Scope scope(cat, s, flops * batch + 2.0 * 27 * sc.cin * sc.cout * (double)svox * batch,
-                    8.0 * batch * vox * d.Ca + 4.0 * batch * (double)svox * (sc.cin + sc.cout));
+  char cat[192];
+  std::snprintf(cat, sizeof cat, "deep_level C%d/%d @%dx%dx%d + conv3x3x3 K-block C%d->%d @%dx%dx%d%s", d.Ca, d.Cb, d.dims.d, d.dims.h,
+                d.dims.w, sc.cin, sc.cout, sc.dims.d, sc.dims.h, sc.dims.w, cat1);
+  prof::Scope scope(cat, s, flops * batch + 2.0 * 27 * sc.cin * sc.cout * (double)svox * batch + flops1,
+                    8.0 * batch * vox * d.Ca + 4.0 * batch * (double)svox * (sc.cin + sc.cout) + bytes1);
   const int NT = (int)((d.dims.vox() + 31) / 32);
   switch (NT) {
     case 1: launch_deep_side_inst<1>(a, (unsigned)grid, lds, s); break;
diff --git a/calodiffusion_amd/csrc/ops.hip b/calodiffusion_amd/csrc/ops.hip
--- a/calodiffusion_amd/csrc/ops.hip
+++ b/calodiffusion_amd/csrc/ops.hip
@@ -69,6 +69,25 @@
   });
 }
 
+int cd_op_flat_conv(const float* x, int cin, const float* w, const float* bias, const float* add_src, float* y, float* ch_part,
+                    int* units, int batch, int cout, const int32_t dims[3], int side_tile, void* scratch, void* stream) {
+  return guarded([&] {
+    CD_REQUIRE(x && w && y && ch_part && units && scratch, "bad argument");
+    CD_REQUIRE(cin % 32 == 0 && cout % 32 == 0, "channel counts must be multiples of 32");
+    CD_REQUIRE(!(bias && add_src), "the accumulate mode takes no bias");
+    hipStream_t s = (hipStream_t)stream;
+    launch_pack_weights_f16x2(w, scratch, cout, cin, 27, s);
+    const Dims3 d{dims[0], dims[1], dims[2]};
+    ConvGeom g{d, d, 3, 3, 3, 1, 1, 1};
+    ConvFusion fu;
+    int u = 0, added = 0;
+    fu.act = 1; fu.ch_part = ch_part; fu.units = &u; fu.add_src = add_src; fu.add_done = &added; fu.flat_side_tile = side_tile != 0;
+    CD_REQUIRE(try_launch_conv3_flat(x, cin, nullptr, 0, scratch, bias, y, batch, cout, g, s, fu, 2) && u > 0 && (!add_src || added),
+               "this conv is not eligible for the flat f16x2 kernel (in that tiling)");
+    *units = u;
+  });
+}
+
 int cd_op_cyl_conv_transpose(const float* x, const float* w, const float* bias, float* y, int batch, int channels,
                              const int32_t dims_in[3], int kernel_z, int stride_z, const int32_t out_pad[3],
                              void* scratch, void* stream) {
diff --git a/calodiffusion_amd/csrc/plan_internal.h b/calodiffusion_amd/csrc/plan_internal.h
--- a/calodiffusion_amd/csrc/plan_internal.h
+++ b/calodiffusion_amd/csrc/plan_internal.h
@@ -257,7 +257,8 @@
                         const float* bias, float* out, int cout, Dims3 dims, const float* coef_in, int* units,
                         const GnDefer* defer_in = nullptr, float* coef_buf = nullptr, const ConvFusion::GnOut* gn_out = nullptr);
 float* res_block(Run& r, const ResP& w, const float* x0, int c0, const float* x1, int c1, Dims3 dims,
-                 float** part_out = nullptr, int* units_out = nullptr, LazyClose* lazy = nullptr, float* h1_side = nullptr);
+                 float** part_out = nullptr, int* units_out = nullptr, LazyClose* lazy = nullptr, float* h1_side = nullptr,
+                 bool side_flat = false);
 float* attn_block(Run& r, const AttnP& w, const float* x, Dims3 dims, float* xpart = nullptr, int xunits = 0);
 void bias_grad(Run& r, const float* dy, int C, int64_t vox, float* db);
 void conv_backward(Run& r, const float* x0, int c0, const float* x1, int c1, const float* w_raw, const float* dy, float* dx,
diff --git a/calodiffusion_amd/engine.py b/calodiffusion_amd/engine.py
--- a/calodiffusion_amd/engine.py
+++ b/calodiffusion_amd/engine.py
@@ -118,6 +118,8 @@
                                  C.POINTER(C.c_int32), C.POINTER(C.c_int32), _P, _P]),
     "cd_op_zslide_conv": (C.c_int, [_P, C.c_int, _P, _P, _P, _P, C.POINTER(C.c_int), C.c_int, C.c_int, C.POINTER(C.c_int32), C.c_int,
                                     _P, _P]),
+    "cd_op_flat_conv": (C.c_int, [_P, C.c_int, _P, _P, _P, _P, _P, C.POINTER(C.c_int), C.c_int, C.c_int, C.POINTER(C.c_int32), C.c_int,
+                                  _P, _P]),
     "cd_op_cyl_conv_transpose": (C.c_int, [_P, _P, _P, _P, C.c_int, C.c_int, C.POINTER(C.c_int32), C.c_int, C.c_int,
                                            C.POINTER(C.c_int32), _P, _P]),
     "cd_op_init_conv": (C.c_int, [_P, _P, _P, _P, C.c_int, C.c_int, C.c_int, C.POINTER(C.c_int32), _P, _P]),
@@ -299,7 +301,7 @@
         self._weights_version = ver
 
     _WS_SWITCHES = ("CD_NO_DEEP_LEVEL", "CD_NO_PW_CLOSE", "CD_NO_FUSED_ATTN", "CD_NO_GNDEFER", "CD_ATTN_COMBINE_LAUNCH", "CD_PW_F32",
-                    "CD_NO_ATTN_MOMENTS", "CD_ATTN_MOM_MIN", "CD_NO_DEEP_SIDE_CONV")
+                    "CD_NO_ATTN_MOMENTS", "CD_ATTN_MOM_MIN", "CD_NO_DEEP_SIDE_CONV", "CD_NO_DEEP_SIDE_L1")
 
     def _ws_key(self, batch: int):
         return (int(batch),) + tuple(os.environ.get(k) for k in self._WS_SWITCHES)
@@ -835,6 +837,24 @@
         u = units.value
         return y, part.view(-1)[:B * u * cout * 2].view(B, u, cout, 2).double().sum(1)
 
+    def flat_conv(self, x_cl, w, bias=None, add_src=None, side_tile=False):
+        x_cl, w = _dev32(x_cl, "x"), _dev32(w, "w")
+        B, D, H, W, cin = x_cl.shape
+        cout = w.shape[0]
+        if add_src is not None:
+            add_src = _dev32(add_src, "add_src")
+            if tuple(add_src.shape) != (B, D, H, W, cout):
+                raise ValueError("add_src must be shaped like the output")
+        y = torch.empty((B, D, H, W, cout), dtype=torch.float32, device=x_cl.device)
+        cap = (D * H * W + 31) // 32
+        part = torch.zeros((B, cap, cout, 2), dtype=torch.float32, device=x_cl.device)
+        units = C.c_int()
+        sc = self.scratch(B, max(cin, cout), D * H * W)
+        _check(self.lib.cd_op_flat_conv(x_cl.data_ptr(), cin, w.data_ptr(), _ptr(bias), _ptr(add_src), y.data_ptr(), part.data_ptr(),
+                                        C.byref(units), B, cout, _i32x3((D, H, W)), int(bool(side_tile)), sc.data_ptr(), _stream()))
+        u = units.value
+        return y, part.view(-1)[:B * u * cout * 2].view(B, u, cout, 2).double().sum(1)
+
     def cyl_conv_transpose(self, x_cl, w, bias, kernel_z, stride_z, out_pad):
         x_cl, w = _dev32(x_cl, "x"), _dev32(w, "w")
         B, D, H, W, c = x_cl.shape
diff --git a/include/calodiff.h b/include/calodiff.h
--- a/include/calodiff.h
+++ b/include/calodiff.h
@@ -185,6 +185,8 @@
                    void* scratch, void* stream);
 int cd_op_zslide_conv(const float* x, int cin, const float* w, const float* bias, float* y, float* ch_part, int* units, int batch,
                       int cout, const int32_t dims[3], int chunks, void* scratch, void* stream);
+int cd_op_flat_conv(const float* x, int cin, const float* w, const float* bias, const float* add_src, float* y, float* ch_part,
+                    int* units, int batch, int cout, const int32_t dims[3], int side_tile, void* scratch, void* stream);
 int cd_op_cyl_conv_transpose(const float* x, const float* w, const float* bias, float* y, int batch, int channels,
                              const int32_t dims_in[3], int kernel_z, int stride_z, const int32_t out_pad[3],
                              void* scratch, void* stream);
```
